# PythonerJOJO/GenPose2

Hardware: AMD Instinct MI355X
Metric: pose candidates/sec (B objs x K cands x T denoise steps) (higher is better)
Workload: dtype f32 (pose_encoder.2 / head-1 GEMMs: f16x3 -- three f16 planes per fp32 operand, six MFMA products, products to 2^-33, fp32 accumulation; encoder SA levels 1-3: split-f16, per-level error vs float64 within exact fp32 MFMA's: tests/test_gpu_precision.py); 1 GPU; config4: B=256 objects/GPU, N=1024 pts, K=50 candidates, T=500 PC steps, ScoreNet+EnergyNet+ranking/aggregation (encoder + sampler per step); global_batch=256, seq_len=500, parallelism=dp1 (object shards), encoder_pipelined=False, energy_encoder=beside the score encoder

## Files before the change

genpose2_amd/_lib.py:

```python
from __future__ import annotations

import ctypes
import os
from typing import Dict, Iterable

_HERE = os.path.dirname(os.path.abspath(__file__))
LIB_PATH = os.environ.get("GENPOSE_HIP_LIB", os.path.join(_HERE, "libgenpose_hip.so"))

c_int, c_float, c_size_t, c_void_p = ctypes.c_int, ctypes.c_float, ctypes.c_size_t, ctypes.c_void_p
c_double = ctypes.c_double
c_int64_p = ctypes.POINTER(ctypes.c_int64)
c_uint64 = ctypes.c_uint64


class GenPoseHipError(RuntimeError):
    pass


class HeadWeights(ctypes.Structure):
    _fields_ = [(n, c_void_p) for n in ("pe0_w", "pe0_b", "pe2_w", "pe2_b", "h1p_w", "h2_w", "h2_b",
                                       "h1pts_t", "h1_b", "gfp_w", "te_w_t", "te_b", "h1t_t", "pe2_h", "h1p_h",
                                       "hsc")]


class HeadGradWeights(ctypes.Structure):
    _fields_ = [(n, c_void_p) for n in ("pe0_wt", "pe2_wt", "h1p_wt")]


class ScaleWeights(ctypes.Structure):
    _fields_ = [(n, c_void_p) for n in ("ae0_w", "ae0_b", "ae2_w", "ae2_b", "ft0_w", "ft0_b", "ft2_w",
                                       "ft2_b")]


_SIGS: Dict[str, tuple] = {
    "gp_last_error": (ctypes.c_char_p, []),
    "gp_abi_version": (c_int, []),
    "gp_furthest_point_sampling": (c_int, [c_int, c_int, c_int, c_void_p, c_void_p, c_void_p, c_void_p]),
    "gp_gather_points": (c_int, [c_int, c_int, c_int, c_int, c_void_p, c_void_p, c_void_p, c_void_p]),
    "gp_ball_query": (c_int, [c_int, c_int, c_int, c_float, c_int, c_void_p, c_void_p, c_void_p, c_void_p]),
    "gp_group_points": (c_int, [c_int, c_int, c_int, c_int, c_int, c_void_p, c_void_p, c_void_p, c_void_p]),
    "gp_encoder_workspace_size": (c_size_t, [c_int, c_int]),
    "gp_encoder_workspace_layout": (c_int, [c_int, c_int, c_int64_p]),
    "gp_encoder_forward": (c_int, [c_void_p, c_int64_p, c_void_p, c_int, c_int, c_void_p, c_size_t, c_void_p,
                                   c_void_p]),
    "gp_encoder_fps": (c_int, [c_void_p, c_int, c_int, c_void_p, c_size_t, c_void_p]),
    "gp_encoder_geometry": (c_int, [c_void_p, c_int, c_int, c_void_p, c_size_t, c_void_p]),
    "gp_encoder_forward_geom": (c_int, [c_void_p, c_int64_p, c_void_p, c_int, c_int, c_void_p, c_void_p, c_size_t,
                                        c_void_p, c_void_p]),
    "gp_encoder_geometry_levels": (c_int, [c_void_p, c_int, c_int, c_void_p, c_size_t, c_int, c_int, c_void_p]),
    "gp_encoder_forward_geom_levels": (c_int, [c_void_p, c_int64_p, c_void_p, c_int, c_int, c_void_p, c_void_p,
                                               c_size_t, c_void_p, c_int, c_int, c_void_p]),
    "gp_sa_level": (c_int, [c_void_p, c_int64_p, c_int, c_int, c_void_p, c_int, c_int, c_void_p, c_void_p, c_size_t,
                            c_void_p, c_void_p]),
    "gp_sa_level_geom": (c_int, [c_void_p, c_int64_p, c_int, c_int, c_void_p, c_int, c_int, c_void_p, c_void_p,
                                 c_void_p, c_size_t, c_void_p, c_void_p]),
    "gp_linear": (c_int, [c_void_p, c_int, c_int, c_int, c_void_p, c_void_p, c_int, c_int, c_void_p, c_int, c_void_p]),
    "gp_linear_split_words": (c_size_t, [c_int, c_int]),
    "gp_linear_split": (c_int, [c_void_p, c_int, c_int, c_int, c_void_p, c_void_p, c_int, c_int, c_void_p, c_int,
                                c_void_p, c_int, c_void_p, c_void_p]),
    "gp_add_layernorm": (c_int, [c_void_p, c_void_p, c_int, c_int, c_void_p, c_void_p, c_float, c_void_p, c_void_p,
                                 c_void_p]),
    "gp_relpe_bias_bytes": (c_size_t, [c_int, c_int]),
    "gp_relpe_bias": (c_int, [c_void_p, c_void_p, c_int, c_int, c_void_p, c_void_p]),
    "gp_mha_attention": (c_int, [c_void_p, c_void_p, c_int, c_int, c_int, c_void_p, c_void_p, c_void_p]),
    "gp_mha_relpe_attention": (c_int, [c_void_p, c_void_p, c_void_p, c_int, c_int, c_int, c_void_p, c_void_p,
                                       c_void_p]),
    "gp_interp_points": (c_int, [c_void_p, c_int, c_int, c_int, c_int, c_void_p, c_void_p, c_void_p]),
    "gp_fusion_attend_workspace_size": (c_size_t, [c_int, c_int, c_int]),
    "gp_fusion_attend": (c_int, [c_void_p, c_void_p, c_int, c_int, c_int, c_void_p, c_void_p, c_void_p, c_void_p,
                                 c_void_p, c_void_p, c_void_p, c_void_p, c_size_t, c_void_p]),
    "gp_fusion_mix": (c_int, [c_void_p, c_void_p, c_int, c_int, c_void_p, c_void_p]),
    "gp_weights_pack": (c_int, [c_int, c_int, c_void_p, c_void_p, c_void_p, ctypes.POINTER(c_void_p)]),
    "gp_weights_free": (None, [c_void_p]),
    "gp_weights_heads": (ctypes.POINTER(HeadWeights), [c_void_p]),
    "gp_weights_scale": (ctypes.POINTER(ScaleWeights), [c_void_p]),
    "gp_weights_encoder": (c_void_p, [c_void_p, ctypes.POINTER(c_int64_p)]),
    "gp_weights_pack_host": (c_int, [c_int, c_int, c_void_p, c_void_p, c_void_p, c_void_p, c_size_t,
                                     ctypes.POINTER(c_size_t), c_int64_p, c_int64_p]),
    "gp_head_object_proj": (c_int, [ctypes.POINTER(HeadWeights), c_void_p, c_int, c_void_p, c_void_p]),
    "gp_head_time_proj": (c_int, [ctypes.POINTER(HeadWeights), c_void_p, c_int, c_void_p, c_void_p]),
    "gp_score_eval": (c_int, [ctypes.POINTER(HeadWeights), c_void_p, c_void_p, c_float, c_void_p, c_int, c_int,
                              c_void_p, c_void_p]),
    "gp_energy_eval": (c_int, [ctypes.POINTER(HeadWeights), c_void_p, c_void_p, c_float, c_void_p, c_int, c_int,
                               c_void_p, c_void_p]),
    "gp_head_grad_floats": (c_size_t, []),
    "gp_head_grad_pack": (c_int, [c_void_p, c_void_p, c_void_p, c_void_p]),
    "gp_energy_score_eval": (c_int, [ctypes.POINTER(HeadWeights), ctypes.POINTER(HeadGradWeights), c_void_p, c_void_p,
                                     c_float, c_void_p, c_int, c_int, c_void_p, c_void_p, c_void_p]),
    "gp_pc_sample_energy": (c_int, [ctypes.POINTER(HeadWeights), ctypes.POINTER(HeadGradWeights), c_void_p, c_void_p,
                                    c_void_p, c_int, c_void_p, c_int, c_int, c_void_p, c_void_p, c_void_p, c_uint64,
                                    c_float, c_void_p, c_void_p, c_void_p, c_void_p, c_size_t, c_void_p]),
    "gp_pc_workspace_size": (c_size_t, [c_int]),
    "gp_pc_tile_rows": (c_int, [c_int, c_int]),
    "gp_pc_sample": (c_int, [ctypes.POINTER(HeadWeights), c_void_p, c_void_p, c_void_p, c_int, c_void_p, c_int,
                             c_int, c_void_p, c_void_p, c_void_p, c_uint64, c_float, c_void_p, c_void_p, c_void_p,
                             c_void_p, c_size_t, c_void_p]),
    "gp_pc_global_partials": (c_int, [c_int, c_int, c_int, c_int]),
    "gp_pc_sample_global": (c_int, [ctypes.POINTER(HeadWeights), c_void_p, c_void_p, c_void_p, c_int, c_void_p, c_int,
                                    c_int, c_void_p, c_uint64, c_float, c_void_p, c_void_p, c_void_p, c_int, c_int,
                                    c_int, c_int, c_int, c_void_p, c_void_p, c_void_p, c_void_p, c_size_t, c_void_p]),
    "gp_pose_epilogue_f64": (c_int, [c_void_p, c_int, c_int, c_void_p, c_void_p, c_void_p]),
    "gp_ode_workspace_size": (c_size_t, [c_int]),
    "gp_ode_rhs": (c_int, [ctypes.POINTER(HeadWeights), c_void_p, c_float, c_float, c_double, c_void_p, c_void_p,
                           c_void_p, c_int, c_double, c_int, c_int, c_void_p, c_void_p, c_size_t, c_void_p]),
    "gp_ode_attempt": (c_int, [ctypes.POINTER(HeadWeights), c_void_p, c_void_p, c_void_p, c_void_p, c_void_p,
                               c_void_p, c_void_p, c_void_p, c_void_p, c_double, c_double, c_double, c_int, c_int,
                               c_void_p, c_void_p, c_void_p, c_size_t, c_void_p]),
    "gp_score_div_eval": (c_int, [ctypes.POINTER(HeadWeights), c_void_p, c_void_p, c_float, c_void_p, c_void_p, c_int,
                                  c_int, c_void_p, c_void_p, c_void_p]),
    "gp_like_workspace_size": (c_size_t, [c_int]),
    "gp_like_rhs": (c_int, [ctypes.POINTER(HeadWeights), c_void_p, c_float, c_float, c_double, c_void_p, c_void_p,
                            c_void_p, c_void_p, c_int, c_double, c_int, c_int, c_void_p, c_void_p, c_size_t,
                            c_void_p]),
    "gp_like_attempt": (c_int, [ctypes.POINTER(HeadWeights), c_void_p, c_void_p, c_void_p, c_void_p, c_void_p,
                                c_void_p, c_void_p, c_void_p, c_void_p, c_void_p, c_double, c_double, c_double,
                                c_int, c_int, c_void_p, c_void_p, c_void_p, c_size_t, c_void_p]),
    "gp_ode_init_norms": (c_int, [c_void_p, c_void_p, c_void_p, ctypes.c_longlong, c_double, c_double, c_void_p,
                                  c_void_p]),
    "gp_ode_dense": (c_int, [c_void_p, c_void_p, c_void_p, c_void_p, c_int, c_int, c_int, c_int, c_double, c_double,
                             ctypes.c_longlong, c_void_p, c_void_p]),
    "gp_ode_denoise": (c_int, [ctypes.POINTER(HeadWeights), c_void_p, c_float, c_float, c_float, c_float, c_void_p,
                               c_int, c_int, c_void_p, c_void_p, c_void_p, c_void_p, c_size_t, c_void_p]),
    "gp_ode_ctl_size": (c_size_t, []),
    "gp_ode_auto_workspace_size": (c_size_t, [c_int]),
    "gp_ode_auto_attempt": (c_int, [ctypes.POINTER(HeadWeights), c_void_p, c_int, c_int, c_double, c_double, c_double,
                                    c_double, c_double, c_double, c_double, c_void_p, c_void_p, c_void_p, c_void_p,
                                    c_void_p, c_void_p, c_int, c_int, c_void_p, c_size_t, c_void_p]),
    "gp_ode_auto_attempt_hs": (c_int, [ctypes.POINTER(HeadWeights), c_void_p, c_int, c_int, c_double, c_double, c_double,
                                    c_double, c_double, c_double, c_double, c_void_p, c_void_p, c_void_p, c_void_p,
                                    c_void_p, c_void_p, c_int, c_int, c_void_p, c_size_t, c_void_p, c_void_p]),
    "gp_ode_global_partials": (c_int, [c_int, c_int, c_int, c_int]),
    "gp_ode_global_workspace_size": (c_size_t, [c_int]),
    "gp_ode_auto_partials_offset": (c_size_t, []),
    "gp_ode_auto_attempt_global": (c_int, [ctypes.POINTER(HeadWeights), c_void_p, c_int, c_int, c_double, c_double,
                                           c_double, c_double, c_double, c_double, c_double, c_void_p, c_void_p,
                                           c_void_p, c_void_p, c_void_p, c_void_p, c_int, c_int, c_int, c_int, c_int,
                                           c_int, c_int, c_void_p, c_void_p, c_void_p, c_size_t, c_void_p,
                                           c_void_p]),
    "gp_pc_step_table": (c_int, [c_int, c_float, c_void_p]),
    "gp_ode_sample_workspace_size": (c_size_t, [c_int]),
    "gp_ode_sample": (c_int, [ctypes.POINTER(HeadWeights), c_void_p, c_void_p, c_int, c_int, c_double, c_double,
                              c_int, c_double, c_double, c_void_p, c_void_p, c_void_p, ctypes.POINTER(c_int),
                              ctypes.POINTER(c_int), c_void_p, c_size_t, c_void_p]),
    "gp_img_encoder_workspace_size": (c_size_t, [c_int, c_int, c_int]),
    "gp_img_encoder": (c_int, [c_void_p, c_void_p, c_void_p, c_int, c_int, c_int, c_void_p, c_void_p, c_void_p, c_float,
                               c_void_p, c_void_p, c_void_p, c_float, c_float, c_void_p, c_void_p, c_void_p, c_void_p,
                               c_size_t, c_void_p]),
    "gp_img_encoder2": (c_int, [c_void_p, c_void_p, c_void_p, c_int, c_int, c_int, c_void_p, c_void_p, c_void_p, c_float,
                                c_void_p, c_void_p, c_void_p, c_float, c_float, c_void_p, c_void_p, c_void_p, c_void_p,
                                c_void_p, c_void_p, c_size_t, c_void_p]),
    "gp_img_encoder3": (c_int, [c_void_p, c_void_p, c_void_p, c_int, c_int, c_int, c_void_p, c_void_p, c_void_p, c_float,
                                c_void_p, c_void_p, c_void_p, c_float, c_float, c_void_p, c_void_p, c_void_p, c_void_p,
                                c_void_p, c_void_p, c_size_t, c_void_p]),
    "gp_img_encoder3_workspace_size": (c_size_t, [c_int, c_int, c_int, c_int]),
    "gp_img_geo_table": (c_int, [c_void_p, c_int, c_int, c_int, c_void_p]),
    "gp_gather_patch_points": (c_int, [c_void_p, c_int, c_int, c_int, c_void_p, c_void_p, c_int, c_int, c_int,
                                       c_void_p, c_void_p]),
    "gp_scale_forward": (c_int, [ctypes.POINTER(ScaleWeights), c_void_p, c_void_p, c_int, c_void_p, c_void_p]),
    "gp_randn": (c_int, [c_uint64, ctypes.c_uint32, c_int, c_int, c_void_p, c_void_p]),
    "gp_points_mean": (c_int, [c_void_p, c_int, c_int, c_int, c_void_p, c_void_p]),
    "gp_bbox_length": (c_int, [c_void_p, c_int, c_int, c_int, c_void_p, c_void_p, c_void_p]),
    "gp_rank_aggregate": (c_int, [c_void_p, c_void_p, c_int, c_int, c_int, c_int, c_float, c_int, c_void_p, c_void_p,
                                  c_void_p, c_void_p]),
}

EXPORTED = tuple(_SIGS)
_lib = None


PC_EXCHANGE_FN = ctypes.CFUNCTYPE(c_int, c_void_p, c_int, c_void_p, c_int, c_void_p)
ODE_EXCHANGE_FN = PC_EXCHANGE_FN


def load(path: str = LIB_PATH):
    global _lib
    if _lib is not None:
        return _lib
    if not os.path.exists(path):
        raise GenPoseHipError(f"{path} not found: build it with `python -c 'import __graft_entry__ as g; "
                              f"g.build()'` (there is no CPU fallback)")
    lib = ctypes.CDLL(path)
    for name, (res, args) in _SIGS.items():
        fn = getattr(lib, name)
        fn.restype = res
        fn.argtypes = args
    _lib = lib
    return lib


def check(rc: int, what: str = "") -> None:
    if rc != 0:
        msg = load().gp_last_error().decode(errors="replace")
        raise GenPoseHipError(f"{what or 'genpose_hip'} failed ({rc}): {msg}")


def exported_symbols(path: str = LIB_PATH) -> Iterable[str]:
    lib = ctypes.CDLL(path)
    return [n for n in _SIGS if hasattr(lib, n)]
```

genpose2_amd/csrc/gp_head.h:

```cpp
#pragma once
#include "gp_common.h"

constexpr int HT = 256;
constexpr int HID = 256;
constexpr int KG_HID = HID / 16;
#ifndef PC_WV1
#define PC_WV1 8
#endif
#ifndef EVAL_WV
#define EVAL_WV 8
#endif
#ifndef PC_D2
#define PC_D2 3
#endif
#ifndef HEAD_PREFETCH
#define HEAD_PREFETCH 2
#endif


#ifndef PC_MARK
#define PC_MARK(k) ((void)trace_slot)
#endif


__device__ __forceinline__ int tid_x() {
    int t = threadIdx.x;
    asm volatile("" : "+v"(t));
    return t;
}

template <int NT, int WV, int PL = 0>
struct HeadSmem {
    static constexpr bool kAliasAct = NT >= 4;
    static constexpr int kAct = PL ? (HID / 32) * NT * PL * 64 : KG_HID * NT * 64;
    float xin[NT * 16 * 16];
    f32x4 act1[kAct];
    f32x4 act2[kAliasAct ? 4 : kAct];
    static constexpr int kRedV = (9 * NT + 3) / 4 * 4;
    float red[kRedV][16][WV];
    float xu[NT * 16 * 9];
    float scratch[WV * 64];
    f32x4 pe0w[PL ? 1 : 16 * 64];
    float pe0b[PL ? 1 : HID], pe2b[HID];
    float h2w[9 * HID];
    float h2b[12];
    f32x4 cscl[NT * 16][2];
};

template <int NT, int WV, int FIRST = 0, bool PE0 = true, int PL>
__device__ __forceinline__ void stage_small_weights(const gp_head_weights& w, HeadSmem<NT, WV, PL>& sm) {
    static_assert(PE0 || PL, "the fp32 trunk reads pose_encoder.0 from LDS");
    constexpr int NTH = WV * 64 - FIRST;
    const int t0 = (int)threadIdx.x - FIRST;
    if (t0 < 0) return;
    if constexpr (PE0)
        for (int i = t0; i < 16 * 64; i += NTH) sm.pe0w[i] = ld4(w.pe0_w + (size_t)i * 4);
    for (int i = t0; i < HID; i += NTH) {
        if constexpr (PE0) sm.pe0b[i] = w.pe0_b[i];
        sm.pe2b[i] = w.pe2_b[i];
    }
    for (int i = t0; i < 9 * HID / 4; i += NTH) st4(&sm.h2w[i * 4], ld4(w.h2_w + (size_t)i * 4));
    if (t0 < 9) sm.h2b[t0] = w.h2_b[t0];
}

template <int NT, int WV, int PL>
__device__ __forceinline__ float head_out(const HeadSmem<NT, WV, PL>& sm, int c, int o) {
    const int h = o / 3;
    const int v = (h * NT + (c >> 4)) * 3 + (o - 3 * h);
    float acc = 0.f;
#pragma unroll
    for (int w = 0; w < WV; ++w) acc += sm.red[v][c & 15][w];
    return sm.h2b[o] + acc;
}

__device__ __forceinline__ void wave_sync() {
    __builtin_amdgcn_fence(__ATOMIC_RELEASE, "wavefront");
    __builtin_amdgcn_wave_barrier();
    __builtin_amdgcn_fence(__ATOMIC_ACQUIRE, "wavefront");
}

template <int G, int GEND, int TT, int NT, int KG, int D>
__device__ __forceinline__ void stream_step(__amdgpu_buffer_rsrc_t W, const int (&T)[TT], const f32x4* __restrict__ B,
                                            int lane, int voff, f32x4 (&ring)[D + 1][TT], f32x4 (&acc)[TT][NT]) {
    if constexpr (G < GEND) {
        if constexpr (G < KG) {
#pragma unroll
            for (int t = 0; t < TT; ++t) ring[G % (D + 1)][t] = ldbuf4(W, voff, (T[t] * KG + G) * 1024);
        }
        __builtin_amdgcn_sched_barrier(0);
        if constexpr (G >= D) {
            constexpr int GG = G - D;
            f32x4 bf[NT];
#pragma unroll
            for (int ct = 0; ct < NT; ++ct) bf[ct] = B[(GG * NT + ct) * 64 + lane];
#pragma unroll
            for (int j = 0; j < 4; ++j)
#pragma unroll
                for (int t = 0; t < TT; ++t)
#pragma unroll
                    for (int ct = 0; ct < NT; ++ct)
                        acc[t][ct] = mfma4(ring[GG % (D + 1)][t][j], bf[ct][j], acc[t][ct]);
        }
        stream_step<G + 1, GEND, TT, NT, KG, D>(W, T, B, lane, voff, ring, acc);
    }
}

template <int TT, int NT, int KG, int D>
__device__ __forceinline__ void stream_layer(__amdgpu_buffer_rsrc_t W, const int (&T)[TT],
                                             const f32x4* __restrict__ B, int lane, f32x4 (&acc)[TT][NT]) {
    f32x4 ring[D + 1][TT];
    stream_step<0, KG + D, TT, NT, KG, D>(W, T, B, lane, lane * 16, ring, acc);
}

__device__ __forceinline__ f32x4 mask4(f32x4 d, f32x4 pre) {
    return f32x4{pre.x > 0.f ? d.x : 0.f, pre.y > 0.f ? d.y : 0.f, pre.z > 0.f ? d.z : 0.f, pre.w > 0.f ? d.w : 0.f};
}
template <int NT, int WV, int PL>
__device__ __forceinline__ float head_out_tan(const HeadSmem<NT, WV, PL>& sm, int c, int o) {
    const int h = o / 3;
    const int v = (h * NT + (c >> 4)) * 3 + (o - 3 * h);
    float acc = 0.f;
#pragma unroll
    for (int w = 0; w < WV; ++w) acc += sm.red[v][c & 15][w];
    return acc;
}

struct GradSmem {
    f32x4 gh[3 * KG_HID * 64];
    f32x4 g2[KG_HID * 64];
};

template <int NT, int WV, bool JVP = false, bool GRAD = false>
__device__ __forceinline__ void head_trunk(const gp_head_weights& w, const float* __restrict__ pobj,
                           const float* __restrict__ tproj, const int* obj_of_col, HeadSmem<NT, WV>& sm,
                           int trace_slot = 0, GradSmem* gs = nullptr, float sigma = 1.f) {
    static_assert(!GRAD || (NT == 1 && !JVP), "the reverse pass runs one 16-candidate tile");
    constexpr int TPW = 16 / WV;
    constexpr int NP = JVP ? NT / 2 : NT;
    static_assert(!JVP || NT % 2 == 0, "a JVP trunk pairs every primal tile with a tangent tile");
    static_assert(!HeadSmem<NT, WV>::kAliasAct, "the exact-fp32 trunk keeps separate activation buffers");
    const int lane = threadIdx.x & 63;
    const int wid = __builtin_amdgcn_readfirstlane(threadIdx.x >> 6);
    const int q = lane >> 4, n = lane & 15;
    const int voff = lane * 16;
    const __amdgpu_buffer_rsrc_t W2 = make_rsrc(w.pe2_w, HID * HID * 4);
    const __amdgpu_buffer_rsrc_t WH = make_rsrc(w.h1p_w, 3 * HID * HID * 4);
    constexpr int D2 = PC_D2, DH = HEAD_PREFETCH;
    int T2[TPW], TH[3 * TPW];
#pragma unroll
    for (int t = 0; t < TPW; ++t) T2[t] = wid * TPW + t;
#pragma unroll
    for (int h = 0; h < 3; ++h)
#pragma unroll
        for (int t = 0; t < TPW; ++t) TH[h * TPW + t] = h * 16 + wid * TPW + t;
    f32x4 acc2[TPW][NT];
#pragma unroll
    for (int t = 0; t < TPW; ++t)
#pragma unroll
        for (int ct = 0; ct < NT; ++ct) acc2[t][ct] = f32x4{0.f, 0.f, 0.f, 0.f};
    f32x4 ring2[D2 + 1][TPW];
    stream_step<0, D2, TPW, NT, KG_HID, D2>(W2, T2, sm.act1, lane, voff, ring2, acc2);
    __syncthreads();
    PC_MARK(1);
    {
        f32x4 bf[NT];
#pragma unroll
        for (int ct = 0; ct < NT; ++ct) bf[ct] = ld4(&sm.xin[(ct * 16 + n) * 16 + 4 * q]);
#pragma unroll
        for (int t = 0; t < TPW; ++t) {
            const int T = wid * TPW + t;
            const f32x4 a = sm.pe0w[T * 64 + lane];
            const f32x4 bias = ld4(&sm.pe0b[16 * T + 4 * q]);
            if constexpr (JVP) {
#pragma unroll
                for (int ct = 0; ct < NP; ++ct) {
                    const f32x4 pre = mfma_kgroup(a, bf[ct], f32x4{0.f, 0.f, 0.f, 0.f}) + bias;
                    sm.act1[(T * NT + ct) * 64 + lane] = relu4(pre);
                    sm.act1[(T * NT + NP + ct) * 64 + lane] =
                        mask4(mfma_kgroup(a, bf[NP + ct], f32x4{0.f, 0.f, 0.f, 0.f}), pre);
                }
            } else {
#pragma unroll
                for (int ct = 0; ct < NT; ++ct)
                    sm.act1[(T * NT + ct) * 64 + lane] = relu4(mfma_kgroup(a, bf[ct], f32x4{0.f, 0.f, 0.f, 0.f}) + bias);
            }
        }
    }
    __syncthreads();
    PC_MARK(2);
    constexpr int PE2_TAIL = 4;
    stream_step<D2, KG_HID + D2 - PE2_TAIL, TPW, NT, KG_HID, D2>(W2, T2, sm.act1, lane, voff, ring2, acc2);
    f32x4 tpv[3 * TPW], pov[3 * TPW][NP];
#pragma unroll
    for (int i = 0; i < 3 * TPW; ++i) {
        const int T = TH[i];
        tpv[i] = ld4(tproj + 16 * T + 4 * q);
#pragma unroll
        for (int ct = 0; ct < NP; ++ct) pov[i][ct] = ld4(pobj + (size_t)obj_of_col[ct * 16 + n] * (3 * HID) + 16 * T + 4 * q);
    }
    stream_step<KG_HID + D2 - PE2_TAIL, KG_HID + D2, TPW, NT, KG_HID, D2>(W2, T2, sm.act1, lane, voff, ring2, acc2);
    PC_MARK(3);
    f32x4 acc[3 * TPW][NT];
#pragma unroll
    for (int i = 0; i < 3 * TPW; ++i)
#pragma unroll
        for (int ct = 0; ct < NT; ++ct) {
            if constexpr (JVP) {
                if (ct < NP) acc[i][ct] = pov[i][ct < NP ? ct : 0] + tpv[i];
                else acc[i][ct] = f32x4{0.f, 0.f, 0.f, 0.f};
            } else {
                acc[i][ct] = pov[i][ct] + tpv[i];
            }
        }
    f32x4 ringh[DH + 1][3 * TPW];
    stream_step<0, DH, 3 * TPW, NT, KG_HID, DH>(WH, TH, sm.act2, lane, voff, ringh, acc);
#pragma unroll
    for (int t = 0; t < TPW; ++t) {
        const f32x4 bias = ld4(&sm.pe2b[16 * T2[t] + 4 * q]);
#pragma unroll
        for (int ct = 0; ct < NT; ++ct) {
            if constexpr (JVP)
                sm.act2[(T2[t] * NT + ct) * 64 + lane] =
                    ct < NP ? relu4(acc2[t][ct] + bias) : mask4(acc2[t][ct], acc2[t][ct < NP ? 0 : ct - NP] + bias);
            else
                sm.act2[(T2[t] * NT + ct) * 64 + lane] = relu4(acc2[t][ct] + bias);
        }
    }
    __syncthreads();
    PC_MARK(4);
    stream_step<DH, KG_HID + DH, 3 * TPW, NT, KG_HID, DH>(WH, TH, sm.act2, lane, voff, ringh, acc);
    PC_MARK(5);
#pragma unroll
    for (int h = 0; h < 3; ++h) {
        [[maybe_unused]] float c0 = 0.f, c1 = 0.f, c2 = 0.f;
        if constexpr (GRAD) {
            c0 = fdiv(ld1(&sm.xin[n * 16 + 3 * h + 0]), sigma);
            c1 = fdiv(ld1(&sm.xin[n * 16 + 3 * h + 1]), sigma);
            c2 = fdiv(ld1(&sm.xin[n * 16 + 3 * h + 2]), sigma);
        }
#pragma unroll
        for (int ct = 0; ct < NT; ++ct) {
            float p0 = 0.f, p1 = 0.f, p2 = 0.f;
#pragma unroll
            for (int t = 0; t < TPW; ++t) {
                f32x4 u;
                if constexpr (JVP)
                    u = ct < NP ? relu4(acc[h * TPW + t][ct])
                                : mask4(acc[h * TPW + t][ct], acc[h * TPW + t][ct < NP ? 0 : ct - NP]);
                else
                    u = relu4(acc[h * TPW + t][ct]);
                const int ch = 16 * (wid * TPW + t) + 4 * q;
                const f32x4 w0 = ld4(&sm.h2w[(h * 3 + 0) * HID + ch]);
                const f32x4 w1 = ld4(&sm.h2w[(h * 3 + 1) * HID + ch]);
                const f32x4 w2 = ld4(&sm.h2w[(h * 3 + 2) * HID + ch]);
                p0 += u.x * w0.x + u.y * w0.y + u.z * w0.z + u.w * w0.w;
                p1 += u.x * w1.x + u.y * w1.y + u.z * w1.z + u.w * w1.w;
                p2 += u.x * w2.x + u.y * w2.y + u.z * w2.z + u.w * w2.w;
                if constexpr (GRAD)
                    gs->gh[TH[h * TPW + t] * 64 + lane] = mask4(w0 * c0 + w1 * c1 + w2 * c2, acc[h * TPW + t][ct]);
            }
            p0 = rows_sum(p0);
            p1 = rows_sum(p1);
            p2 = rows_sum(p2);
            if (q == 0) {
                sm.red[(h * NT + ct) * 3 + 0][n][wid] = p0;
                sm.red[(h * NT + ct) * 3 + 1][n][wid] = p1;
                sm.red[(h * NT + ct) * 3 + 2][n][wid] = p2;
            }
        }
    }
    if constexpr (!GRAD) __syncthreads();
    PC_MARK(6);
}

#ifndef GRAD_D
#define GRAD_D 4
#endif

template <int WV>
__device__ __forceinline__ void head_backward(const gp_head_grad_weights& gw, const HeadSmem<1, WV>& sm, GradSmem& gs,
                                              int trace_slot = 0) {
    constexpr int TPW = 16 / WV;
    constexpr int KPW = KG_HID / WV;
    constexpr int D = GRAD_D;
    static_assert(KPW * WV == KG_HID && WV * 64 <= KG_HID * 64, "the partial tiles fit g2");
    const int tid = tid_x();
    const int lane = tid & 63;
    const int wid = __builtin_amdgcn_readfirstlane(tid >> 6);
    const int voff = lane * 16;
    const __amdgpu_buffer_rsrc_t WH = make_rsrc(gw.h1p_wt, 3 * HID * HID * 4);
    const __amdgpu_buffer_rsrc_t W2 = make_rsrc(gw.pe2_wt, HID * HID * 4);
    const __amdgpu_buffer_rsrc_t W0 = make_rsrc(gw.pe0_wt, 16 * HID * 4);
    int T2[TPW];
#pragma unroll
    for (int t = 0; t < TPW; ++t) T2[t] = wid * TPW + t;
    f32x4 ring[D + 1][TPW];
    f32x4 acc[TPW][1];
#pragma unroll
    for (int t = 0; t < TPW; ++t) acc[t][0] = f32x4{0.f, 0.f, 0.f, 0.f};
    stream_step<0, D, TPW, 1, 3 * KG_HID, D>(WH, T2, gs.gh, lane, voff, ring, acc);
    __syncthreads();
    PC_MARK(13);
    stream_step<D, 3 * KG_HID + D, TPW, 1, 3 * KG_HID, D>(WH, T2, gs.gh, lane, voff, ring, acc);
#pragma unroll
    for (int t = 0; t < TPW; ++t) {
        gs.g2[T2[t] * 64 + lane] = mask4(acc[t][0], sm.act2[T2[t] * 64 + lane]);
        acc[t][0] = f32x4{0.f, 0.f, 0.f, 0.f};
    }
    f32x4* g1 = gs.gh;
    stream_step<0, D, TPW, 1, KG_HID, D>(W2, T2, gs.g2, lane, voff, ring, acc);
    __syncthreads();
    PC_MARK(14);
    stream_step<D, KG_HID + D, TPW, 1, KG_HID, D>(W2, T2, gs.g2, lane, voff, ring, acc);
#pragma unroll
    for (int t = 0; t < TPW; ++t) g1[T2[t] * 64 + lane] = mask4(acc[t][0], sm.act1[T2[t] * 64 + lane]);
    const int T0[1] = {wid};
    f32x4 ring0[KPW + 1][1];
    f32x4 acc0[1][1] = {{f32x4{0.f, 0.f, 0.f, 0.f}}};
    stream_step<0, KPW, 1, 1, KPW, KPW>(W0, T0, g1, lane, voff, ring0, acc0);
    __syncthreads();
    PC_MARK(15);
    stream_step<KPW, 2 * KPW, 1, 1, KPW, KPW>(W0, T0, g1 + wid * KPW * 64, lane, voff, ring0, acc0);
    gs.g2[wid * 64 + lane] = acc0[0][0];
    __syncthreads();
}

template <int WV>
__device__ __forceinline__ float pose_grad(const GradSmem& gs, int c, int o) {
    float acc = 0.f;
#pragma unroll
    for (int w = 0; w < WV; ++w) acc += gs.g2[w * 64 + 16 * (o >> 2) + c][o & 3];
    return acc;
}

typedef _Float16 f16x8 __attribute__((ext_vector_type(8)));
constexpr int KC_HID = HID / 32;

__device__ __forceinline__ f32x4 mfma_h(f16x8 a, f16x8 b, f32x4 c) {
    return __builtin_amdgcn_mfma_f32_16x16x32_f16(a, b, c, 0, 0, 0);
}
__device__ __forceinline__ float exp2i(int e) {
    e = e < -126 ? -126 : (e > 127 ? 127 : e);
    return __uint_as_float((uint32_t)(e + 127) << 23);
}
__device__ __forceinline__ int ilog2f(float v) { return (int)((__float_as_uint(v) >> 23) & 0xff) - 127; }
__device__ __forceinline__ float rows_max(float v) {
    const auto a = __builtin_amdgcn_permlane16_swap(__float_as_uint(v), __float_as_uint(v), false, false);
    v = fmaxf(__uint_as_float(a[0]), __uint_as_float(a[1]));
    const auto b = __builtin_amdgcn_permlane32_swap(__float_as_uint(v), __float_as_uint(v), false, false);
    return fmaxf(__uint_as_float(b[0]), __uint_as_float(b[1]));
}
__device__ __forceinline__ void split_pair(f32x4 u, f32x4 v, float s, f16x8& hi, f16x8& lo) {
#pragma clang fp contract(off)
    const float x[8] = {u.x * s, u.y * s, u.z * s, u.w * s, v.x * s, v.y * s, v.z * s, v.w * s};
#pragma unroll
    for (int j = 0; j < 8; ++j) {
        const _Float16 h = (_Float16)x[j];
        hi[j] = h;
        lo[j] = (_Float16)(x[j] - (float)h);
    }
}

template <int KC, int G, int GEND, int TT, int NT, int D>
__device__ __forceinline__ void stream_hk_step(__amdgpu_buffer_rsrc_t W, const int (&T)[TT], const f16x8* __restrict__ B,
                                               int lane, int voff, f16x8 (&ring)[D + 1][TT][2], f32x4 (&acc)[TT][NT]) {
    if constexpr (G < GEND) {
        if constexpr (G < KC) {
#pragma unroll
            for (int t = 0; t < TT; ++t)
#pragma unroll
                for (int p = 0; p < 2; ++p)
                    ring[G % (D + 1)][t][p] =
                        __builtin_bit_cast(f16x8, ldbuf4(W, voff, ((T[t] * KC + G) * 2 + p) * 1024));
        }
        __builtin_amdgcn_sched_barrier(0);
        if constexpr (G >= D && NT > 4) {
            constexpr int GG = G - D, S = GG % (D + 1);
#pragma unroll
            for (int ct = 0; ct < NT; ++ct) {
                const f16x8 bh = B[((GG * NT + ct) * 2 + 0) * 64 + lane];
                const f16x8 bl = B[((GG * NT + ct) * 2 + 1) * 64 + lane];
#pragma unroll
                for (int t = 0; t < TT; ++t) acc[t][ct] = mfma_h(ring[S][t][1], bh, acc[t][ct]);
#pragma unroll
                for (int t = 0; t < TT; ++t) acc[t][ct] = mfma_h(ring[S][t][0], bl, acc[t][ct]);
#pragma unroll
                for (int t = 0; t < TT; ++t) acc[t][ct] = mfma_h(ring[S][t][0], bh, acc[t][ct]);
            }
        } else if constexpr (G >= D) {
            constexpr int GG = G - D, S = GG % (D + 1);
            f16x8 bh[NT], bl[NT];
#pragma unroll
            for (int ct = 0; ct < NT; ++ct) {
                bh[ct] = B[((GG * NT + ct) * 2 + 0) * 64 + lane];
                bl[ct] = B[((GG * NT + ct) * 2 + 1) * 64 + lane];
            }
#pragma unroll
            for (int t = 0; t < TT; ++t)
#pragma unroll
                for (int ct = 0; ct < NT; ++ct) acc[t][ct] = mfma_h(ring[S][t][1], bh[ct], acc[t][ct]);
#pragma unroll
            for (int t = 0; t < TT; ++t)
#pragma unroll
                for (int ct = 0; ct < NT; ++ct) acc[t][ct] = mfma_h(ring[S][t][0], bl[ct], acc[t][ct]);
#pragma unroll
            for (int t = 0; t < TT; ++t)
#pragma unroll
                for (int ct = 0; ct < NT; ++ct) acc[t][ct] = mfma_h(ring[S][t][0], bh[ct], acc[t][ct]);
        }
        stream_hk_step<KC, G + 1, GEND, TT, NT, D>(W, T, B, lane, voff, ring, acc);
    }
}


constexpr int HSPLIT_WV = 8;
struct SplitScalars {
    float A0, B0, A2, B2;
    int ew2, ewh;
    f32x4 pe0a[4], pe0b[4];
};
template <int WV = HSPLIT_WV>
__device__ __forceinline__ SplitScalars load_split_scalars(const gp_head_weights& w) {
    static_assert(WV == 4 || WV == 8, "the split trunk runs 4- or 8-wave workgroups");
    const f32x4 a = ld4(w.hsc), b = ld4(w.hsc + 4);
    SplitScalars r{a.x, a.y, a.z, a.w, (int)b.x, (int)b.y, {}, {}};
    const int tid = tid_x();
    const int lane = tid & 63, q = lane >> 4;
    const int wid = __builtin_amdgcn_readfirstlane(tid >> 6);
#pragma unroll
    for (int t = 0; t < 16 / WV; ++t) {
        const int T = wid * (16 / WV) + t;
        r.pe0a[t] = ld4(w.pe0_w + ((size_t)T * 64 + lane) * 4);
        r.pe0b[t] = ld4(w.pe0_b + 16 * T + 4 * q);
    }
    return r;
}

__device__ __forceinline__ float rows_sum_scatter4(float a, float b, float c, float d) {
    const auto ab = __builtin_amdgcn_permlane16_swap(__float_as_uint(a), __float_as_uint(b), false, false);
    const auto cd = __builtin_amdgcn_permlane16_swap(__float_as_uint(c), __float_as_uint(d), false, false);
    const float s = __uint_as_float(ab[0]) + __uint_as_float(ab[1]);
    const float t = __uint_as_float(cd[0]) + __uint_as_float(cd[1]);
    const auto st = __builtin_amdgcn_permlane32_swap(__float_as_uint(s), __float_as_uint(t), false, false);
    return __uint_as_float(st[0]) + __uint_as_float(st[1]);
}


struct ColScales {
    float s1, s2, u2, uh, sh;
};
__device__ __forceinline__ ColScales split_col_scales(float m0, const SplitScalars& hs) {
    const float b1 = fmaxf(__builtin_fmaf(hs.A0, m0, hs.B0) * 1.0009765625f, 1e-18f);
    const float b2 = fmaxf(__builtin_fmaf(hs.A2, b1, hs.B2) * 1.0009765625f, 1e-18f);
    const int e1 = ilog2f(b1), e2 = ilog2f(b2);
    return ColScales{exp2i(14 - e1), exp2i(14 - e2), exp2i(e1 - 14 - hs.ew2), exp2i(e2 - 14 - hs.ewh),
                     exp2i(14 - e2 + hs.ewh)};
}
__device__ __forceinline__ float xin_row_absmax(f32x4 b) {
    return rows_max(fmaxf(fmaxf(fabsf(b.x), fabsf(b.y)), fmaxf(fabsf(b.z), fabsf(b.w))));
}

#ifndef X3_D2
#define X3_D2 2
#endif
#ifndef X3_DH
#define X3_DH 1
#endif
#ifndef X3_PRIO
#define X3_PRIO 0
#endif
#ifndef X3_BPIPE
#define X3_BPIPE 1
#endif
#ifndef X3_CHAIN
#define X3_CHAIN 1
#endif
#ifndef X3_EPI_EARLY
#define X3_EPI_EARLY 1
#endif
#ifndef X3_DIAG
#define X3_DIAG 0
#endif
#ifndef X3_HEAD_BARRIER
#define X3_HEAD_BARRIER 0
#endif
constexpr int X3P = 3;

__device__ __forceinline__ void split3(float x, _Float16& h, _Float16& m, _Float16& l) {
#pragma clang fp contract(off)
    h = (_Float16)x;
    const float r = x - (float)h;
    m = (_Float16)r;
    l = (_Float16)(r - (float)m);
}
__device__ __forceinline__ void split3_pair(f32x4 u, f32x4 v, float s, f16x8 (&p)[X3P]) {
#pragma clang fp contract(off)
    const float x[8] = {u.x * s, u.y * s, u.z * s, u.w * s, v.x * s, v.y * s, v.z * s, v.w * s};
#pragma unroll
    for (int j = 0; j < 8; ++j) {
        _Float16 h, m, l;
        split3(x[j], h, m, l);
        p[0][j] = h;
        p[1][j] = m;
        p[2][j] = l;
    }
}

template <int G, int GEND, int TT, int NT, int D>
__device__ __forceinline__ void stream_x3_rec(__amdgpu_buffer_rsrc_t W, const int (&T)[TT], const f16x8* __restrict__ B,
                                              int lane, int voff, f16x8 (&ring)[D + 1][TT][X3P],
                                              f32x4 (&acc)[TT][NT], f32x4 (&cor)[TT][NT], f16x8 (&bc)[X3P]) {
    if constexpr (G < GEND) {
        if constexpr (G < KC_HID && ((X3_DIAG & 2) == 0 || G < D + 1)) {
#pragma unroll
            for (int t = 0; t < TT; ++t)
#pragma unroll
                for (int p = 0; p < X3P; ++p)
                    ring[G % (D + 1)][t][p] =
                        __builtin_bit_cast(f16x8, ldbuf4(W, voff, ((T[t] * KC_HID + G) * X3P + p) * 1024));
        }
        __builtin_amdgcn_sched_barrier(0);
        if constexpr (G >= D) {
            constexpr int GG = G - D, S = GG % (D + 1);
#if X3_PRIO
            if ((__builtin_amdgcn_readfirstlane(threadIdx.x >> 8) ^ GG) & 1)
                __builtin_amdgcn_s_setprio(1);
            else
                __builtin_amdgcn_s_setprio(0);
#endif
#if X3_BPIPE
            if constexpr (GG == 0) {
#pragma unroll
                for (int p = 0; p < X3P; ++p) bc[p] = B[p * 64 + lane];
            }
#pragma unroll
            for (int ct = 0; ct < NT; ++ct) {
                f16x8 bn[X3P];
                const int nx = ct + 1 < NT ? (GG * NT + ct + 1) : ((GG + 1) * NT);
                if ((X3_DIAG & 1) == 0 && (ct + 1 < NT || GG + 1 < KC_HID)) {
#pragma unroll
                    for (int p = 0; p < X3P; ++p) bn[p] = B[(nx * X3P + p) * 64 + lane];
                }
#if X3_DIAG & 1
#pragma unroll
                for (int p = 0; p < X3P; ++p) {
                    using u4 = __attribute__((ext_vector_type(4))) unsigned;
                    bn[p] = __builtin_bit_cast(f16x8, __builtin_bit_cast(u4, bc[p]) ^ (unsigned)(nx + 1));
                }
#endif
                __builtin_amdgcn_sched_barrier(0);
                const f16x8 b0 = bc[0], b1 = bc[1], b2 = bc[2];
#if X3_CHAIN
#pragma unroll
                for (int t = 0; t < TT; ++t) {
                    f32x4 c = cor[t][ct];
                    c = mfma_h(ring[S][t][2], b0, c);
                    c = mfma_h(ring[S][t][0], b2, c);
                    c = mfma_h(ring[S][t][1], b1, c);
                    c = mfma_h(ring[S][t][1], b0, c);
                    c = mfma_h(ring[S][t][0], b1, c);
                    cor[t][ct] = c;
                    __builtin_amdgcn_sched_barrier(0);
                }
#pragma unroll
                for (int t = 0; t < TT; ++t) acc[t][ct] = mfma_h(ring[S][t][0], b0, acc[t][ct]);
#else
#pragma unroll
                for (int t = 0; t < TT; ++t) {
                    f32x4 c = cor[t][ct];
                    c = mfma_h(ring[S][t][2], b0, c);
                    c = mfma_h(ring[S][t][0], b2, c);
                    c = mfma_h(ring[S][t][1], b1, c);
                    c = mfma_h(ring[S][t][1], b0, c);
                    c = mfma_h(ring[S][t][0], b1, c);
                    cor[t][ct] = c;
                    acc[t][ct] = mfma_h(ring[S][t][0], b0, acc[t][ct]);
                }
#endif
                __builtin_amdgcn_sched_barrier(0);
                if (ct + 1 < NT || GG + 1 < KC_HID) {
#pragma unroll
                    for (int p = 0; p < X3P; ++p) bc[p] = bn[p];
                }
            }
#else
#pragma unroll
            for (int ct = 0; ct < NT; ++ct) {
                const f16x8 b0 = B[((GG * NT + ct) * X3P + 0) * 64 + lane];
                const f16x8 b1 = B[((GG * NT + ct) * X3P + 1) * 64 + lane];
                const f16x8 b2 = B[((GG * NT + ct) * X3P + 2) * 64 + lane];
#pragma unroll
                for (int t = 0; t < TT; ++t) {
                    f32x4 c = cor[t][ct];
                    c = mfma_h(ring[S][t][2], b0, c);
                    c = mfma_h(ring[S][t][0], b2, c);
                    c = mfma_h(ring[S][t][1], b1, c);
                    c = mfma_h(ring[S][t][1], b0, c);
                    c = mfma_h(ring[S][t][0], b1, c);
                    cor[t][ct] = c;
                    acc[t][ct] = mfma_h(ring[S][t][0], b0, acc[t][ct]);
                }
            }
#endif
        }
        stream_x3_rec<G + 1, GEND, TT, NT, D>(W, T, B, lane, voff, ring, acc, cor, bc);
    }
}
template <int G, int GEND, int TT, int NT, int D>
__device__ __forceinline__ void stream_x3_step(__amdgpu_buffer_rsrc_t W, const int (&T)[TT], const f16x8* __restrict__ B,
                                               int lane, int voff, f16x8 (&ring)[D + 1][TT][X3P],
                                               f32x4 (&acc)[TT][NT], f32x4 (&cor)[TT][NT]) {
    f16x8 bc[X3P];
    stream_x3_rec<G, GEND, TT, NT, D>(W, T, B, lane, voff, ring, acc, cor, bc);
}

template <int H, int NT, int TPW, int NP = NT>
__device__ __forceinline__ void head_x3_init_load(__amdgpu_buffer_rsrc_t RP, __amdgpu_buffer_rsrc_t RT, const int (&vo)[NT],
                                                  int wid, int lane, f32x4 (&tpv)[TPW], f32x4 (&pov)[TPW][NP]) {
    const int q = lane >> 4;
#pragma unroll
    for (int t = 0; t < TPW; ++t) {
        const int T = H * 16 + wid * TPW + t;
        tpv[t] = ldbuf4(RT, 16 * q, 64 * T);
#pragma unroll
        for (int ct = 0; ct < NP; ++ct) pov[t][ct] = ldbuf4(RP, vo[ct], 64 * T);
    }
}

template <int H, int NT, int WV, int TPW, int DH, bool JVP = false>
__device__ __forceinline__ void head_x3_head(__amdgpu_buffer_rsrc_t WH, const f16x8* __restrict__ act2h,
                                             __amdgpu_buffer_rsrc_t RP, __amdgpu_buffer_rsrc_t RT, const int (&vo)[NT],
                                             HeadSmem<NT, WV, X3P>& sm, const float (&uh)[NT], const float (&sh)[NT],
                                             int wid, int lane, f16x8 (&ringh)[DH + 1][TPW][X3P],
                                             f32x4 (&tpv)[TPW], f32x4 (&pov)[TPW][JVP ? NT / 2 : NT],
                                             float (&pv)[HeadSmem<NT, WV, X3P>::kRedV]) {
    constexpr int NP = JVP ? NT / 2 : NT;
    const int q = lane >> 4, n = lane & 15;
    const int voff = lane * 16;
    int TH[TPW];
#pragma unroll
    for (int t = 0; t < TPW; ++t) TH[t] = H * 16 + wid * TPW + t;
    f32x4 acc[TPW][NT], cor[TPW][NT];
#pragma unroll
    for (int t = 0; t < TPW; ++t)
#pragma unroll
        for (int ct = 0; ct < NT; ++ct) {
            if constexpr (JVP) {
                if (ct < NP) acc[t][ct] = (pov[t][ct < NP ? ct : 0] + tpv[t]) * sh[ct];
                else acc[t][ct] = f32x4{0.f, 0.f, 0.f, 0.f};
            } else {
                acc[t][ct] = (pov[t][ct] + tpv[t]) * sh[ct];
            }
            cor[t][ct] = f32x4{0.f, 0.f, 0.f, 0.f};
        }
    stream_x3_step<DH, KC_HID + DH, TPW, NT, DH>(WH, TH, act2h, lane, voff, ringh, acc, cor);
    if constexpr (H < 2) {
        int TN[TPW];
#pragma unroll
        for (int t = 0; t < TPW; ++t) TN[t] = TH[t] + 16;
        stream_x3_step<0, DH, TPW, NT, DH>(WH, TN, act2h, lane, voff, ringh, acc, cor);
        head_x3_init_load<H + 1, NT, TPW, NP>(RP, RT, vo, wid, lane, tpv, pov);
    }
    __builtin_amdgcn_sched_barrier(0);
    float p[NT][3];
#pragma unroll
    for (int ct = 0; ct < NT; ++ct) p[ct][0] = p[ct][1] = p[ct][2] = 0.f;
#if X3_DIAG & 4
#pragma unroll
    for (int t = 0; t < TPW; ++t)
#pragma unroll
        for (int ct = 0; ct < NT; ++ct)
#pragma unroll
            for (int o = 0; o < 3; ++o) p[ct][o] += acc[t][ct][o] + cor[t][ct][o + 1];
#else
#pragma unroll
    for (int t = 0; t < TPW; ++t) {
        const int ch = 16 * (wid * TPW + t) + 4 * q;
        const f32x4 w0 = ld4(&sm.h2w[(H * 3 + 0) * HID + ch]);
        const f32x4 w1 = ld4(&sm.h2w[(H * 3 + 1) * HID + ch]);
        const f32x4 w2 = ld4(&sm.h2w[(H * 3 + 2) * HID + ch]);
#pragma unroll
        for (int ct = 0; ct < NT; ++ct) {
            f32x4 u;
            if constexpr (JVP) {
                constexpr int NPP = JVP ? NP : 0;
                const int cp = ct < NPP ? 0 : ct - NPP;
                u = ct < NPP ? relu4((acc[t][ct] + cor[t][ct]) * uh[ct])
                             : mask4((acc[t][ct] + cor[t][ct]) * uh[ct], (acc[t][cp] + cor[t][cp]) * uh[cp]);
            } else {
                u = relu4((acc[t][ct] + cor[t][ct]) * uh[ct]);
            }
#pragma unroll
            for (int j = 0; j < 4; ++j) {
                p[ct][0] = __builtin_fmaf(u[j], w0[j], p[ct][0]);
                p[ct][1] = __builtin_fmaf(u[j], w1[j], p[ct][1]);
                p[ct][2] = __builtin_fmaf(u[j], w2[j], p[ct][2]);
            }
        }
    }
#endif
#pragma unroll
    for (int ct = 0; ct < NT; ++ct)
#pragma unroll
        for (int o = 0; o < 3; ++o) pv[(H * NT + ct) * 3 + o] = p[ct][o];
    if constexpr ((3 * NT) % 4 == 0) {
#pragma unroll
        for (int g = H * 3 * NT / 4; g < (H + 1) * 3 * NT / 4; ++g)
            sm.red[4 * g + q][n][wid] = rows_sum_scatter4(pv[4 * g], pv[4 * g + 1], pv[4 * g + 2], pv[4 * g + 3]);
    }
    __builtin_amdgcn_sched_barrier(0);
}

template <int NT, int WV, bool PRE = false, bool JVP = false>
__device__ __forceinline__ void head_trunk_x3(const gp_head_weights& w, const float* __restrict__ pobj,
                                              const float* __restrict__ tproj, const int* obj_of_col,
                                              HeadSmem<NT, WV, X3P>& sm, int trace_slot, const SplitScalars hs) {
    constexpr int TPW = 16 / WV;
    static_assert(TPW % 2 == 0, "the f16x3 trunk pairs a wave's output tiles into 32-deep chunks");
    static_assert(TPW <= 4, "SplitScalars carries at most four pose_encoder.0 tiles per wave");
    constexpr int CPW = TPW / 2;
    constexpr int NP = JVP ? NT / 2 : NT;
    static_assert(!JVP || NT % 2 == 0, "a JVP trunk pairs every primal tile with a tangent tile");
    using SM = HeadSmem<NT, WV, X3P>;
    const int tid = tid_x();
    const int lane = tid & 63;
    const int wid = __builtin_amdgcn_readfirstlane(tid >> 6);
    const int q = lane >> 4, n = lane & 15;
    const int voff = lane * 16;
    const __amdgpu_buffer_rsrc_t W2 = make_rsrc(w.pe2_h, HID * HID * 2 * X3P);
    const __amdgpu_buffer_rsrc_t WH = make_rsrc(w.h1p_h, 3 * HID * HID * 2 * X3P);
    f16x8* act1h = reinterpret_cast<f16x8*>(sm.act1);
    f16x8* act2h = reinterpret_cast<f16x8*>(SM::kAliasAct ? sm.act1 : sm.act2);
    constexpr int D2 = X3_D2, DH = X3_DH;
    int T2[TPW];
#pragma unroll
    for (int t = 0; t < TPW; ++t) T2[t] = wid * TPW + t;
    f32x4 acc2[TPW][NT], cor2[TPW][NT];
#pragma unroll
    for (int t = 0; t < TPW; ++t)
#pragma unroll
        for (int ct = 0; ct < NT; ++ct) acc2[t][ct] = cor2[t][ct] = f32x4{0.f, 0.f, 0.f, 0.f};
    f16x8 ring2[D2 + 1][TPW][X3P];
    stream_x3_step<0, D2, TPW, NT, D2>(W2, T2, act1h, lane, voff, ring2, acc2, cor2);
    __syncthreads();
    PC_MARK(1);
    f32x4 bf[NT];
    float s1[NT], s2[NT], u2[NT], uh[NT], sh[NT];
#pragma unroll
    for (int ct = 0; ct < NT; ++ct) {
        bf[ct] = ld4(&sm.xin[(ct * 16 + n) * 16 + 4 * q]);
        ColScales cs;
        if constexpr (PRE) {
            const f32x4 a = sm.cscl[ct * 16 + n][0];
            cs = ColScales{a.x, a.y, a.z, a.w, sm.cscl[ct * 16 + n][1].x};
        } else {
            cs = split_col_scales(xin_row_absmax(bf[ct]), hs);
        }
        s1[ct] = cs.s1;
        s2[ct] = cs.s2;
        u2[ct] = cs.u2;
        uh[ct] = cs.uh;
        sh[ct] = cs.sh;
    }
#pragma unroll
    for (int c = 0; c < CPW; ++c) {
        const int Ta = wid * TPW + 2 * c;
        const f32x4 a0 = hs.pe0a[2 * c], a1 = hs.pe0a[2 * c + 1];
        const f32x4 bias0 = hs.pe0b[2 * c], bias1 = hs.pe0b[2 * c + 1];
#pragma unroll
        for (int ct = 0; ct < NP; ++ct) {
            const f32x4 z = f32x4{0.f, 0.f, 0.f, 0.f};
            f16x8 pl[X3P];
            if constexpr (JVP) {
                constexpr int dt = JVP ? NP : 0;
                const f32x4 pre0 = mfma_kgroup(a0, bf[ct], z) + bias0, pre1 = mfma_kgroup(a1, bf[ct], z) + bias1;
                split3_pair(relu4(pre0), relu4(pre1), s1[ct], pl);
#pragma unroll
                for (int p = 0; p < X3P; ++p) act1h[(((Ta >> 1) * NT + ct) * X3P + p) * 64 + lane] = pl[p];
                split3_pair(mask4(mfma_kgroup(a0, bf[ct + dt], z), pre0), mask4(mfma_kgroup(a1, bf[ct + dt], z), pre1),
                            s1[ct + dt], pl);
#pragma unroll
                for (int p = 0; p < X3P; ++p) act1h[(((Ta >> 1) * NT + ct + dt) * X3P + p) * 64 + lane] = pl[p];
            } else {
                split3_pair(relu4(mfma_kgroup(a0, bf[ct], z) + bias0), relu4(mfma_kgroup(a1, bf[ct], z) + bias1), s1[ct], pl);
#pragma unroll
                for (int p = 0; p < X3P; ++p) act1h[(((Ta >> 1) * NT + ct) * X3P + p) * 64 + lane] = pl[p];
            }
        }
    }
    __syncthreads();
    PC_MARK(2);
    stream_x3_step<D2, KC_HID + D2, TPW, NT, D2>(W2, T2, act1h, lane, voff, ring2, acc2, cor2);
    PC_MARK(3);
    f16x8 ringh[DH + 1][TPW][X3P];
    {
        int TH0[TPW];
#pragma unroll
        for (int t = 0; t < TPW; ++t) TH0[t] = wid * TPW + t;
        stream_x3_step<0, DH, TPW, NT, DH>(WH, TH0, act2h, lane, voff, ringh, acc2, cor2);
    }
    const __amdgpu_buffer_rsrc_t RP = make_rsrc(pobj, 0x7ffffff0u), RT = make_rsrc(tproj, 3 * HID * 4);
    int vo[NT];
#pragma unroll
    for (int ct = 0; ct < NT; ++ct) vo[ct] = obj_of_col[ct * 16 + n] * (3 * HID * 4) + 16 * q;
    f32x4 tpv[TPW], pov[TPW][NP];
    head_x3_init_load<0, NT, TPW, NP>(RP, RT, vo, wid, lane, tpv, pov);
#if X3_EPI_EARLY
    f16x8 pls[CPW][NT][X3P];
#pragma unroll
    for (int c = 0; c < CPW; ++c) {
        const int Ta = T2[2 * c];
        const f32x4 bias0 = ld4(&sm.pe2b[16 * Ta + 4 * q]), bias1 = ld4(&sm.pe2b[16 * (Ta + 1) + 4 * q]);
#pragma unroll
        for (int ct = 0; ct < NP; ++ct) {
            if constexpr (JVP) {
                constexpr int dt = JVP ? NP : 0;
                const f32x4 pre0 = (acc2[2 * c][ct] + cor2[2 * c][ct]) * u2[ct] + bias0;
                const f32x4 pre1 = (acc2[2 * c + 1][ct] + cor2[2 * c + 1][ct]) * u2[ct] + bias1;
                split3_pair(relu4(pre0), relu4(pre1), s2[ct], pls[c][ct]);
                split3_pair(mask4((acc2[2 * c][ct + dt] + cor2[2 * c][ct + dt]) * u2[ct + dt], pre0),
                            mask4((acc2[2 * c + 1][ct + dt] + cor2[2 * c + 1][ct + dt]) * u2[ct + dt], pre1),
                            s2[ct + dt], pls[c][ct + dt]);
            } else {
                split3_pair(relu4((acc2[2 * c][ct] + cor2[2 * c][ct]) * u2[ct] + bias0),
                            relu4((acc2[2 * c + 1][ct] + cor2[2 * c + 1][ct]) * u2[ct] + bias1), s2[ct], pls[c][ct]);
            }
        }
    }
    if constexpr (SM::kAliasAct) __syncthreads();
#pragma unroll
    for (int c = 0; c < CPW; ++c)
#pragma unroll
        for (int ct = 0; ct < NT; ++ct)
#pragma unroll
            for (int p = 0; p < X3P; ++p) act2h[(((T2[2 * c] >> 1) * NT + ct) * X3P + p) * 64 + lane] = pls[c][ct][p];
#else
    if constexpr (SM::kAliasAct) __syncthreads();
#pragma unroll
    for (int c = 0; c < CPW; ++c) {
        const int Ta = T2[2 * c];
        const f32x4 bias0 = ld4(&sm.pe2b[16 * Ta + 4 * q]), bias1 = ld4(&sm.pe2b[16 * (Ta + 1) + 4 * q]);
#pragma unroll
        for (int ct = 0; ct < NP; ++ct) {
            f16x8 pl[X3P];
            if constexpr (!JVP) {
                split3_pair(relu4((acc2[2 * c][ct] + cor2[2 * c][ct]) * u2[ct] + bias0),
                            relu4((acc2[2 * c + 1][ct] + cor2[2 * c + 1][ct]) * u2[ct] + bias1), s2[ct], pl);
#pragma unroll
                for (int p = 0; p < X3P; ++p) act2h[(((Ta >> 1) * NT + ct) * X3P + p) * 64 + lane] = pl[p];
            } else {
                constexpr int dt = JVP ? NP : 0;
                const f32x4 pre0 = (acc2[2 * c][ct] + cor2[2 * c][ct]) * u2[ct] + bias0;
                const f32x4 pre1 = (acc2[2 * c + 1][ct] + cor2[2 * c + 1][ct]) * u2[ct] + bias1;
                split3_pair(relu4(pre0), relu4(pre1), s2[ct], pl);
#pragma unroll
                for (int p = 0; p < X3P; ++p) act2h[(((Ta >> 1) * NT + ct) * X3P + p) * 64 + lane] = pl[p];
                split3_pair(mask4((acc2[2 * c][ct + dt] + cor2[2 * c][ct + dt]) * u2[ct + dt], pre0),
                            mask4((acc2[2 * c + 1][ct + dt] + cor2[2 * c + 1][ct + dt]) * u2[ct + dt], pre1),
                            s2[ct + dt], pl);
#pragma unroll
                for (int p = 0; p < X3P; ++p) act2h[(((Ta >> 1) * NT + ct + dt) * X3P + p) * 64 + lane] = pl[p];
            }
        }
    }
#endif
    __syncthreads();
    PC_MARK(4);
    float pv[SM::kRedV];
#pragma unroll
    for (int v = 9 * NT; v < SM::kRedV; ++v) pv[v] = 0.f;
#if X3_DIAG & 8
    if (wid < WV / 2) {
        head_x3_head<0, NT, WV, TPW, DH, JVP>(WH, act2h, RP, RT, vo, sm, uh, sh, wid, lane, ringh, tpv, pov, pv);
        PC_MARK(13);
        head_x3_head<1, NT, WV, TPW, DH, JVP>(WH, act2h, RP, RT, vo, sm, uh, sh, wid, lane, ringh, tpv, pov, pv);
        PC_MARK(14);
        head_x3_head<2, NT, WV, TPW, DH, JVP>(WH, act2h, RP, RT, vo, sm, uh, sh, wid, lane, ringh, tpv, pov, pv);
        const int vw = wid + WV / 2;
        int TV[TPW];
#pragma unroll
        for (int t = 0; t < TPW; ++t) TV[t] = vw * TPW + t;
        stream_x3_step<0, DH, TPW, NT, DH>(WH, TV, act2h, lane, voff, ringh, acc2, cor2);
        head_x3_init_load<0, NT, TPW, NP>(RP, RT, vo, vw, lane, tpv, pov);
        head_x3_head<0, NT, WV, TPW, DH, JVP>(WH, act2h, RP, RT, vo, sm, uh, sh, vw, lane, ringh, tpv, pov, pv);
        head_x3_head<1, NT, WV, TPW, DH, JVP>(WH, act2h, RP, RT, vo, sm, uh, sh, vw, lane, ringh, tpv, pov, pv);
        head_x3_head<2, NT, WV, TPW, DH, JVP>(WH, act2h, RP, RT, vo, sm, uh, sh, vw, lane, ringh, tpv, pov, pv);
    }
#else
    head_x3_head<0, NT, WV, TPW, DH, JVP>(WH, act2h, RP, RT, vo, sm, uh, sh, wid, lane, ringh, tpv, pov, pv);
    if constexpr (X3_HEAD_BARRIER) __syncthreads();
    PC_MARK(13);
    head_x3_head<1, NT, WV, TPW, DH, JVP>(WH, act2h, RP, RT, vo, sm, uh, sh, wid, lane, ringh, tpv, pov, pv);
    if constexpr (X3_HEAD_BARRIER) __syncthreads();
    PC_MARK(14);
    head_x3_head<2, NT, WV, TPW, DH, JVP>(WH, act2h, RP, RT, vo, sm, uh, sh, wid, lane, ringh, tpv, pov, pv);
#endif
    if constexpr (X3_PRIO) __builtin_amdgcn_s_setprio(0);
    PC_MARK(5);
    if constexpr ((3 * NT) % 4 != 0) {
#pragma unroll
        for (int g = 0; g < SM::kRedV / 4; ++g)
            sm.red[4 * g + q][n][wid] = rows_sum_scatter4(pv[4 * g], pv[4 * g + 1], pv[4 * g + 2], pv[4 * g + 3]);
    }
    __syncthreads();
    PC_MARK(6);
}

#ifndef PC_SPLIT_NT2_MIN
#define PC_SPLIT_NT2_MIN 4097
#endif
#ifndef PC_SPLIT_NT4_MIN
#define PC_SPLIT_NT4_MIN 8193
#endif
static inline int head_pick_nt(int rows, bool split) {
    if (!split) return 1;
    return rows >= PC_SPLIT_NT4_MIN ? 4 : (rows >= PC_SPLIT_NT2_MIN ? 2 : 1);
}

template <typename T>
__device__ __forceinline__ T tsqrt(T v);
template <>
__device__ __forceinline__ float tsqrt<float>(float v) { return sqrtf(v); }
template <>
__device__ __forceinline__ double tsqrt<double>(double v) { return sqrt(v); }

template <typename T>
__device__ __forceinline__ void gram_schmidt6(T* v) {
#pragma clang fp contract(off)
    T n1 = tsqrt<T>((v[0] * v[0] + v[1] * v[1]) + v[2] * v[2]);
    n1 = n1 > (T)1e-12 ? n1 : (T)1e-12;
    const T b0 = v[0] / n1, b1 = v[1] / n1, b2 = v[2] / n1;
    const T d = (b0 * v[3] + b1 * v[4]) + b2 * v[5];
    T c0 = v[3] - d * b0, c1 = v[4] - d * b1, c2 = v[5] - d * b2;
    T n2 = tsqrt<T>((c0 * c0 + c1 * c1) + c2 * c2);
    n2 = n2 > (T)1e-12 ? n2 : (T)1e-12;
    v[0] = b0;
    v[1] = b1;
    v[2] = b2;
    v[3] = c0 / n2;
    v[4] = c1 / n2;
    v[5] = c2 / n2;
}

#ifdef PC_FAST_UPDATE
__device__ __forceinline__ float udiv(float a, float b) { return a * __builtin_amdgcn_rcpf(b); }
__device__ __forceinline__ float usqrt(float x) { return __builtin_amdgcn_sqrtf(x); }
#else
__device__ __forceinline__ float udiv(float a, float b) { return fdiv(a, b); }
__device__ __forceinline__ float usqrt(float x) { return sqrtf(x); }
#endif

__device__ __forceinline__ void gram_schmidt6_quad(float* v, int p, int lane) {
#pragma clang fp contract(off)
    float n1 = usqrt((v[0] * v[0] + v[1] * v[1]) + v[2] * v[2]);
    n1 = n1 > 1e-12f ? n1 : 1e-12f;
    const float b0 = udiv(v[0], n1), b1 = udiv(v[1], n1), b2 = udiv(v[2], n1);
    (void)lane;
    const float B0 = quad_bcast0(b0), B1 = quad_bcast0(b1), B2 = quad_bcast0(b2);
    const float d = (B0 * v[0] + B1 * v[1]) + B2 * v[2];
    float c0 = v[0] - d * B0, c1 = v[1] - d * B1, c2 = v[2] - d * B2;
    float n2 = usqrt((c0 * c0 + c1 * c1) + c2 * c2);
    n2 = n2 > 1e-12f ? n2 : 1e-12f;
    if (p == 0) {
        v[0] = b0; v[1] = b1; v[2] = b2;
    } else if (p == 1) {
        v[0] = udiv(c0, n2); v[1] = udiv(c1, n2); v[2] = udiv(c2, n2);
    }
}

template <typename T>
__device__ __forceinline__ void quat_from_gs(const T* v, T* qo) {
#pragma clang fp contract(off)
    T g[6] = {v[0], v[1], v[2], v[3], v[4], v[5]};
    gram_schmidt6<T>(g);
    const T b3x = g[1] * g[5] - g[2] * g[4];
    const T b3y = g[2] * g[3] - g[0] * g[5];
    const T b3z = g[0] * g[4] - g[1] * g[3];
    const T m00 = g[0], m01 = g[3], m02 = b3x;
    const T m10 = g[1], m11 = g[4], m12 = b3y;
    const T m20 = g[2], m21 = g[5], m22 = b3z;
    const T one = (T)1;
    T qa[4] = {((one + m00) + m11) + m22, ((one + m00) - m11) - m22, ((one - m00) + m11) - m22,
               ((one - m00) - m11) + m22};
#pragma unroll
    for (int i = 0; i < 4; ++i) qa[i] = qa[i] > (T)0 ? tsqrt<T>(qa[i]) : (T)0;
    int best = 0;
#pragma unroll
    for (int i = 1; i < 4; ++i)
        if (qa[i] > qa[best]) best = i;
    T c[4];
    if (best == 0) {
        c[0] = qa[0] * qa[0]; c[1] = m21 - m12; c[2] = m02 - m20; c[3] = m10 - m01;
    } else if (best == 1) {
        c[0] = m21 - m12; c[1] = qa[1] * qa[1]; c[2] = m10 + m01; c[3] = m02 + m20;
    } else if (best == 2) {
        c[0] = m02 - m20; c[1] = m10 + m01; c[2] = qa[2] * qa[2]; c[3] = m12 + m21;
    } else {
        c[0] = m10 - m01; c[1] = m20 + m02; c[2] = m21 + m12; c[3] = qa[3] * qa[3];
    }
    const T den = (T)2 * (qa[best] > (T)0.1 ? qa[best] : (T)0.1);
#pragma unroll
    for (int i = 0; i < 4; ++i) qo[i] = c[i] / den;
}

template <int N, int CH>
__device__ __forceinline__ float dot_chains(const float* __restrict__ W, size_t stride, const float* x) {
    static_assert(N % CH == 0 && (CH & (CH - 1)) == 0, "N must be a multiple of the power-of-two CH");
    float p[CH];
#pragma unroll
    for (int j = 0; j < CH; ++j) p[j] = 0.f;
#pragma unroll 1
    for (int c0 = 0; c0 < N; c0 += CH) {
#pragma unroll
        for (int j = 0; j < CH; ++j) p[j] = fmaf(W[(size_t)(c0 + j) * stride], x[c0 + j], p[j]);
    }
#pragma unroll
    for (int s = CH / 2; s >= 1; s >>= 1)
#pragma unroll
        for (int j = 0; j < s; ++j) p[j] += p[j + s];
    return p[0];
}

#ifndef HOIST64
#define HOIST64 0
#endif
template <int N>
__device__ __forceinline__ double dot_f64(const float* __restrict__ W, size_t stride, const float* x) {
    double s = 0.0;
#pragma unroll 8
    for (int c = 0; c < N; ++c) s = fma((double)W[(size_t)c * stride], (double)x[c], s);
    return s;
}

__device__ __forceinline__ void time_row(const gp_head_weights& w, float t, float* emb, float* tf,
                                         float* __restrict__ out, int o0 = 0, int o1 = 768) {
    const int i = threadIdx.x;
    if (i < 64) {
        const float a = fmul(fmul(fmul(t, w.gfp_w[i]), 2.0f), 3.14159265358979323846f);
        emb[i] = sinf(a);
        emb[64 + i] = cosf(a);
    }
    __syncthreads();
#if HOIST64
    if (i < 128) tf[i] = fmaxf((float)(dot_f64<128>(w.te_w_t + i, 128, emb) + (double)w.te_b[i]), 0.f);
    __syncthreads();
    for (int o = o0 + i; o < o1; o += HT) out[o] = (float)dot_f64<128>(w.h1t_t + o, 768, tf);
#else
    if (i < 128) tf[i] = fmaxf(dot_chains<128, 16>(w.te_w_t + i, 128, emb) + w.te_b[i], 0.f);
    __syncthreads();
    for (int o = o0 + i; o < o1; o += HT) out[o] = dot_chains<128, 16>(w.h1t_t + o, 768, tf);
#endif
}
```

genpose2_amd/csrc/gp_pack.hip:

```cpp
#include <cmath>
#include <cstring>
#include <map>
#include <string>
#include <vector>

#include "gp_common.h"

namespace {

struct Tensor {
    const float* p;
    int64_t n;
};

struct StateDict {
    std::map<std::string, Tensor> m;
    std::string missing;
    const float* get(const std::string& k, int64_t numel) {
        auto it = m.find(k);
        if (it == m.end() || it->second.n != numel) {
            if (missing.empty())
                missing = k + (it == m.end() ? " (missing)" : " (size " + std::to_string(it->second.n) + ", want " +
                                                                  std::to_string(numel) + ")");
            return nullptr;
        }
        return it->second.p;
    }
};

const int kW[5][2][4] = {{{3, 16, 16, 32}, {3, 32, 32, 64}},
                         {{99, 64, 64, 128}, {99, 64, 96, 128}},
                         {{259, 128, 196, 256}, {259, 128, 196, 256}},
                         {{515, 256, 256, 512}, {515, 256, 384, 512}},
                         {{1027, 512, 512, 0}, {1027, 512, 512, 0}}};
constexpr double kBnEps = 1e-5;

int pad_to(int v, int a) { return (v + a - 1) / a * a; }

std::vector<float> pack_a(const std::vector<float>& w, int n_out, int k_in, int n_pad, int k_pad) {
    std::vector<float> out((size_t)n_pad * k_pad, 0.f);
    const int NT = n_pad / 16, KG = k_pad / 16;
    for (int T = 0; T < NT; ++T)
        for (int g = 0; g < KG; ++g)
            for (int q = 0; q < 4; ++q)
                for (int i = 0; i < 16; ++i)
                    for (int j = 0; j < 4; ++j) {
                        const int r = 16 * T + i, c = 16 * g + 4 * q + j;
                        out[((((size_t)T * KG + g) * 4 + q) * 16 + i) * 4 + j] =
                            (r < n_out && c < k_in) ? w[(size_t)r * k_in + c] : 0.f;
                    }
    return out;
}

int split_exponent(const std::vector<float>& w) {
    float m = 0.f;
    for (float v : w) m = std::fmax(m, std::fabs(v));
    return m > 0.f ? 14 - (int)std::floor(std::log2((double)m)) : 0;
}

std::vector<uint32_t> pack_h16(const std::vector<float>& w, int n_out, int k_in, int e, int planes = 2) {
    const int NT = n_out / 16, KC = k_in / 32;
    std::vector<uint16_t> h((size_t)n_out * k_in * planes);
    const float s = std::ldexp(1.0f, e);
    for (int T = 0; T < NT; ++T)
        for (int c = 0; c < KC; ++c)
            for (int q = 0; q < 4; ++q)
                for (int i = 0; i < 16; ++i)
                    for (int half = 0; half < 2; ++half)
                        for (int j4 = 0; j4 < 4; ++j4) {
                            float r = w[(size_t)(16 * T + i) * k_in + 32 * c + 16 * half + 4 * q + j4] * s;
                            for (int plane = 0; plane < planes; ++plane) {
                                const _Float16 v = (_Float16)r;
                                r = r - (float)v;
                                uint16_t bits;
                                std::memcpy(&bits, &v, 2);
                                h[((((((size_t)T * KC + c) * planes + plane) * 4 + q) * 16 + i) * 2 + half) * 4 + j4] = bits;
                            }
                        }
    std::vector<uint32_t> out(h.size() / 2);
    std::memcpy(out.data(), h.data(), h.size() * 2);
    return out;
}

double np_pairwise(const double* a, int64_t n) {
    if (n < 8) {
        double r = 0.0;
        for (int64_t i = 0; i < n; ++i) r += a[i];
        return r;
    }
    if (n <= 128) {
        double r[8];
        for (int k = 0; k < 8; ++k) r[k] = a[k];
        int64_t i;
        for (i = 8; i < n - (n % 8); i += 8)
            for (int k = 0; k < 8; ++k) r[k] += a[i + k];
        double res = ((r[0] + r[1]) + (r[2] + r[3])) + ((r[4] + r[5]) + (r[6] + r[7]));
        for (; i < n; ++i) res += a[i];
        return res;
    }
    int64_t n2 = n / 2;
    n2 -= n2 % 8;
    return np_pairwise(a, n2) + np_pairwise(a + n2, n - n2);
}

double max_row_l1(const float* w, int rows, int cols) {
    std::vector<double> r(cols);
    double m = 0.0;
    for (int o = 0; o < rows; ++o) {
        for (int c = 0; c < cols; ++c) r[c] = std::fabs((double)w[(size_t)o * cols + c]);
        m = std::fmax(m, np_pairwise(r.data(), cols));
    }
    return m;
}

struct Packer {
    std::vector<float> buf;
    size_t add(const float* p, size_t n) {
        const size_t o = buf.size();
        buf.insert(buf.end(), p, p + n);
        buf.resize(buf.size() + (4 - buf.size() % 4) % 4, 0.f);
        return o;
    }
    size_t add(const std::vector<float>& v) { return add(v.data(), v.size()); }
    size_t add_bits(const std::vector<uint32_t>& v) {
        std::vector<float> f(v.size());
        std::memcpy(f.data(), v.data(), v.size() * 4);
        return add(f);
    }
};

bool fold_conv_bn(StateDict& sd, const std::string& p, int n_out, int k_in, std::vector<float>& W, std::vector<float>& b) {
    const float* w = sd.get(p + ".conv.weight", (int64_t)n_out * k_in);
    const float* g = sd.get(p + ".bn.bn.weight", n_out);
    const float* be = sd.get(p + ".bn.bn.bias", n_out);
    const float* mu = sd.get(p + ".bn.bn.running_mean", n_out);
    const float* var = sd.get(p + ".bn.bn.running_var", n_out);
    if (!w || !g || !be || !mu || !var) return false;
    W.resize((size_t)n_out * k_in);
    b.resize(n_out);
    for (int o = 0; o < n_out; ++o) {
        const double sc = (double)g[o] / std::sqrt((double)var[o] + kBnEps);
        for (int c = 0; c < k_in; ++c) W[(size_t)o * k_in + c] = (float)((double)w[(size_t)o * k_in + c] * sc);
        b[o] = (float)((double)be[o] - (double)mu[o] * sc);
    }
    return true;
}

bool pack_encoder(StateDict& sd, Packer& P, int64_t* table) {
    const size_t base = P.buf.size();
    for (int i = 0; i < 120; ++i) table[i] = -1;
    for (int lv = 0; lv < 5; ++lv) {
        const int c_prev = kW[lv][0][0] - 3;
        const int nl = lv < 4 ? 3 : 2;
        for (int br = 0; br < 2; ++br)
            for (int i = 0; i < nl; ++i) {
                const int n_out = kW[lv][br][i + 1], k_in = kW[lv][br][i];
                std::vector<float> W, b;
                const std::string p = "pts_encoder.SA_modules." + std::to_string(lv) + ".mlps." + std::to_string(br) +
                                      ".layer" + std::to_string(i);
                if (!fold_conv_bn(sd, p, n_out, k_in, W, b)) return false;
                int64_t* row = table + ((lv * 2 + br) * 3 + i) * 4;
                std::vector<float> packed;
                if (i == 0) {
                    std::vector<float> wp((size_t)n_out * (c_prev + 16), 0.f);
                    for (int o = 0; o < n_out; ++o) {
                        for (int c = 0; c < c_prev; ++c) wp[(size_t)o * (c_prev + 16) + c] = W[(size_t)o * k_in + 3 + c];
                        for (int c = 0; c < 3; ++c) wp[(size_t)o * (c_prev + 16) + c_prev + c] = W[(size_t)o * k_in + c];
                    }
                    packed = pack_a(wp, n_out, c_prev + 16, pad_to(n_out, 16), c_prev + 16);
                } else {
                    packed = pack_a(W, n_out, k_in, pad_to(n_out, 16), pad_to(k_in, 16));
                }
                row[0] = (int64_t)(P.add(packed) - base);
                std::vector<float> bp(pad_to(n_out, 32), 0.f);
                std::copy(b.begin(), b.end(), bp.begin());
                row[1] = (int64_t)(P.add(bp) - base);
                if (lv >= 1 || i >= 1) {
                    const int np = pad_to(n_out, 32), kp = pad_to(k_in, 32);
                    std::vector<float> wq((size_t)np * kp, 0.f);
                    for (int o = 0; o < n_out; ++o) {
                        if (i == 0) {
                            for (int c = 0; c < c_prev; ++c) wq[(size_t)o * kp + c] = W[(size_t)o * k_in + 3 + c];
                            for (int c = 0; c < 3; ++c) wq[(size_t)o * kp + c_prev + c] = W[(size_t)o * k_in + c];
                        } else {
                            for (int c = 0; c < k_in; ++c) wq[(size_t)o * kp + c] = W[(size_t)o * k_in + c];
                        }
                    }
                    const int e = split_exponent(W);
                    row[2] = (int64_t)(P.add_bits(pack_h16(wq, np, kp, e)) - base);
                    row[3] = e;
                }
            }
    }
    return true;
}

bool pack_heads(StateDict& sd, Packer& P, int64_t* f) {
    const std::string n = "pose_score_net.";
    const float* pe0_w = sd.get(n + "pose_encoder.0.weight", 256 * 9);
    const float* pe0_b = sd.get(n + "pose_encoder.0.bias", 256);
    const float* pe2_w = sd.get(n + "pose_encoder.2.weight", 256 * 256);
    const float* pe2_b = sd.get(n + "pose_encoder.2.bias", 256);
    const float* gfp = sd.get(n + "t_encoder.0.W", 64);
    const float* te_w = sd.get(n + "t_encoder.1.weight", 128 * 128);
    const float* te_b = sd.get(n + "t_encoder.1.bias", 128);
    const char* heads[3] = {"fusion_tail_rot_x", "fusion_tail_rot_y", "fusion_tail_trans"};
    const float *h1w[3], *h1b[3], *h2w[3], *h2b[3];
    for (int h = 0; h < 3; ++h) {
        h1w[h] = sd.get(n + heads[h] + ".0.weight", 256 * 1408);
        h1b[h] = sd.get(n + heads[h] + ".0.bias", 256);
        h2w[h] = sd.get(n + heads[h] + ".2.weight", 3 * 256);
        h2b[h] = sd.get(n + heads[h] + ".2.bias", 3);
        if (!h1w[h] || !h1b[h] || !h2w[h] || !h2b[h]) return false;
    }
    if (!pe0_w || !pe0_b || !pe2_w || !pe2_b || !gfp || !te_w || !te_b) return false;
    std::vector<float> w_pe0(pe0_w, pe0_w + 256 * 9), w_pe2(pe2_w, pe2_w + 256 * 256);
    std::vector<float> h1_pose((size_t)768 * 256), h1pts_t((size_t)1024 * 768), h1t_t((size_t)128 * 768), h1_b(768);
    std::vector<float> h2_w(9 * 256), h2_b(9), te_w_t(128 * 128);
    for (int h = 0; h < 3; ++h)
        for (int o = 0; o < 256; ++o) {
            const float* row = h1w[h] + (size_t)o * 1408;
            const int oo = h * 256 + o;
            for (int c = 0; c < 1024; ++c) h1pts_t[(size_t)c * 768 + oo] = row[c];
            for (int c = 0; c < 128; ++c) h1t_t[(size_t)c * 768 + oo] = row[1024 + c];
            for (int c = 0; c < 256; ++c) h1_pose[(size_t)oo * 256 + c] = row[1152 + c];
            h1_b[oo] = h1b[h][o];
        }
    for (int h = 0; h < 3; ++h) {
        for (int i = 0; i < 3 * 256; ++i) h2_w[h * 768 + i] = h2w[h][i];
        for (int i = 0; i < 3; ++i) h2_b[h * 3 + i] = h2b[h][i];
    }
    for (int r = 0; r < 128; ++r)
        for (int c = 0; c < 128; ++c) te_w_t[(size_t)c * 128 + r] = te_w[(size_t)r * 128 + c];
    f[0] = P.add(pack_a(w_pe0, 256, 9, 256, 16));
    f[1] = P.add(pe0_b, 256);
    f[2] = P.add(pack_a(w_pe2, 256, 256, 256, 256));
    f[3] = P.add(pe2_b, 256);
    f[4] = P.add(pack_a(h1_pose, 768, 256, 768, 256));
    f[5] = P.add(h2_w);
    f[6] = P.add(h2_b);
    f[7] = P.add(h1pts_t);
    f[8] = P.add(h1_b);
    f[9] = P.add(gfp, 64);
    f[10] = P.add(te_w_t);
    f[11] = P.add(te_b, 128);
    f[12] = P.add(h1t_t);
    const int e2 = split_exponent(w_pe2), eh = split_exponent(h1_pose);
    f[13] = P.add_bits(pack_h16(w_pe2, 256, 256, e2, 3));
    f[14] = P.add_bits(pack_h16(h1_pose, 768, 256, eh, 3));
    float b0 = 0.f, b2 = 0.f;
    for (int i = 0; i < 256; ++i) {
        b0 = std::fmax(b0, std::fabs(pe0_b[i]));
        b2 = std::fmax(b2, std::fabs(pe2_b[i]));
    }
    const float v[4] = {(float)max_row_l1(pe0_w, 256, 9), b0, (float)max_row_l1(pe2_w, 256, 256), b2};
    float hsc[8];
    for (int i = 0; i < 4; ++i) hsc[i] = std::nextafter(v[i], INFINITY);
    hsc[4] = (float)e2;
    hsc[5] = (float)eh;
    hsc[6] = hsc[7] = 0.f;
    f[15] = P.add(hsc, 8);
    return true;
}

bool pack_scale(StateDict& sd, Packer& P, int64_t* f) {
    const char* keys[8] = {"axes_encoder.0.weight", "axes_encoder.0.bias", "axes_encoder.2.weight",
                           "axes_encoder.2.bias", "fusion_tail_length.0.weight", "fusion_tail_length.0.bias",
                           "fusion_tail_length.2.weight", "fusion_tail_length.2.bias"};
    const int64_t sz[8] = {256 * 180, 256, 256 * 256, 256, 256 * 1280, 256, 3 * 256, 3};
    for (int i = 0; i < 8; ++i) {
        const float* p = sd.get(keys[i], sz[i]);
        if (!p) return false;
        f[i] = P.add(p, sz[i]);
    }
    return true;
}

int pack_all(int kind, int n, const char* const* names, const float* const* data, const int64_t* numel, Packer& P,
             int64_t* fields, int64_t* enc_table) {
    GP_REQUIRE(kind >= GP_MODEL_SCORE && kind <= GP_MODEL_SCALE, "weights_pack: kind %d", kind);
    GP_REQUIRE(n >= 0 && (n == 0 || (names && data && numel)), "weights_pack: null arrays");
    StateDict sd;
    for (int i = 0; i < n; ++i) {
        GP_REQUIRE(names[i] && (data[i] || numel[i] == 0), "weights_pack: null entry %d", i);
        std::string k = names[i];
        if (k.rfind("module.", 0) == 0) k = k.substr(7);
        sd.m[k] = Tensor{data[i], numel[i]};
    }
    for (int i = 0; i < GP_PACK_NFIELDS; ++i) fields[i] = -1;
    bool ok;
    if (kind == GP_MODEL_SCALE) {
        ok = pack_scale(sd, P, fields + GP_PACK_SCALE);
    } else {
        fields[GP_PACK_ENC] = 0;
        ok = pack_encoder(sd, P, enc_table) && pack_heads(sd, P, fields + GP_PACK_HEADS);
    }
    if (!ok) {
        gp_set_error("weights_pack: state dict entry %s", sd.missing.c_str());
        return GP_ERR_INVALID;
    }
    return GP_OK;
}

}

struct gp_weights {
    int kind;
    void* dev;
    size_t bytes;
    gp_head_weights heads;
    gp_scale_weights scale;
    int64_t table[120];
};

extern "C" int gp_weights_pack_host(int kind, int n, const char* const* names, const float* const* data,
                                    const int64_t* numel, float* out, size_t out_floats, size_t* need_floats,
                                    int64_t* fields, int64_t* enc_table) {
    GP_REQUIRE(need_floats && fields && enc_table, "weights_pack_host: null outputs");
    Packer P;
    const int rc = pack_all(kind, n, names, data, numel, P, fields, enc_table);
    if (rc) return rc;
    *need_floats = P.buf.size();
    if (out) {
        GP_REQUIRE(out_floats >= P.buf.size(), "weights_pack_host: out holds %zu floats, need %zu", out_floats,
                   P.buf.size());
        std::memcpy(out, P.buf.data(), P.buf.size() * sizeof(float));
    }
    return GP_OK;
}

extern "C" int gp_weights_pack(int kind, int n, const char* const* names, const float* const* data,
                               const int64_t* numel, gp_weights** out) {
    GP_REQUIRE(out, "weights_pack: null out");
    *out = nullptr;
    Packer P;
    int64_t fields[GP_PACK_NFIELDS];
    gp_weights* w = new gp_weights();
    int rc = pack_all(kind, n, names, data, numel, P, fields, w->table);
    if (rc) {
        delete w;
        return rc;
    }
    w->kind = kind;
    w->bytes = P.buf.size() * sizeof(float);
    if (hipMalloc(&w->dev, w->bytes) != hipSuccess ||
        hipMemcpy(w->dev, P.buf.data(), w->bytes, hipMemcpyHostToDevice) != hipSuccess) {
        if (w->dev) (void)hipFree(w->dev);
        delete w;
        return gp_check_launch("weights_pack: device upload");
    }
    const float* base = static_cast<const float*>(w->dev);
    auto at = [&](int64_t o) -> const float* { return o >= 0 ? base + o : nullptr; };
    if (kind == GP_MODEL_SCALE) {
        const float** s = reinterpret_cast<const float**>(&w->scale);
        for (int i = 0; i < 8; ++i) s[i] = at(fields[GP_PACK_SCALE + i]);
    } else {
        const float** h = reinterpret_cast<const float**>(&w->heads);
        for (int i = 0; i < 16; ++i) h[i] = at(fields[GP_PACK_HEADS + i]);
    }
    *out = w;
    return GP_OK;
}

extern "C" int gp_head_grad_pack(const float* pe0_w, const float* pe2_w, const float* h1_pose, float* out) {
    GP_REQUIRE(pe0_w && pe2_w && h1_pose && out, "head_grad_pack: null pointer");
    auto transposed = [](const float* w, int n_out, int k_in) {
        std::vector<float> t((size_t)n_out * k_in);
        for (int o = 0; o < n_out; ++o)
            for (int c = 0; c < k_in; ++c) t[(size_t)c * n_out + o] = w[(size_t)o * k_in + c];
        return t;
    };
    const std::vector<float> p0 = pack_a(transposed(pe0_w, 256, 9), 9, 256, 16, 256);
    const std::vector<float> p2 = pack_a(transposed(pe2_w, 256, 256), 256, 256, 256, 256);
    const std::vector<float> ph = pack_a(transposed(h1_pose, 768, 256), 256, 768, 256, 768);
    std::memcpy(out, p0.data(), p0.size() * sizeof(float));
    std::memcpy(out + p0.size(), p2.data(), p2.size() * sizeof(float));
    std::memcpy(out + p0.size() + p2.size(), ph.data(), ph.size() * sizeof(float));
    return GP_OK;
}

extern "C" void gp_weights_free(gp_weights* w) {
    if (!w) return;
    if (w->dev) (void)hipFree(w->dev);
    delete w;
}

extern "C" const gp_head_weights* gp_weights_heads(const gp_weights* w) {
    return w && w->kind != GP_MODEL_SCALE ? &w->heads : nullptr;
}

extern "C" const gp_scale_weights* gp_weights_scale(const gp_weights* w) {
    return w && w->kind == GP_MODEL_SCALE ? &w->scale : nullptr;
}

extern "C" const float* gp_weights_encoder(const gp_weights* w, const int64_t** layer_off) {
    if (!w || w->kind == GP_MODEL_SCALE) return nullptr;
    if (layer_off) *layer_off = w->table;
    return static_cast<const float*>(w->dev);
}
```

genpose2_amd/csrc/gp_score.hip:

```cpp

#include "gp_common.h"


#ifdef PC_TRACE
constexpr int PC_TR_SLOTS = 20;
__device__ unsigned long long g_pc_trace[3 * 256 * 8 * PC_TR_SLOTS];
#define PC_TR_AT(k) g_pc_trace[((trace_slot * 256 + blockIdx.x) * 8 + (threadIdx.x >> 6)) * PC_TR_SLOTS + (k)]
#define PC_MARK(k)                                                                                       \
    do {                                                                                                 \
        if ((threadIdx.x & 63) == 0 && blockIdx.x < 256) {                                               \
            PC_TR_AT(k) = __builtin_amdgcn_s_memtime();                                                  \
            if ((k) == 0 || (k) == 8) PC_TR_AT(16 + ((k) == 8)) = __builtin_amdgcn_s_memrealtime();      \
            if ((k) == 0)                                                                                \
                PC_TR_AT(18) = (unsigned long long)(unsigned)__builtin_amdgcn_s_getreg((31 << 11) | 4) | \
                               ((unsigned long long)(unsigned)__builtin_amdgcn_s_getreg((3 << 11) | 20) << 32); \
        }                                                                                                \
    } while (0)
extern "C" int gp_debug_pc_trace(unsigned long long* host) {
    return hipMemcpyFromSymbol(host, HIP_SYMBOL(g_pc_trace), sizeof(g_pc_trace)) == hipSuccess ? 0 : -1;
}
#else
#define PC_MARK(k) ((void)trace_slot)
#endif
#include "gp_head.h"

__global__ __launch_bounds__(HT) void object_proj_kernel(gp_head_weights w, const float* __restrict__ feat,
                                                         float* __restrict__ pobj) {
    __shared__ float sf[1024];
    const int b = blockIdx.y;
    for (int i = threadIdx.x; i < 1024; i += HT) sf[i] = feat[(size_t)b * 1024 + i];
    __syncthreads();
    const int o = blockIdx.x * HT + threadIdx.x;
#if HOIST64
    pobj[(size_t)b * 768 + o] = (float)(dot_f64<1024>(w.h1pts_t + o, 768, sf) + (double)w.h1_b[o]);
#else
    pobj[(size_t)b * 768 + o] = dot_chains<1024, 32>(w.h1pts_t + o, 768, sf) + w.h1_b[o];
#endif
}

extern "C" int gp_head_object_proj(const gp_head_weights* w, const float* pts_feat, int b, float* pobj,
                                   hipStream_t stream) {
    GP_REQUIRE(w && pts_feat && pobj && b >= 0, "head_object_proj: bad arguments");
    if (!b) return GP_OK;
    hipLaunchKernelGGL(object_proj_kernel, dim3(3, b), dim3(HT), 0, stream, *w, pts_feat, pobj);
    return gp_check_launch("object_proj_kernel");
}

__global__ __launch_bounds__(HT) void time_proj_kernel(gp_head_weights w, const float* __restrict__ tv,
                                                       float* __restrict__ tproj) {
    __shared__ float emb[128];
    __shared__ float tf[128];
    const int k = blockIdx.x;
    time_row(w, tv[k], emb, tf, tproj + (size_t)k * 768);
}

extern "C" int gp_head_time_proj(const gp_head_weights* w, const float* t, int nt, float* tproj,
                                 hipStream_t stream) {
    GP_REQUIRE(w && t && tproj && nt >= 0, "head_time_proj: bad arguments");
    if (!nt) return GP_OK;
    hipLaunchKernelGGL(time_proj_kernel, dim3(nt), dim3(HT), 0, stream, *w, t, tproj);
    return gp_check_launch("time_proj_kernel");
}

template <int MODE, int PL>
__global__ __launch_bounds__(EVAL_WV * 64) void head_eval_kernel(gp_head_weights w, const float* __restrict__ pobj,
                                                       const float* __restrict__ tproj, float sigma,
                                                       const float* __restrict__ x, int rows, int kper,
                                                       float* __restrict__ out) {
    __shared__ HeadSmem<1, EVAL_WV, PL> sm;
    constexpr bool SPLIT = PL != 0;
    __shared__ int obj[16];
    const int r0 = blockIdx.x * 16;
    SplitScalars hs = {};
    if constexpr (SPLIT) hs = load_split_scalars(w);
    stage_small_weights<1, EVAL_WV, 0, !SPLIT>(w, sm);
    for (int i = threadIdx.x; i < 256; i += EVAL_WV * 64) {
        const int c = i >> 4, j = i & 15;
        const int r = r0 + c;
        sm.xin[i] = (r < rows && j < 9) ? x[(size_t)r * 9 + j] : 0.f;
    }
    if (threadIdx.x < 16) {
        const int r = r0 + threadIdx.x;
        obj[threadIdx.x] = (r < rows ? r : rows - 1) / kper;
    }
    if constexpr (SPLIT)
        head_trunk_x3<1, EVAL_WV>(w, pobj, tproj, obj, sm, 0, hs);
    else
        head_trunk<1, EVAL_WV>(w, pobj, tproj, obj, sm);
    if (MODE == 0) {
        if (threadIdx.x < 144) {
            const int c = threadIdx.x / 9, o = threadIdx.x - c * 9;
            if (r0 + c < rows) out[(size_t)(r0 + c) * 9 + o] = fdiv(head_out(sm, c, o), fadd(sigma, 1e-7f));
        }
    } else {
        if (threadIdx.x < 32) {
            const int c = threadIdx.x >> 1, part = threadIdx.x & 1;
            if (r0 + c < rows) {
                float p[9];
#pragma unroll
                for (int o = 0; o < 9; ++o) p[o] = fmul(sm.xin[c * 16 + o], fdiv(head_out(sm, c, o), sigma));
                const float e = part ? fadd(fadd(p[6], p[7]), p[8])
                                     : fadd(fadd(fadd(fadd(fadd(p[0], p[4]), p[5]), p[1]), p[2]), p[3]);
                out[(size_t)(r0 + c) * 2 + part] = e;
            }
        }
    }
}

extern "C" int gp_score_eval(const gp_head_weights* w, const float* pobj, const float* tproj_row, float sigma,
                             const float* x, int rows, int k, float* score, hipStream_t stream) {
    GP_REQUIRE(w && pobj && tproj_row && x && score && rows >= 0 && k >= 1, "score_eval: bad arguments");
    if (!rows) return GP_OK;
    if (w->pe2_h)
        hipLaunchKernelGGL((head_eval_kernel<0, X3P>), dim3((rows + 15) / 16), dim3(EVAL_WV * 64), 0, stream, *w, pobj, tproj_row,
                       sigma, x, rows, k, score);
    else
        hipLaunchKernelGGL((head_eval_kernel<0, 0>), dim3((rows + 15) / 16), dim3(EVAL_WV * 64), 0, stream, *w, pobj, tproj_row,
                       sigma, x, rows, k, score);
    return gp_check_launch("head_eval_kernel<score>");
}

template <int PL>
__global__ __launch_bounds__(EVAL_WV * 64) void head_div_eval_kernel(gp_head_weights w, const float* __restrict__ pobj,
                                                       const float* __restrict__ tproj, float sigma,
                                                       const float* __restrict__ x, const float* __restrict__ eps,
                                                       int rows, int kper, float* __restrict__ score,
                                                       float* __restrict__ div) {
    __shared__ HeadSmem<2, EVAL_WV, PL> sm;
    constexpr bool SPLIT = PL != 0;
    __shared__ int obj[32];
    const int r0 = blockIdx.x * 16;
    SplitScalars hs = {};
    if constexpr (SPLIT) hs = load_split_scalars(w);
    stage_small_weights<2, EVAL_WV, 0, !SPLIT>(w, sm);
    for (int i = threadIdx.x; i < 512; i += EVAL_WV * 64) {
        const int c = i >> 4, j = i & 15;
        const int r = r0 + (c & 15);
        const float* src = c < 16 ? x : eps;
        sm.xin[i] = (r < rows && j < 9) ? src[(size_t)r * 9 + j] : 0.f;
    }
    if (threadIdx.x < 32) {
        const int r = r0 + (threadIdx.x & 15);
        obj[threadIdx.x] = (r < rows ? r : rows - 1) / kper;
    }
    if constexpr (SPLIT)
        head_trunk_x3<2, EVAL_WV, false, true>(w, pobj, tproj, obj, sm, 0, hs);
    else
        head_trunk<2, EVAL_WV, true>(w, pobj, tproj, obj, sm);
    if (threadIdx.x < 160) {
        const int c = threadIdx.x / 10, o = threadIdx.x - c * 10;
        if (r0 + c < rows) {
            const float den = fadd(sigma, 1e-7f);
            if (o < 9) {
                score[(size_t)(r0 + c) * 9 + o] = fdiv(head_out(sm, c, o), den);
            } else {
                float d = 0.f;
#pragma unroll
                for (int j = 0; j < 9; ++j) d = fadd(d, fmul(ld1(&sm.xin[(16 + c) * 16 + j]), fdiv(head_out_tan(sm, 16 + c, j), den)));
                div[r0 + c] = d;
            }
        }
    }
}

extern "C" int gp_score_div_eval(const gp_head_weights* w, const float* pobj, const float* tproj_row, float sigma,
                                 const float* x, const float* eps, int rows, int k, float* score, float* div,
                                 hipStream_t stream) {
    GP_REQUIRE(w && pobj && tproj_row && x && eps && score && div && rows >= 0 && k >= 1, "score_div_eval: bad arguments");
    if (!rows) return GP_OK;
    if (w->pe2_h)
        hipLaunchKernelGGL((head_div_eval_kernel<X3P>), dim3((rows + 15) / 16), dim3(EVAL_WV * 64), 0, stream, *w, pobj,
                           tproj_row, sigma, x, eps, rows, k, score, div);
    else
        hipLaunchKernelGGL((head_div_eval_kernel<0>), dim3((rows + 15) / 16), dim3(EVAL_WV * 64), 0, stream, *w, pobj,
                           tproj_row, sigma, x, eps, rows, k, score, div);
    return gp_check_launch("head_div_eval_kernel");
}

extern "C" int gp_energy_eval(const gp_head_weights* w, const float* pobj, const float* tproj_row, float sigma,
                              const float* pose, int rows, int k, float* energy, hipStream_t stream) {
    GP_REQUIRE(w && pobj && tproj_row && pose && energy && rows >= 0 && k >= 1, "energy_eval: bad arguments");
    if (!rows) return GP_OK;
    if (w->pe2_h)
        hipLaunchKernelGGL((head_eval_kernel<1, X3P>), dim3((rows + 15) / 16), dim3(EVAL_WV * 64), 0, stream, *w, pobj, tproj_row,
                       sigma, pose, rows, k, energy);
    else
        hipLaunchKernelGGL((head_eval_kernel<1, 0>), dim3((rows + 15) / 16), dim3(EVAL_WV * 64), 0, stream, *w, pobj, tproj_row,
                       sigma, pose, rows, k, energy);
    return gp_check_launch("head_eval_kernel<energy>");
}

__global__ __launch_bounds__(EVAL_WV * 64) void head_grad_eval_kernel(gp_head_weights w, gp_head_grad_weights gw,
                                                       const float* __restrict__ pobj,
                                                       const float* __restrict__ tproj, float sigma,
                                                       const float* __restrict__ x, int rows, int kper,
                                                       float* __restrict__ score, float* __restrict__ energy) {
    __shared__ HeadSmem<1, EVAL_WV, 0> sm;
    __shared__ GradSmem gs;
    __shared__ int obj[16];
    const int r0 = blockIdx.x * 16;
    stage_small_weights<1, EVAL_WV, 0, true>(w, sm);
    for (int i = threadIdx.x; i < 256; i += EVAL_WV * 64) {
        const int c = i >> 4, j = i & 15;
        const int r = r0 + c;
        sm.xin[i] = (r < rows && j < 9) ? x[(size_t)r * 9 + j] : 0.f;
    }
    if (threadIdx.x < 16) {
        const int r = r0 + threadIdx.x;
        obj[threadIdx.x] = (r < rows ? r : rows - 1) / kper;
    }
    head_trunk<1, EVAL_WV, false, true>(w, pobj, tproj, obj, sm, 0, &gs, sigma);
    head_backward<EVAL_WV>(gw, sm, gs);
    if (threadIdx.x < 144) {
        const int c = threadIdx.x / 9, o = threadIdx.x - c * 9;
        float f = fdiv(head_out(sm, c, o), sigma);
        asm volatile("" : "+v"(f));
        if (r0 + c < rows) score[(size_t)(r0 + c) * 9 + o] = fadd(f, pose_grad<EVAL_WV>(gs, c, o));
        sm.scratch[c * 9 + o] = fmul(ld1(&sm.xin[c * 16 + o]), f);
    }
    if (energy != nullptr) {
        __syncthreads();
        if (threadIdx.x < 16 && r0 + (int)threadIdx.x < rows) {
            float e = 0.f;
#pragma unroll
            for (int j = 0; j < 9; ++j) e = fadd(e, ld1(&sm.scratch[threadIdx.x * 9 + j]));
            energy[r0 + threadIdx.x] = e;
        }
    }
}

extern "C" size_t gp_head_grad_floats(void) { return (size_t)16 * HID + (size_t)HID * HID + (size_t)HID * 3 * HID; }

static bool grad_weights_ok(const gp_head_grad_weights* gw) { return gw && gw->pe0_wt && gw->pe2_wt && gw->h1p_wt; }

extern "C" int gp_energy_score_eval(const gp_head_weights* w, const gp_head_grad_weights* gw, const float* pobj,
                                    const float* tproj_row, float sigma, const float* x, int rows, int k,
                                    float* score, float* energy, hipStream_t stream) {
    GP_REQUIRE(w && grad_weights_ok(gw) && pobj && tproj_row && x && score && rows >= 0 && k >= 1 && sigma > 0.f,
               "energy_score_eval: bad arguments");
    if (!rows) return GP_OK;
    hipLaunchKernelGGL(head_grad_eval_kernel, dim3((rows + 15) / 16), dim3(EVAL_WV * 64), 0, stream, *w, *gw, pobj,
                       tproj_row, sigma, x, rows, k, score, energy);
    return gp_check_launch("head_grad_eval_kernel");
}

struct PCStep {
    float t, sigma, g, dt, sqrt_dt;
};

struct PCArgs {
    gp_head_weights w;
    const float* pobj;
    const float* tproj;
    float* x;
    float* s;
    float* part;
    int part_n, part_off;
    int norm_rows;
    int row_off;
    float* zbuf;
    const float* z1;
    const float* z2;
    uint64_t seed;
    const float* center;
    float* res;
    float* q;
    float* xs;
    int rows, kper, steps, nwg;
    float ls_coef;
};
struct PCArgsGrad : PCArgs {
    gp_head_grad_weights gw;
};

template <int NT, int WV, int PL>
__device__ __forceinline__ void pc_update_rows(const PCArgs& a, int i, const PCStep& prev, HeadSmem<NT, WV, PL>& sm,
                                               int* obj, int g, int lane, int r0, float gacc, float (&x3)[3],
                                               const float (&sv)[3], const float (&z1v)[3], const float (&z2v)[3],
                                               const SplitScalars& hs, bool store_x, int trace_slot) {
#pragma clang fp contract(off)
    constexpr bool SPLIT = PL != 0;
    const int p = lane & 3;
    const int e0 = 3 * (p < 3 ? p : 0);
    if (lane < 16) {
        const int r = r0 + 16 * g + lane;
        obj[16 * g + lane] = (r < a.rows ? r : a.rows - 1) / a.kper;
    }
    PC_MARK(10);
    gacc = wave_sum(gacc);
    PC_MARK(11);
    const int c = 16 * g + (lane >> 2);
    const int r = r0 + c;
    const bool upd = i > 0 && r < a.rows && p < 3;
    if (upd) {
        const float gn = udiv(gacc, (float)a.norm_rows);
        const float ratio = udiv(a.ls_coef, gn);
        const float ls = 2.0f * (ratio * ratio);
        const float sq2ls = usqrt(2.0f * ls);
        float mean[3];
#pragma unroll
        for (int k = 0; k < 3; ++k) x3[k] = (x3[k] + ls * sv[k]) + sq2ls * z1v[k];
        if (p < 2) {
            const float nn = usqrt((x3[0] * x3[0] + x3[1] * x3[1]) + x3[2] * x3[2]);
            x3[0] = udiv(x3[0], nn); x3[1] = udiv(x3[1], nn); x3[2] = udiv(x3[2], nn);
        }
        const float g2 = prev.g * prev.g;
        const float gs = prev.g * prev.sqrt_dt;
#pragma unroll
        for (int k = 0; k < 3; ++k) {
            const float drift = 0.0f - g2 * sv[k];
            mean[k] = x3[k] + drift * prev.dt;
            x3[k] = mean[k] + gs * z2v[k];
        }
        gram_schmidt6_quad(x3, p, lane);
        float cen[3] = {0.f, 0.f, 0.f};
        if (a.xs || i == a.steps) {
            const float* cp = a.center + (size_t)(r / a.kper) * 3;
            cen[0] = ld1(cp);
            cen[1] = ld1(cp + 1);
            cen[2] = ld1(cp + 2);
        }
        if (a.xs) {
            float* o = a.xs + ((size_t)r * a.steps + (i - 1)) * 9 + e0;
#pragma unroll
            for (int k = 0; k < 3; ++k) o[k] = p == 2 ? x3[k] + cen[k] : x3[k];
        }
        if (i == a.steps) {
            if (p == 2) {
                mean[0] += cen[0];
                mean[1] += cen[1];
                mean[2] += cen[2];
            }
            gram_schmidt6_quad(mean, p, lane);
#pragma unroll
            for (int k = 0; k < 3; ++k) {
                a.res[(size_t)r * 9 + e0 + k] = mean[k];
                sm.xu[c * 9 + e0 + k] = mean[k];
            }
        }
        if (store_x || i == a.steps) {
#pragma unroll
            for (int k = 0; k < 3; ++k) a.x[(size_t)r * 9 + e0 + k] = x3[k];
        }
    }
    if (i == a.steps) {
        wave_sync();
        if (p == 0 && r < a.rows) {
            float m9[9], qq[4];
#pragma unroll
            for (int j = 0; j < 9; ++j) m9[j] = sm.xu[c * 9 + j];
            quat_from_gs<float>(m9, qq);
#pragma unroll
            for (int j = 0; j < 4; ++j) a.q[(size_t)r * 7 + j] = qq[j];
            a.q[(size_t)r * 7 + 4] = m9[6];
            a.q[(size_t)r * 7 + 5] = m9[7];
            a.q[(size_t)r * 7 + 6] = m9[8];
        }
    }
    if (p < 3) {
#pragma unroll
        for (int k = 0; k < 3; ++k) sm.xin[c * 16 + e0 + k] = (r < a.rows) ? x3[k] : 0.f;
    } else {
#pragma unroll
        for (int j = 9; j < 16; ++j) sm.xin[c * 16 + j] = 0.f;
    }
    if constexpr (SPLIT) {
        float m = (p < 3 && r < a.rows) ? fmaxf(fmaxf(fabsf(x3[0]), fabsf(x3[1])), fabsf(x3[2])) : 0.f;
        m = fmaxf(m, __int_as_float(__builtin_amdgcn_mov_dpp(__float_as_int(m), 0xB1, 0xF, 0xF, true)));
        m = fmaxf(m, __int_as_float(__builtin_amdgcn_mov_dpp(__float_as_int(m), 0x4E, 0xF, 0xF, true)));
        if (p == 0) {
            const ColScales cs = split_col_scales(m, hs);
            sm.cscl[c][0] = f32x4{cs.s1, cs.s2, cs.u2, cs.uh};
            sm.cscl[c][1] = f32x4{cs.sh, 0.f, 0.f, 0.f};
        }
    }
}

template <int NT, int WV, typename Dst>
__device__ __forceinline__ void pc_make_draws(const PCArgs& a, int i, int r0, Dst dst) {
    constexpr int ROWS = NT * 16;
    for (int e = tid_x() - 64 * NT; e < ROWS * 6; e += (WV - NT) * 64) {
        const int c = e / 6, st = (e - c * 6) / 3, blk = e - c * 6 - st * 3;
        const int r = r0 + c;
        if (r < a.rows) {
            const f32x4 v = philox_normal4(a.seed, (uint32_t)(st + 2 * i), (uint32_t)(a.row_off + r), (uint32_t)blk);
            dst(st, c, blk * 4 + 0, v.x);
            if (blk < 2) {
                dst(st, c, blk * 4 + 1, v.y);
                dst(st, c, blk * 4 + 2, v.z);
                dst(st, c, blk * 4 + 3, v.w);
            }
        }
    }
}

template <int NT, int WV, int PL, typename Put>
__device__ __forceinline__ float pc_score_norm(const PCArgs& a, const PCStep& cur, HeadSmem<NT, WV, PL>& sm, int r0,
                                               int wid, int lane, Put put) {
    constexpr int ROWS = NT * 16;
    const float den = fadd(cur.sigma, 1e-7f);
    float wsum = 0.f;
    for (int cg = wid; cg < ROWS / 4; cg += WV) {
        const int c = 4 * cg + (lane >> 4), o = lane & 15;
        const int r = r0 + c;
        float v = 0.f;
        if (o < 9 && r < a.rows) {
            v = fdiv(head_out(sm, c, o), den);
            put(c, o, v);
        }
        wsum += rows_sum(sqrtf(row16_sum(fmul(v, v))));
    }
    if (lane == 0) sm.scratch[wid] = wsum;
    __syncthreads();
    float t = 0.f;
    if (wid == 0 && lane == 0) {
#pragma unroll
        for (int v = 0; v < WV; ++v) t += sm.scratch[v];
    }
    return t;
}

template <int WV, typename Put>
__device__ __forceinline__ float pc_energy_score_norm(const PCArgs& a, const PCStep& cur, HeadSmem<1, WV, 0>& sm,
                                                      const GradSmem& gs, int r0, int wid, int lane, Put put) {
    float wsum = 0.f;
    for (int cg = wid; cg < 4; cg += WV) {
        const int c = 4 * cg + (lane >> 4), o = lane & 15;
        const int r = r0 + c;
        float v = 0.f;
        if (o < 9 && r < a.rows) {
            float f = fdiv(head_out(sm, c, o), cur.sigma);
            asm volatile("" : "+v"(f));
            v = fadd(f, pose_grad<WV>(gs, c, o));
            put(c, o, v);
        }
        wsum += rows_sum(sqrtf(row16_sum(fmul(v, v))));
    }
    if (lane == 0) sm.scratch[wid] = wsum;
    __syncthreads();
    float t = 0.f;
    if (wid == 0 && lane == 0) {
#pragma unroll
        for (int v = 0; v < WV; ++v) t += sm.scratch[v];
    }
    return t;
}

template <int NT, int WV, int PL, bool GRAD = false>
__global__ __launch_bounds__(WV * 64) void pc_step_kernel(std::conditional_t<GRAD, PCArgsGrad, PCArgs> a, int i,
                                                          PCStep cur, PCStep prev) {
    constexpr int ROWS = NT * 16;
    static_assert(NT < WV, "at least one wave besides the update waves");
    static_assert(!GRAD || (NT == 1 && PL == 0), "the energy gradient runs the exact-fp32 16-candidate tile");
    __shared__ HeadSmem<NT, WV, PL> sm;
    constexpr bool SPLIT = PL != 0;
    __shared__ int obj[ROWS];
    const int tid = threadIdx.x;
    const int lane = tid & 63;
    const int wid = __builtin_amdgcn_readfirstlane(tid >> 6);
    const int r0 = blockIdx.x * ROWS;
    const int trace_slot = i == a.steps ? 2 : (i & 1);
    SplitScalars hs = {};
    if constexpr (SPLIT) hs = load_split_scalars<WV>(a.w);
    PC_MARK(0);
    if (wid < NT) {
        const int g = wid;
        const bool inj = a.z1 != nullptr;
        const float* zslot = a.zbuf + (size_t)((i - 1) & 1) * 2 * a.rows * 9;
        const float* z1p = inj ? a.z1 + ((size_t)(i > 0 ? i - 1 : 0) * a.rows) * 9 : zslot;
        const float* z2p = inj ? a.z2 + ((size_t)(i > 0 ? i - 1 : 0) * a.rows) * 9 : zslot + (size_t)a.rows * 9;
        const float* part = a.part + (size_t)((i - 1) & 1) * a.part_n;
        float pv[8];
#pragma unroll
        for (int u = 0; u < 8; ++u) pv[u] = part[min(lane + 64 * u, a.part_n - 1)];
        const int p = lane & 3;
        const int e0 = 3 * (p < 3 ? p : 0);
        float x3[3], sv[3], z1v[3], z2v[3];
        {
            const size_t e = (size_t)min(r0 + 16 * g + (lane >> 2), a.rows - 1) * 9 + e0;
#pragma unroll
            for (int k = 0; k < 3; ++k) {
                x3[k] = ld1(a.x + e + k);
                sv[k] = ld1(a.s + e + k);
                z1v[k] = ld1(z1p + e + k);
                z2v[k] = ld1(z2p + e + k);
            }
        }
        float gacc = 0.f;
#pragma unroll
        for (int u = 0; u < 8; ++u) gacc += lane + 64 * u < a.part_n ? pv[u] : 0.f;
        for (int t0 = 512; t0 < a.part_n; t0 += 512) {
#pragma unroll
            for (int u = 0; u < 8; ++u) pv[u] = part[min(t0 + lane + 64 * u, a.part_n - 1)];
#pragma unroll
            for (int u = 0; u < 8; ++u) gacc += t0 + lane + 64 * u < a.part_n ? pv[u] : 0.f;
        }
        PC_MARK(9);
        pc_update_rows<NT, WV, PL>(a, i, prev, sm, obj, g, lane, r0, gacc, x3, sv, z1v, z2v, hs, true, trace_slot);
        PC_MARK(12);
    }
    if (i == a.steps) return;
    if (wid >= NT && a.z1 == nullptr)
        pc_make_draws<NT, WV>(a, i, r0, [&](int st, int c, int e, float v) {
            a.zbuf[((size_t)((i & 1) * 2 + st) * a.rows + r0 + c) * 9 + e] = v;
        });
    stage_small_weights<NT, WV, 64 * NT, !SPLIT>(a.w, sm);
    if constexpr (GRAD) {
        __shared__ GradSmem gs;
        head_trunk<NT, WV, false, true>(a.w, a.pobj, a.tproj + (size_t)i * 768, obj, sm, trace_slot, &gs, cur.sigma);
        head_backward<WV>(a.gw, sm, gs, trace_slot);
        PC_MARK(7);
        const float t = pc_energy_score_norm<WV>(a, cur, sm, gs, r0, wid, lane,
                                                 [&](int c, int o, float v) { a.s[(size_t)(r0 + c) * 9 + o] = v; });
        if (tid == 0) a.part[(size_t)(i & 1) * a.part_n + a.part_off + blockIdx.x] = t;
        PC_MARK(8);
    } else {
        if constexpr (SPLIT)
            head_trunk_x3<NT, WV, true>(a.w, a.pobj, a.tproj + (size_t)i * 768, obj, sm, trace_slot, hs);
        else
            head_trunk<NT, WV>(a.w, a.pobj, a.tproj + (size_t)i * 768, obj, sm, trace_slot);
        PC_MARK(7);
        const float t = pc_score_norm<NT, WV, PL>(a, cur, sm, r0, wid, lane,
                                                  [&](int c, int o, float v) { a.s[(size_t)(r0 + c) * 9 + o] = v; });
        if (tid == 0) a.part[(size_t)(i & 1) * a.part_n + a.part_off + blockIdx.x] = t;
        PC_MARK(8);
    }
}

__global__ void randn_kernel(uint64_t seed, uint32_t stream, int rows, int cols, float* __restrict__ out) {
    const int nb = (cols + 3) >> 2;
    const long long e = (long long)blockIdx.x * blockDim.x + threadIdx.x;
    if (e >= (long long)rows * nb) return;
    const int r = (int)(e / nb), blk = (int)(e - (long long)r * nb);
    const f32x4 v = philox_normal4(seed, stream, (uint32_t)r, (uint32_t)blk);
    const float vv[4] = {v.x, v.y, v.z, v.w};
#pragma unroll
    for (int k = 0; k < 4; ++k)
        if (4 * blk + k < cols) out[(size_t)r * cols + 4 * blk + k] = vv[k];
}

extern "C" int gp_randn(uint64_t seed, uint32_t stream, int rows, int cols, float* out, hipStream_t hs) {
    GP_REQUIRE(rows >= 0 && cols >= 1 && (out || rows == 0), "randn: bad arguments");
    if (!rows) return GP_OK;
    const long long n = (long long)rows * ((cols + 3) >> 2);
    hipLaunchKernelGGL(randn_kernel, dim3((unsigned)((n + 255) / 256)), dim3(256), 0, hs, seed, stream, rows, cols, out);
    return gp_check_launch("randn_kernel");
}

extern "C" size_t gp_pc_workspace_size(int rows) {
    const size_t ntiles = ((size_t)rows + 15) / 16;
    return sizeof(float) * ((size_t)rows * 9 * 5 + 2 * ntiles) + 256;
}

extern "C" int gp_pc_tile_rows(int rows, int split) { return 16 * head_pick_nt(rows, split != 0); }

extern "C" int gp_pc_step_table(int steps, float eps, float* out) {
    GP_REQUIRE(out && steps >= 2, "pc_step_table: need steps >= 2 and an output of steps x 5 floats");
    const float start = 1.0f, end = eps;
    const float step = (end - start) / (float)(steps - 1);
    const int half = steps / 2;
    const float diff_scale = (float)sqrt(2.0 * (log(50.0) - log(0.01)));
    float t0 = 0.f, t1 = 0.f;
    for (int i = 0; i < steps; ++i) {
        const float t = i < half ? fmaf(step, (float)i, start) : fmaf(-step, (float)(steps - 1 - i), end);
        if (i == 0) t0 = t;
        if (i == 1) t1 = t;
        out[5 * i] = t;
    }
    const float dt = t0 - t1, sdt = sqrtf(t0 - t1);
    for (int i = 0; i < steps; ++i) {
        const float t = out[5 * i];
        const float sig = 0.01f * (float)pow(5000.0, (double)t);
        out[5 * i + 1] = sig;
        out[5 * i + 2] = sig * diff_scale;
        out[5 * i + 3] = dt;
        out[5 * i + 4] = sdt;
    }
    return GP_OK;
}

static int pc_sample_impl(const gp_head_weights* w, const float* pobj, const float* tproj, const float* step_tab,
                          int steps, float* x, int rows, int k, const float* pts_center, const float* z1,
                          const float* z2, uint64_t seed, float snr, float* res, float* q, float* xs, void* workspace,
                          size_t workspace_bytes, int nt, float* part, int part_n, int part_off, int norm_rows,
                          int row_off, gp_pc_exchange_fn exchange, void* ctx, hipStream_t stream,
                          const gp_head_grad_weights* gw = nullptr) {
    GP_REQUIRE(w && pobj && tproj && step_tab && x && pts_center && res && q && workspace,
               "pc_sample: null pointer");
    GP_REQUIRE(steps >= 2 && rows >= 1 && k >= 1, "pc_sample: need steps>=2, rows>=1, k>=1");
    GP_REQUIRE((z1 == nullptr) == (z2 == nullptr), "pc_sample: z1/z2 must both be given or both null");
    GP_REQUIRE(workspace_bytes >= gp_pc_workspace_size(rows), "pc_sample: workspace too small");
    const bool split = w->pe2_h != nullptr;
    GP_REQUIRE(!split || (w->h1p_h && w->hsc), "pc_sample: pe2_h, h1p_h and hsc must be given together");
    PCArgs a;
    a.w = *w;
    a.pobj = pobj;
    a.tproj = tproj;
    a.x = x;
    a.s = static_cast<float*>(workspace);
    a.zbuf = a.s + (size_t)rows * 9 + 2 * (((size_t)rows + 15) / 16);
    a.z1 = z1;
    a.z2 = z2;
    a.seed = seed;
    a.center = pts_center;
    a.res = res;
    a.q = q;
    a.xs = xs;
    a.rows = rows;
    a.kper = k;
    a.steps = steps;
    a.nwg = (rows + 16 * nt - 1) / (16 * nt);
    a.part = part != nullptr ? part : a.s + (size_t)rows * 9;
    a.part_n = part != nullptr ? part_n : a.nwg;
    a.part_off = part != nullptr ? part_off : 0;
    a.norm_rows = norm_rows;
    a.row_off = row_off;
    a.ls_coef = snr * 3.0f;
    GP_REQUIRE(gw == nullptr || nt == 1, "pc_sample_energy: one 16-candidate tile per workgroup");
    GP_REQUIRE(a.part_off >= 0 && a.part_off + a.nwg <= a.part_n, "pc_sample: partials [%d, %d) outside %d entries",
               a.part_off, a.part_off + a.nwg, a.part_n);
    const dim3 grid(a.nwg);
    for (int i = 0; i <= steps; ++i) {
        PCStep cur = {}, prev = {};
        if (i < steps) cur = PCStep{step_tab[5 * i], step_tab[5 * i + 1], step_tab[5 * i + 2], step_tab[5 * i + 3],
                                    step_tab[5 * i + 4]};
        if (i > 0) prev = PCStep{step_tab[5 * (i - 1)], step_tab[5 * (i - 1) + 1], step_tab[5 * (i - 1) + 2],
                                 step_tab[5 * (i - 1) + 3], step_tab[5 * (i - 1) + 4]};
        if (gw != nullptr) {
            PCArgsGrad ag;
            static_cast<PCArgs&>(ag) = a;
            ag.gw = *gw;
            hipLaunchKernelGGL((pc_step_kernel<1, PC_WV1, 0, true>), grid, dim3(PC_WV1 * 64), 0, stream, ag, i, cur, prev);
        }
        else if (nt == 4)
            hipLaunchKernelGGL((pc_step_kernel<4, PC_WV1, X3P>), grid, dim3(PC_WV1 * 64), 0, stream, a, i, cur, prev);
        else if (nt == 2)
            hipLaunchKernelGGL((pc_step_kernel<2, PC_WV1, X3P>), grid, dim3(PC_WV1 * 64), 0, stream, a, i, cur, prev);
        else if (split)
            hipLaunchKernelGGL((pc_step_kernel<1, PC_WV1, X3P>), grid, dim3(PC_WV1 * 64), 0, stream, a, i, cur, prev);
        else
            hipLaunchKernelGGL((pc_step_kernel<1, PC_WV1, 0>), grid, dim3(PC_WV1 * 64), 0, stream, a, i, cur, prev);
        if (exchange != nullptr && i < steps) {
            const int rc = gp_check_launch("pc_step_kernel");
            if (rc) return rc;
            GP_REQUIRE(exchange(ctx, i, a.part + (size_t)(i & 1) * a.part_n, a.part_n, stream) == 0,
                       "pc_sample_global: the partials exchange of step %d failed", i);
        }
    }
    return gp_check_launch("pc_step_kernel");
}

extern "C" int gp_pc_sample(const gp_head_weights* w, const float* pobj, const float* tproj, const float* step_tab,
                            int steps, float* x, int rows, int k, const float* pts_center, const float* z1,
                            const float* z2, uint64_t seed, float snr, float* res, float* q, float* xs,
                            void* workspace, size_t workspace_bytes, hipStream_t stream) {
    GP_REQUIRE(w != nullptr, "pc_sample: null pointer");
    return pc_sample_impl(w, pobj, tproj, step_tab, steps, x, rows, k, pts_center, z1, z2, seed, snr, res, q, xs,
                          workspace, workspace_bytes, head_pick_nt(rows, w->pe2_h != nullptr), nullptr, 0, 0, rows, 0,
                          nullptr, nullptr, stream);
}

extern "C" int gp_pc_sample_energy(const gp_head_weights* w, const gp_head_grad_weights* gw, const float* pobj,
                                   const float* tproj, const float* step_tab, int steps, float* x, int rows, int k,
                                   const float* pts_center, const float* z1, const float* z2, uint64_t seed,
                                   float snr, float* res, float* q, float* xs, void* workspace,
                                   size_t workspace_bytes, hipStream_t stream) {
    GP_REQUIRE(w != nullptr && grad_weights_ok(gw), "pc_sample_energy: null pointer");
    return pc_sample_impl(w, pobj, tproj, step_tab, steps, x, rows, k, pts_center, z1, z2, seed, snr, res, q, xs,
                          workspace, workspace_bytes, 1, nullptr, 0, 0, rows, 0, nullptr, nullptr, stream, gw);
}

extern "C" int gp_pc_global_partials(int rows_total, int shard_rows_max, int shards, int split) {
    if (rows_total < 1 || shard_rows_max < 1 || shards < 1) return 0;
    const int tile = 16 * head_pick_nt(rows_total, split != 0);
    return shards * ((shard_rows_max + tile - 1) / tile);
}

extern "C" int gp_pc_sample_global(const gp_head_weights* w, const float* pobj, const float* tproj,
                                   const float* step_tab, int steps, float* x, int rows, int k,
                                   const float* pts_center, uint64_t seed, float snr, float* res, float* q, float* xs,
                                   int rows_total, int row_off, int shard, int shards, int shard_rows_max,
                                   float* part, gp_pc_exchange_fn exchange, void* ctx, void* workspace,
                                   size_t workspace_bytes, hipStream_t stream) {
    GP_REQUIRE(w && part && exchange, "pc_sample_global: null pointer");
    GP_REQUIRE(shards >= 1 && shard >= 0 && shard < shards && rows >= 1 && rows <= shard_rows_max &&
                   row_off >= 0 && row_off + rows <= rows_total,
               "pc_sample_global: shard %d of %d, rows [%d, %d) of %d (at most %d per shard)", shard, shards, row_off,
               row_off + rows, rows_total, shard_rows_max);
    const int nt = head_pick_nt(rows_total, w->pe2_h != nullptr);
    const int per = (shard_rows_max + 16 * nt - 1) / (16 * nt);
    return pc_sample_impl(w, pobj, tproj, step_tab, steps, x, rows, k, pts_center, nullptr, nullptr, seed, snr, res, q,
                          xs, workspace, workspace_bytes, nt, part, shards * per, shard * per, rows_total, row_off,
                          exchange, ctx, stream);
}

__global__ void pose_epilogue_f64_kernel(double* pose, int rows, int kper, const float* center, double* q) {
    const int r = blockIdx.x * blockDim.x + threadIdx.x;
    if (r >= rows) return;
    double v[9];
    for (int j = 0; j < 9; ++j) v[j] = pose[(size_t)r * 9 + j];
    gram_schmidt6<double>(v);
    const float* c = center + (size_t)(r / kper) * 3;
    v[6] += (double)ld1(c);
    v[7] += (double)ld1(c + 1);
    v[8] += (double)ld1(c + 2);
    double qq[4];
    quat_from_gs<double>(v, qq);
    for (int j = 0; j < 9; ++j) pose[(size_t)r * 9 + j] = v[j];
    for (int j = 0; j < 4; ++j) q[(size_t)r * 7 + j] = qq[j];
    for (int j = 0; j < 3; ++j) q[(size_t)r * 7 + 4 + j] = v[6 + j];
}

extern "C" int gp_pose_epilogue_f64(double* pose, int rows, int k, const float* pts_center, double* q,
                                    hipStream_t stream) {
    GP_REQUIRE(pose && pts_center && q && rows >= 0 && k >= 1, "pose_epilogue_f64: bad arguments");
    if (!rows) return GP_OK;
    hipLaunchKernelGGL(pose_epilogue_f64_kernel, dim3((rows + 255) / 256), dim3(256), 0, stream, pose, rows, k,
                       pts_center, q);
    return gp_check_launch("pose_epilogue_f64_kernel");
}

__global__ __launch_bounds__(HT) void scale_kernel(gp_scale_weights w, const float* __restrict__ axes,
                                                   const float* __restrict__ feat, float* __restrict__ len) {
    __shared__ float emb[180];
    __shared__ float h1[256];
    __shared__ float tot[1280];
    __shared__ float u[256];
    const int b = blockIdx.x, i = threadIdx.x;
    if (i < 90) {
        const int a = i / 10, e = i - a * 10;
        const float v = fmul((float)(1 << e), axes[(size_t)b * 9 + a]);
        emb[i] = sinf(v);
        emb[90 + i] = cosf(v);
    }
    for (int c = i; c < 1024; c += HT) tot[c] = feat[(size_t)b * 1024 + c];
    __syncthreads();
    {
        float acc = 0.f;
        for (int c = 0; c < 180; ++c) acc += w.ae0_w[i * 180 + c] * emb[c];
        h1[i] = fmaxf(acc + w.ae0_b[i], 0.f);
    }
    __syncthreads();
    {
        float acc = 0.f;
        for (int c = 0; c < 256; ++c) acc += w.ae2_w[i * 256 + c] * h1[c];
        tot[1024 + i] = fmaxf(acc + w.ae2_b[i], 0.f);
    }
    __syncthreads();
    {
        float acc = 0.f;
        for (int c = 0; c < 1280; ++c) acc += w.ft0_w[(size_t)i * 1280 + c] * tot[c];
        u[i] = fmaxf(acc + w.ft0_b[i], 0.f);
    }
    __syncthreads();
    if (i < 3) {
        float acc = 0.f;
        for (int c = 0; c < 256; ++c) acc += w.ft2_w[i * 256 + c] * u[c];
        len[(size_t)b * 3 + i] = acc + w.ft2_b[i];
    }
}

extern "C" int gp_scale_forward(const gp_scale_weights* w, const float* axes, const float* pts_feat, int b,
                                float* length, hipStream_t stream) {
    GP_REQUIRE(w && axes && pts_feat && length && b >= 0, "scale_forward: bad arguments");
    if (!b) return GP_OK;
    hipLaunchKernelGGL(scale_kernel, dim3(b), dim3(HT), 0, stream, *w, axes, pts_feat, length);
    return gp_check_launch("scale_kernel");
}
```

genpose2_amd/device.py:

```python
from __future__ import annotations

import ctypes
import os
from typing import Dict, Optional

import numpy as np
import torch

from . import _lib, arch, pack, weights
from ._lib import check


def _ptr(t: Optional[torch.Tensor]) -> Optional[int]:
    return None if t is None else t.data_ptr()


def stream_handle(device: torch.device) -> int:
    return torch.cuda.current_stream(device).cuda_stream


def require_device_tensor(t: torch.Tensor, name: str, dtype=torch.float32) -> torch.Tensor:
    if not isinstance(t, torch.Tensor):
        raise TypeError(f"{name} must be a torch.Tensor")
    if t.device.type != "cuda":
        raise ValueError(f"{name} must live on a HIP device (got {t.device}); the path has no CPU fallback")
    return t.to(dtype).contiguous()


class _Uploaded:
    def __init__(self, arrays: Dict[str, np.ndarray], device: torch.device):
        self.t = {k: torch.from_numpy(np.ascontiguousarray(v)).to(device) for k, v in arrays.items()}

    def ptr(self, k: str) -> int:
        return self.t[k].data_ptr()


class EncoderGeometry:

    def __init__(self, ws: torch.Tensor, event, key, producer=None, gen: int = 0, event0=None):
        self.ws, self.event, self.key = ws, event, key
        self.producer, self.gen = producer, gen
        self.event0 = event0


class EncoderModel:

    def __init__(self, sd: weights.StateDict, device: torch.device):
        self.lib = _lib.load()
        self.device = device
        buf, offs = pack.pack_encoder(sd)
        self.wbuf = torch.from_numpy(buf).to(device)
        self._table = np.ascontiguousarray(offs, np.int64)
        self._ws: Optional[torch.Tensor] = None
        self._gen = 0
        self.geometry_overlap = os.environ.get("GENPOSE2_GEOM_OVERLAP", "1") == "1"
        self._geo_stream: Optional[torch.cuda.Stream] = None
        self._geo_event: Optional[torch.cuda.Event] = None
        self.set_arith(os.environ.get("GENPOSE2_ENC_ARITH", "split_f16"))

    @property
    def table(self) -> np.ndarray:
        return self._table

    def set_table(self, table: np.ndarray) -> None:
        table = np.ascontiguousarray(table, np.int64).reshape(self._table.shape)
        self._table = table
        self.set_arith(self.arith)

    def set_arith(self, arith: str) -> None:
        if arith not in ("split_f16", "f32"):
            raise ValueError(f"unknown encoder arithmetic {arith!r} (split_f16 | f32)")
        t = self._table.copy()
        if arith == "f32":
            t[..., 2] = -1
        self.arith = arith
        self.offsets = np.ascontiguousarray(t.reshape(-1), np.int64)

    def workspace(self, b: int, n: int) -> torch.Tensor:
        need = int(self.lib.gp_encoder_workspace_size(b, n))
        if self._ws is None or self._ws.numel() < need:
            self._ws = torch.empty(need, dtype=torch.uint8, device=self.device)
        return self._ws

    def _after_side_writes(self, cur) -> None:
        if self._geo_event is not None:
            cur.wait_event(self._geo_event)

    @staticmethod
    def _xyz(pts: torch.Tensor) -> torch.Tensor:
        pts = require_device_tensor(pts, "pts")
        if pts.dim() != 3 or pts.shape[2] < 3:
            raise ValueError("pts must be (B, N, 3+)")
        return pts if pts.shape[2] == 3 else pts[..., :3].contiguous()

    def geometry(self, pts: torch.Tensor) -> "EncoderGeometry":
        key = (require_device_tensor(pts, "pts").data_ptr(), tuple(pts.shape[:2]))
        pts = self._xyz(pts)
        B, N, _ = pts.shape
        ws = self.workspace(B, N)
        self._gen += 1
        cur = torch.cuda.current_stream(self.device)
        self._after_side_writes(cur)
        if not self.geometry_overlap:
            check(self.lib.gp_encoder_geometry(ctypes.c_void_p(pts.data_ptr()), B, N, ctypes.c_void_p(ws.data_ptr()),
                                               ws.numel(), ctypes.c_void_p(cur.cuda_stream)), "encoder_geometry")
            ev = torch.cuda.Event()
            ev.record(cur)
            return EncoderGeometry(ws, ev, key, self, self._gen)
        check(self.lib.gp_encoder_geometry_levels(ctypes.c_void_p(pts.data_ptr()), B, N, ctypes.c_void_p(ws.data_ptr()),
                                                  ws.numel(), 0, 1, ctypes.c_void_p(cur.cuda_stream)),
              "encoder_geometry level 0")
        ev0 = torch.cuda.Event()
        ev0.record(cur)
        if self._geo_stream is None:
            self._geo_stream = torch.cuda.Stream(device=self.device)
        side = self._geo_stream
        side.wait_event(ev0)
        check(self.lib.gp_encoder_geometry_levels(ctypes.c_void_p(pts.data_ptr()), B, N, ctypes.c_void_p(ws.data_ptr()),
                                                  ws.numel(), 1, 4, ctypes.c_void_p(side.cuda_stream)),
              "encoder_geometry levels 1-3")
        ws.record_stream(side)
        pts.record_stream(side)
        ev = torch.cuda.Event()
        ev.record(side)
        self._geo_event = ev
        return EncoderGeometry(ws, ev, key, self, self._gen, event0=ev0)

    def forward(self, pts: torch.Tensor, return_workspace: bool = False,
                geometry: Optional["EncoderGeometry"] = None):
        key = (require_device_tensor(pts, "pts").data_ptr(), tuple(pts.shape[:2]))
        pts = self._xyz(pts)
        B, N, _ = pts.shape
        feat = torch.empty((B, arch.PTS_FEAT_DIM), dtype=torch.float32, device=self.device)
        ws = self.workspace(B, N)
        self._after_side_writes(torch.cuda.current_stream(self.device))
        st = ctypes.c_void_p(stream_handle(self.device))
        if geometry is None:
            self._gen += 1
            check(self.lib.gp_encoder_forward(
                ctypes.c_void_p(self.wbuf.data_ptr()), self.offsets.ctypes.data_as(_lib.c_int64_p),
                ctypes.c_void_p(pts.data_ptr()), B, N, ctypes.c_void_p(ws.data_ptr()), ws.numel(),
                ctypes.c_void_p(feat.data_ptr()), st), "encoder_forward")
        else:
            if geometry.key != key:
                raise ValueError("encoder geometry was computed for other points")
            if geometry.producer is not None and geometry.producer._gen != geometry.gen:
                raise ValueError("encoder geometry is stale: its model encoded other points since")
            cur = torch.cuda.current_stream(self.device)
            spans = ((0, 1, geometry.event0), (1, 5, geometry.event)) if geometry.event0 is not None else \
                ((0, 5, geometry.event),)
            for first, last, ev in spans:
                cur.wait_event(ev)
                check(self.lib.gp_encoder_forward_geom_levels(
                    ctypes.c_void_p(self.wbuf.data_ptr()), self.offsets.ctypes.data_as(_lib.c_int64_p),
                    ctypes.c_void_p(pts.data_ptr()), B, N, ctypes.c_void_p(geometry.ws.data_ptr()),
                    ctypes.c_void_p(ws.data_ptr()), ws.numel(), ctypes.c_void_p(feat.data_ptr()), first, last, st),
                    "encoder_forward_geom")
            if geometry.ws is not ws:
                geometry.ws.record_stream(torch.cuda.current_stream(self.device))
        return (feat, ws) if return_workspace else feat

    def levels(self, b: int, n: int, ws: torch.Tensor):
        off = np.zeros(25, np.int64)
        check(self.lib.gp_encoder_workspace_layout(b, n, off.ctypes.data_as(_lib.c_int64_p)))
        out = []
        couts = [arch.level_out_channels(lv) for lv in range(5)]
        for lv in range(5):
            m = arch.NPOINTS[lv] if lv < 4 else 1
            d = {}
            if lv < 4:
                d["fps_idx"] = ws[off[lv * 5]:].view(torch.int32)[: b * m].view(b, m)
                d["new_xyz"] = ws[off[lv * 5 + 1]:].view(torch.float32)[: b * m * 3].view(b, m, 3)
                d["ball_idx"] = [ws[off[lv * 5 + 2 + i]:].view(torch.int32)[: b * m * ns].view(b, m, ns)
                                 for i, ns in enumerate(arch.NSAMPLES[lv])]
            if lv < 4:
                d["features"] = ws[off[lv * 5 + 4]:].view(torch.float32)[: b * m * couts[lv]].view(b, m, couts[lv])
            out.append(d)
        return out


class HeadModel:

    def __init__(self, sd: weights.StateDict, device: torch.device):
        self.lib = _lib.load()
        self.device = device
        self.up = _Uploaded(pack.pack_heads(sd), device)
        self.set_arith(os.environ.get("GENPOSE2_HEAD_ARITH", "f16x3"))
        self._pc_ws: Optional[torch.Tensor] = None
        self._gw = None

    def weights_changed(self) -> None:
        self._gw = None

    @property
    def grad_weights(self) -> "_lib.HeadGradWeights":
        if self._gw is None:
            src = [self.up.t[k] for k in ("pe0_w", "pe2_w", "h1p_w")]
            bufs = {}
            for name, t, n_out, k_in in zip(pack.HEAD_GRAD_FIELDS, src, (arch.POSE_HID, arch.POSE_HID, 3 * arch.HEAD_HID),
                                            (16, arch.POSE_HID, arch.POSE_HID)):
                w = t.view(n_out // 16, k_in // 16, 4, 16, 4).permute(0, 3, 1, 2, 4).reshape(n_out, k_in)
                bufs[name] = w.t().reshape(k_in // 16, 16, n_out // 16, 4, 4).permute(0, 2, 3, 1, 4).contiguous().view(-1)
            self._gw = (bufs, _lib.HeadGradWeights(**{k: v.data_ptr() for k, v in bufs.items()}))
        return self._gw[1]

    def set_arith(self, arith: str) -> None:
        if arith not in ("f16x3", "f32"):
            raise ValueError(f"unknown head arithmetic {arith!r} (f16x3 | f32)")
        ptrs = {k: self.up.ptr(k) for k in pack.HEAD_FIELDS}
        if arith == "f32":
            ptrs.update(pe2_h=None, h1p_h=None, hsc=None)
        self.arith = arith
        self.w = _lib.HeadWeights(**ptrs)

    def _s(self):
        return ctypes.c_void_p(stream_handle(self.device))

    def object_proj(self, feat: torch.Tensor) -> torch.Tensor:
        feat = require_device_tensor(feat, "pts_feat")
        B = feat.shape[0]
        pobj = torch.empty((B, 3 * arch.HEAD_HID), dtype=torch.float32, device=self.device)
        check(self.lib.gp_head_object_proj(ctypes.byref(self.w), ctypes.c_void_p(feat.data_ptr()), B,
                                           ctypes.c_void_p(pobj.data_ptr()), self._s()), "head_object_proj")
        return pobj

    def time_proj(self, t: torch.Tensor) -> torch.Tensor:
        t = require_device_tensor(t.reshape(-1), "t")
        out = torch.empty((t.numel(), 3 * arch.HEAD_HID), dtype=torch.float32, device=self.device)
        check(self.lib.gp_head_time_proj(ctypes.byref(self.w), ctypes.c_void_p(t.data_ptr()), t.numel(),
                                         ctypes.c_void_p(out.data_ptr()), self._s()), "head_time_proj")
        return out

    def score(self, pobj, tproj_row, sigma: float, x: torch.Tensor, k: int, out=None) -> torch.Tensor:
        x = require_device_tensor(x, "x")
        R = x.shape[0]
        out = torch.empty((R, arch.POSE_DIM), dtype=torch.float32, device=self.device) if out is None else out
        check(self.lib.gp_score_eval(ctypes.byref(self.w), ctypes.c_void_p(pobj.data_ptr()),
                                     ctypes.c_void_p(tproj_row.data_ptr()), ctypes.c_float(sigma),
                                     ctypes.c_void_p(x.data_ptr()), R, k, ctypes.c_void_p(out.data_ptr()),
                                     self._s()), "score_eval")
        return out

    def score_div(self, pobj, tproj_row, sigma: float, x: torch.Tensor, eps: torch.Tensor, k: int):
        x = require_device_tensor(x, "x")
        eps = require_device_tensor(eps, "eps")
        R = x.shape[0]
        if tuple(eps.shape) != (R, arch.POSE_DIM):
            raise ValueError(f"eps must be ({R}, {arch.POSE_DIM}), got {tuple(eps.shape)}")
        score = torch.empty((R, arch.POSE_DIM), dtype=torch.float32, device=self.device)
        div = torch.empty((R,), dtype=torch.float32, device=self.device)
        check(self.lib.gp_score_div_eval(ctypes.byref(self.w), ctypes.c_void_p(pobj.data_ptr()),
                                         ctypes.c_void_p(tproj_row.data_ptr()), ctypes.c_float(sigma),
                                         ctypes.c_void_p(x.data_ptr()), ctypes.c_void_p(eps.data_ptr()), R, k,
                                         ctypes.c_void_p(score.data_ptr()), ctypes.c_void_p(div.data_ptr()),
                                         self._s()), "score_div_eval")
        return score, div

    def energy(self, pobj, tproj_row, sigma: float, pose: torch.Tensor, k: int) -> torch.Tensor:
        pose = require_device_tensor(pose, "pose")
        R = pose.shape[0]
        out = torch.empty((R, 2), dtype=torch.float32, device=self.device)
        check(self.lib.gp_energy_eval(ctypes.byref(self.w), ctypes.c_void_p(pobj.data_ptr()),
                                      ctypes.c_void_p(tproj_row.data_ptr()), ctypes.c_float(sigma),
                                      ctypes.c_void_p(pose.data_ptr()), R, k, ctypes.c_void_p(out.data_ptr()),
                                      self._s()), "energy_eval")
        return out

    def energy_score(self, pobj, tproj_row, sigma: float, x: torch.Tensor, k: int, want_energy: bool = False):
        x = require_device_tensor(x, "x")
        R = x.shape[0]
        score = torch.empty((R, arch.POSE_DIM), dtype=torch.float32, device=self.device)
        energy = torch.empty((R,), dtype=torch.float32, device=self.device) if want_energy else None
        check(self.lib.gp_energy_score_eval(ctypes.byref(self.w), ctypes.byref(self.grad_weights),
                                            ctypes.c_void_p(pobj.data_ptr()), ctypes.c_void_p(tproj_row.data_ptr()),
                                            ctypes.c_float(sigma), ctypes.c_void_p(x.data_ptr()), R, k,
                                            ctypes.c_void_p(score.data_ptr()), ctypes.c_void_p(_ptr(energy)),
                                            self._s()), "energy_score_eval")
        return (score, energy) if want_energy else score

    def pc_sample(self, pobj, tproj, step_tab: np.ndarray, x: torch.Tensor, k: int, pts_center: torch.Tensor,
                  z1=None, z2=None, seed: int = 0, snr: float = arch.SNR, want_xs: bool = False, global_batch=None,
                  energy_grad: bool = False):
        if energy_grad and global_batch is not None:
            raise NotImplementedError("the energy-gradient sampler has no global-batch mode")
        R = x.shape[0]
        T = step_tab.shape[0]
        need = int(self.lib.gp_pc_workspace_size(R))
        if self._pc_ws is None or self._pc_ws.numel() < need:
            self._pc_ws = torch.empty(need, dtype=torch.uint8, device=self.device)
        res = torch.empty((R, 9), dtype=torch.float32, device=self.device)
        q = torch.empty((R, 7), dtype=torch.float32, device=self.device)
        xs = torch.empty((R, T, 9), dtype=torch.float32, device=self.device) if want_xs else None
        tab = np.ascontiguousarray(step_tab, np.float32)
        if global_batch is not None:
            from .shard import PartialsExchange
            gb = global_batch
            if z1 is not None or z2 is not None:
                raise ValueError("global-batch sampling draws its noise on the device (z1 / z2 not supported)")
            rows_total, rows_max = gb.total * k, gb.per_max * k
            if R != (gb.hi - gb.lo) * k:
                raise ValueError(f"global-batch shard: {R} rows for objects [{gb.lo}, {gb.hi}) x {k}")
            n = int(self.lib.gp_pc_global_partials(rows_total, rows_max, gb.world, int(self.w.pe2_h is not None)))
            part = torch.zeros(2 * n, dtype=torch.float32, device=self.device)
            ex = PartialsExchange(part, n, gb)
            rc = self.lib.gp_pc_sample_global(
                ctypes.byref(self.w), ctypes.c_void_p(pobj.data_ptr()), ctypes.c_void_p(tproj.data_ptr()),
                tab.ctypes.data_as(ctypes.c_void_p), T, ctypes.c_void_p(x.data_ptr()), R, k,
                ctypes.c_void_p(pts_center.data_ptr()), ctypes.c_uint64(seed), ctypes.c_float(snr),
                ctypes.c_void_p(res.data_ptr()), ctypes.c_void_p(q.data_ptr()), ctypes.c_void_p(_ptr(xs)),
                rows_total, gb.lo * k, gb.rank, gb.world, rows_max, ctypes.c_void_p(part.data_ptr()), ex.fn, None,
                ctypes.c_void_p(self._pc_ws.data_ptr()), self._pc_ws.numel(), self._s())
            if ex.error is not None:
                raise RuntimeError("pc_sample_global: partials exchange failed") from ex.error
            check(rc, "pc_sample_global")
            return res, q, xs
        if energy_grad:
            check(self.lib.gp_pc_sample_energy(
                ctypes.byref(self.w), ctypes.byref(self.grad_weights), ctypes.c_void_p(pobj.data_ptr()),
                ctypes.c_void_p(tproj.data_ptr()), tab.ctypes.data_as(ctypes.c_void_p), T,
                ctypes.c_void_p(x.data_ptr()), R, k, ctypes.c_void_p(pts_center.data_ptr()),
                ctypes.c_void_p(_ptr(z1)), ctypes.c_void_p(_ptr(z2)), ctypes.c_uint64(seed), ctypes.c_float(snr),
                ctypes.c_void_p(res.data_ptr()), ctypes.c_void_p(q.data_ptr()), ctypes.c_void_p(_ptr(xs)),
                ctypes.c_void_p(self._pc_ws.data_ptr()), self._pc_ws.numel(), self._s()), "pc_sample_energy")
            return res, q, xs
        check(self.lib.gp_pc_sample(
            ctypes.byref(self.w), ctypes.c_void_p(pobj.data_ptr()), ctypes.c_void_p(tproj.data_ptr()),
            tab.ctypes.data_as(ctypes.c_void_p), T, ctypes.c_void_p(x.data_ptr()), R, k,
            ctypes.c_void_p(pts_center.data_ptr()), ctypes.c_void_p(_ptr(z1)), ctypes.c_void_p(_ptr(z2)),
            ctypes.c_uint64(seed), ctypes.c_float(snr), ctypes.c_void_p(res.data_ptr()),
            ctypes.c_void_p(q.data_ptr()), ctypes.c_void_p(_ptr(xs)), ctypes.c_void_p(self._pc_ws.data_ptr()),
            self._pc_ws.numel(), self._s()), "pc_sample")
        return res, q, xs


    def ode_denoise(self, pobj, t32: float, sigma: float, g2: float, step: float, x: torch.Tensor, k: int,
                    pts_center: torch.Tensor, ws: torch.Tensor):
        R = x.numel() // arch.POSE_DIM
        pose = torch.empty((R, arch.POSE_DIM), dtype=torch.float64, device=self.device)
        q = torch.empty((R, 7), dtype=torch.float64, device=self.device)
        check(self.lib.gp_ode_denoise(
            ctypes.byref(self.w), ctypes.c_void_p(pobj.data_ptr()), t32, sigma, g2, step,
            ctypes.c_void_p(x.data_ptr()), R, k, ctypes.c_void_p(require_device_tensor(pts_center, "pts_center").data_ptr()),
            ctypes.c_void_p(pose.data_ptr()), ctypes.c_void_p(q.data_ptr()), ctypes.c_void_p(ws.data_ptr()),
            ws.numel(), self._s()), "ode_denoise")
        return pose, q


class ScaleModel:
    def __init__(self, sd: weights.StateDict, device: torch.device):
        self.lib = _lib.load()
        self.device = device
        self.up = _Uploaded(pack.pack_scale(sd), device)
        self.w = _lib.ScaleWeights(**{k: self.up.ptr(k) for k in pack.SCALE_FIELDS})

    def forward(self, axes: torch.Tensor, pts_feat: torch.Tensor) -> torch.Tensor:
        axes = require_device_tensor(axes, "axes")
        pts_feat = require_device_tensor(pts_feat, "pts_feat")
        B = axes.shape[0]
        out = torch.empty((B, 3), dtype=torch.float32, device=self.device)
        check(self.lib.gp_scale_forward(ctypes.byref(self.w), ctypes.c_void_p(axes.data_ptr()),
                                        ctypes.c_void_p(pts_feat.data_ptr()), B, ctypes.c_void_p(out.data_ptr()),
                                        ctypes.c_void_p(stream_handle(self.device))), "scale_forward")
        return out


def pose_epilogue_f64(pose: torch.Tensor, k: int, pts_center: torch.Tensor):
    lib = _lib.load()
    pose = pose.contiguous()
    q = torch.empty((pose.shape[0], 7), dtype=torch.float64, device=pose.device)
    check(lib.gp_pose_epilogue_f64(ctypes.c_void_p(pose.data_ptr()), pose.shape[0], k,
                                   ctypes.c_void_p(require_device_tensor(pts_center, "pts_center").data_ptr()),
                                   ctypes.c_void_p(q.data_ptr()), ctypes.c_void_p(stream_handle(pose.device))),
          "pose_epilogue_f64")
    return pose, q


def points_mean(pts: torch.Tensor) -> torch.Tensor:
    pts = require_device_tensor(pts, "pts")
    B, N, C = pts.shape
    out = torch.empty((B, 3), dtype=torch.float32, device=pts.device)
    check(_lib.load().gp_points_mean(ctypes.c_void_p(pts.data_ptr()), B, N, C, ctypes.c_void_p(out.data_ptr()),
                                     ctypes.c_void_p(stream_handle(pts.device))), "points_mean")
    return out


def bbox_length(pcl: torch.Tensor, pose: torch.Tensor) -> torch.Tensor:
    pcl = require_device_tensor(pcl, "pcl")
    pose = require_device_tensor(pose, "pose")
    B, N, C = pcl.shape
    if pose.shape != (B, 4, 4):
        raise ValueError(f"pose must be ({B},4,4), got {tuple(pose.shape)}")
    out = torch.empty((B, 3), dtype=torch.float32, device=pcl.device)
    check(_lib.load().gp_bbox_length(ctypes.c_void_p(pcl.data_ptr()), B, N, C, ctypes.c_void_p(pose.data_ptr()),
                                     ctypes.c_void_p(out.data_ptr()), ctypes.c_void_p(stream_handle(pcl.device))),
          "bbox_length")
    return out


def randn(seed: int, stream: int, rows: int, cols: int, device) -> torch.Tensor:
    lib = _lib.load()
    out = torch.empty((rows, cols), dtype=torch.float32, device=device)
    check(lib.gp_randn(ctypes.c_uint64(seed), ctypes.c_uint32(stream), rows, cols, ctypes.c_void_p(out.data_ptr()),
                       ctypes.c_void_p(stream_handle(out.device))), "randn")
    return out
```

genpose2_amd/pack.py:

```python
from __future__ import annotations

from typing import Dict, List, Optional, Tuple

import numpy as np

from . import arch, weights


def pad16(v: int) -> int:
    return (v + 15) // 16 * 16


def pack_a_fragments(w: np.ndarray, k_pad: Optional[int] = None, n_pad: Optional[int] = None) -> np.ndarray:
    n_out, k_in = w.shape
    NP = pad16(n_out) if n_pad is None else n_pad
    KP = pad16(k_in) if k_pad is None else k_pad
    wp = np.zeros((NP, KP), np.float32)
    wp[:n_out, :k_in] = w
    NT, KG = NP // 16, KP // 16
    t = wp.reshape(NT, 16, KG, 4, 4)
    return np.ascontiguousarray(t.transpose(0, 2, 3, 1, 4)).reshape(-1)


def unpack_a_fragments(p: np.ndarray, n_pad: int, k_pad: int) -> np.ndarray:
    t = p.reshape(n_pad // 16, k_pad // 16, 4, 16, 4).transpose(0, 3, 1, 2, 4)
    return t.reshape(n_pad, k_pad)


def pad_vec(b: np.ndarray, n: int) -> np.ndarray:
    out = np.zeros(n, np.float32)
    out[: b.shape[0]] = b
    return out


ENC_SPLIT_LEVELS = (1, 2, 3, 4)


def enc_split_layer(lv: int, i: int) -> bool:
    return lv in ENC_SPLIT_LEVELS or i >= 1


def pad32(v: int) -> int:
    return (v + 31) // 32 * 32


def pack_encoder(sd: weights.StateDict, levels=None) -> Tuple[np.ndarray, np.ndarray]:
    levels = arch.sa_branches() if levels is None else levels
    folded = weights.encoder_layers(sd, levels)
    chunks: List[np.ndarray] = []
    offsets = np.full((5, 2, 3, 4), -1, np.int64)
    pos = 0

    def add(a: np.ndarray) -> int:
        nonlocal pos
        o = pos
        a = np.ascontiguousarray(a).reshape(-1)
        if a.dtype != np.float32:
            a = a.view(np.float32)
        chunks.append(a)
        pos += a.size
        padn = (-pos) % 4
        if padn:
            chunks.append(np.zeros(padn, np.float32))
            pos += padn
        return o

    for lv, branches in enumerate(levels):
        c_prev = branches[0].widths[0] - 3
        for br in branches:
            for i, (W, b) in enumerate(folded[lv][br.branch]):
                if i == 0:
                    wp = np.zeros((W.shape[0], c_prev + 16), np.float32)
                    wp[:, :c_prev] = W[:, 3:]
                    wp[:, c_prev:c_prev + 3] = W[:, :3]
                    packed = pack_a_fragments(wp, k_pad=c_prev + 16)
                else:
                    packed = pack_a_fragments(W)
                offsets[lv, br.branch, i, 0] = add(packed)
                offsets[lv, br.branch, i, 1] = add(pad_vec(b, pad32(W.shape[0])))
                if enc_split_layer(lv, i):
                    if i == 0:
                        wq = np.zeros((pad32(W.shape[0]), pad32(c_prev + 3)), np.float32)
                        wq[:W.shape[0], :c_prev] = W[:, 3:]
                        wq[:W.shape[0], c_prev:c_prev + 3] = W[:, :3]
                    else:
                        wq = np.zeros((pad32(W.shape[0]), pad32(W.shape[1])), np.float32)
                        wq[:W.shape[0], :W.shape[1]] = W
                    e = split_exponent(W)
                    offsets[lv, br.branch, i, 2] = add(pack_h16_fragments(wq, e))
                    offsets[lv, br.branch, i, 3] = e
    return np.concatenate(chunks), offsets


HEAD_FIELDS = ("pe0_w", "pe0_b", "pe2_w", "pe2_b", "h1p_w", "h2_w", "h2_b", "h1pts_t", "h1_b",
               "gfp_w", "te_w_t", "te_b", "h1t_t", "pe2_h", "h1p_h", "hsc")


def split_exponent(w: np.ndarray) -> int:
    m = float(np.abs(w).max())
    return 14 - int(np.floor(np.log2(m))) if m > 0 else 0


def pack_h16_fragments(w: np.ndarray, e: int, planes: int = 2) -> np.ndarray:
    n_out, k_in = w.shape
    assert n_out % 16 == 0 and k_in % 32 == 0, (n_out, k_in)
    assert planes in (2, 3), planes
    r = (np.asarray(w, np.float32) * np.float32(2.0 ** e)).astype(np.float32)
    ps = []
    for _ in range(planes):
        h = r.astype(np.float16)
        ps.append(h)
        r = (r - h.astype(np.float32)).astype(np.float32)
    NT, KC = n_out // 16, k_in // 32

    def frag(p):
        return p.reshape(NT, 16, KC, 2, 4, 4).transpose(0, 2, 4, 1, 3, 5)
    out = np.stack([frag(p) for p in ps], axis=2)
    return np.ascontiguousarray(out).reshape(-1).view(np.int32)


HEAD_PLANES = 3


def split_constants(p: Dict[str, np.ndarray], e2: int, eh: int) -> np.ndarray:
    a0 = np.abs(p["pe0_w"].astype(np.float64)).sum(1).max()
    a2 = np.abs(p["pe2_w"].astype(np.float64)).sum(1).max()
    b0, b2 = np.abs(p["pe0_b"]).max(), np.abs(p["pe2_b"]).max()
    return np.nextafter(np.array([a0, b0, a2, b2], np.float32), np.float32(np.inf)).tolist() + [e2, eh, 0, 0]


def pack_heads(sd: weights.StateDict) -> Dict[str, np.ndarray]:
    p = weights.head_params(sd)
    H = arch.HEAD_HID
    out = {
        "pe0_w": pack_a_fragments(p["pe0_w"], k_pad=16),
        "pe0_b": p["pe0_b"],
        "pe2_w": pack_a_fragments(p["pe2_w"]),
        "pe2_b": p["pe2_b"],
        "h1p_w": pack_a_fragments(p["h1_pose"].reshape(3 * H, arch.POSE_HID)),
        "h2_w": p["h2_w"].reshape(-1),
        "h2_b": p["h2_b"].reshape(-1),
        "h1pts_t": np.ascontiguousarray(p["h1_pts"].reshape(3 * H, arch.PTS_FEAT_DIM).T),
        "h1_b": p["h1_b"].reshape(-1),
        "gfp_w": p["gfp_w"],
        "te_w_t": np.ascontiguousarray(p["te_w"].T),
        "te_b": p["te_b"],
        "h1t_t": np.ascontiguousarray(p["h1_t"].reshape(3 * H, arch.T_EMB).T),
    }
    out = {k: np.ascontiguousarray(v, np.float32) for k, v in out.items()}
    h1_pose = p["h1_pose"].reshape(3 * H, arch.POSE_HID)
    e2, eh = split_exponent(p["pe2_w"]), split_exponent(h1_pose)
    out["pe2_h"] = pack_h16_fragments(p["pe2_w"], e2, HEAD_PLANES)
    out["h1p_h"] = pack_h16_fragments(h1_pose, eh, HEAD_PLANES)
    out["hsc"] = np.asarray(split_constants(p, e2, eh), np.float32)
    return out


HEAD_GRAD_FIELDS = ("pe0_wt", "pe2_wt", "h1p_wt")


def pack_heads_grad(sd: weights.StateDict) -> Dict[str, np.ndarray]:
    p = weights.head_params(sd)
    h1_pose = p["h1_pose"].reshape(3 * arch.HEAD_HID, arch.POSE_HID)
    out = {
        "pe0_wt": pack_a_fragments(np.ascontiguousarray(p["pe0_w"].T), n_pad=16),
        "pe2_wt": pack_a_fragments(np.ascontiguousarray(p["pe2_w"].T)),
        "h1p_wt": pack_a_fragments(np.ascontiguousarray(h1_pose.T)),
    }
    return {k: np.ascontiguousarray(v, np.float32) for k, v in out.items()}


SCALE_FIELDS = ("ae0_w", "ae0_b", "ae2_w", "ae2_b", "ft0_w", "ft0_b", "ft2_w", "ft2_b")


def pack_scale(sd: weights.StateDict) -> Dict[str, np.ndarray]:
    m = {"ae0": "axes_encoder.0", "ae2": "axes_encoder.2", "ft0": "fusion_tail_length.0",
         "ft2": "fusion_tail_length.2"}
    out = {}
    for short, key in m.items():
        out[f"{short}_w"] = np.ascontiguousarray(sd[f"{key}.weight"], np.float32)
        out[f"{short}_b"] = np.ascontiguousarray(sd[f"{key}.bias"], np.float32)
    return out
```

include/genpose_hip.h:

```cpp
#ifndef GENPOSE_HIP_H
#define GENPOSE_HIP_H

#include <stddef.h>
#include <stdint.h>
#include <hip/hip_runtime_api.h>

#ifdef __cplusplus
extern "C" {
#endif

enum { GP_OK = 0, GP_ERR_INVALID = -1, GP_ERR_LAUNCH = -2, GP_ERR_UNSUPPORTED = -3 };

const char *gp_last_error(void);
int gp_abi_version(void);
#define GP_ABI_VERSION 7


int gp_furthest_point_sampling(int b, int n, int m, const float *xyz, float *temp, int *idx,
                               hipStream_t stream);

int gp_gather_points(int b, int c, int n, int npoints, const float *points, const int *idx,
                     float *out, hipStream_t stream);

int gp_ball_query(int b, int n, int m, float radius, int nsample, const float *new_xyz,
                  const float *xyz, int *idx, hipStream_t stream);

int gp_group_points(int b, int c, int n, int npoints, int nsample, const float *points,
                    const int *idx, float *out, hipStream_t stream);

size_t gp_encoder_workspace_size(int b, int n);
int gp_encoder_workspace_layout(int b, int n, int64_t *offsets);
int gp_encoder_forward(const float *wbuf, const int64_t *layer_off, const float *pts, int b, int n,
                       void *workspace, size_t workspace_bytes, float *feat, hipStream_t stream);
int gp_encoder_geometry(const float *pts, int b, int n, void *workspace, size_t workspace_bytes,
                        hipStream_t stream);
int gp_encoder_forward_geom(const float *wbuf, const int64_t *layer_off, const float *pts, int b, int n,
                            const void *geometry, void *workspace, size_t workspace_bytes, float *feat,
                            hipStream_t stream);
int gp_encoder_geometry_levels(const float *pts, int b, int n, void *workspace, size_t workspace_bytes,
                               int first, int last, hipStream_t stream);
int gp_encoder_forward_geom_levels(const float *wbuf, const int64_t *layer_off, const float *pts, int b, int n,
                                   const void *geometry, void *workspace, size_t workspace_bytes, float *feat,
                                   int first, int last, hipStream_t stream);
int gp_encoder_fps(const float *pts, int b, int n, void *workspace, size_t workspace_bytes,
                   hipStream_t stream);
int gp_sa_level(const float *wbuf, const int64_t *layer_off, int level, int c_prev, const float *pts,
                int b, int n, const float *feat_prev, void *workspace, size_t workspace_bytes,
                float *out, hipStream_t stream);
int gp_sa_level_geom(const float *wbuf, const int64_t *layer_off, int level, int c_prev, const float *pts,
                     int b, int n, const float *feat_prev, const void *geometry, void *workspace,
                     size_t workspace_bytes, float *out, hipStream_t stream);

int gp_linear(const float *x, int ldx, int m, int k, const float *w, const float *bias, int n,
              int act, float *y, int ldy, hipStream_t stream);
#define GP_LINEAR_RMAX_GIVEN 1
size_t gp_linear_split_words(int n, int k);
int gp_linear_split(const float *x, int ldx, int m, int k, const int32_t *wpk, const float *bias, int n,
                    int act, float *y, int ldy, float *rmax, int flags, float *ymax, hipStream_t stream);
int gp_add_layernorm(const float *x, const float *r, int m, int d, const float *gamma,
                     const float *beta, float eps, float *y, float *ymax, hipStream_t stream);
size_t gp_relpe_bias_bytes(int b, int n);
int gp_relpe_bias(const float *pe, const float *xyz, int b, int n, float *bias, hipStream_t stream);
int gp_mha_attention(const float *qkv, const float *bias, int b, int n, int d, float *out,
                     float *ymax, hipStream_t stream);
int gp_mha_relpe_attention(const float *qkv, const float *xyz, const float *pe, int b, int n, int d,
                           float *out, float *ymax, hipStream_t stream);
int gp_interp_points(const float *x, int b, int n_in, int c, int n_out, float *y, float *ymax,
                     hipStream_t stream);
size_t gp_fusion_attend_workspace_size(int b, int n, int c);
int gp_fusion_attend(const float *cur, const float *ot, int b, int n, int c, const float *ca1_w,
                     const float *ca1_b, const float *ca3_w, const float *ca3_b, const float *sp_w,
                     float *gcat, float *gmax, void *ws, size_t ws_bytes, hipStream_t stream);
int gp_fusion_mix(const float *g, const float *gcat, int rows, int c, float *out, hipStream_t stream);

typedef struct {
    const float *pe0_w;
    const float *pe0_b;
    const float *pe2_w;
    const float *pe2_b;
    const float *h1p_w;
    const float *h2_w;
    const float *h2_b;
    const float *h1pts_t;
    const float *h1_b;
    const float *gfp_w;
    const float *te_w_t;
    const float *te_b;
    const float *h1t_t;
    const void *pe2_h;
    const void *h1p_h;
    const float *hsc;
} gp_head_weights;

int gp_head_object_proj(const gp_head_weights *w, const float *pts_feat, int b, float *pobj,
                        hipStream_t stream);
int gp_head_time_proj(const gp_head_weights *w, const float *t, int nt, float *tproj,
                      hipStream_t stream);

int gp_score_eval(const gp_head_weights *w, const float *pobj, const float *tproj_row,
                  float sigma, const float *x, int rows, int k, float *score, hipStream_t stream);

int gp_score_div_eval(const gp_head_weights *w, const float *pobj, const float *tproj_row,
                      float sigma, const float *x, const float *eps, int rows, int k, float *score,
                      float *div, hipStream_t stream);

int gp_energy_eval(const gp_head_weights *w, const float *pobj, const float *tproj_row,
                   float sigma, const float *pose, int rows, int k, float *energy,
                   hipStream_t stream);

typedef struct {
    const float *pe0_wt;
    const float *pe2_wt;
    const float *h1p_wt;
} gp_head_grad_weights;
size_t gp_head_grad_floats(void);
int gp_head_grad_pack(const float *pe0_w, const float *pe2_w, const float *h1_pose, float *out);
int gp_energy_score_eval(const gp_head_weights *w, const gp_head_grad_weights *gw, const float *pobj,
                         const float *tproj_row, float sigma, const float *x, int rows, int k,
                         float *score, float *energy, hipStream_t stream);

size_t gp_pc_workspace_size(int rows);
int gp_pc_tile_rows(int rows, int split);
int gp_pc_sample(const gp_head_weights *w, const float *pobj, const float *tproj,
                 const float *step_tab, int steps, float *x, int rows, int k,
                 const float *pts_center, const float *z1, const float *z2, uint64_t seed,
                 float snr, float *res, float *q, float *xs, void *workspace,
                 size_t workspace_bytes, hipStream_t stream);
int gp_pc_sample_energy(const gp_head_weights *w, const gp_head_grad_weights *gw, const float *pobj,
                        const float *tproj, const float *step_tab, int steps, float *x, int rows, int k,
                        const float *pts_center, const float *z1, const float *z2, uint64_t seed,
                        float snr, float *res, float *q, float *xs, void *workspace,
                        size_t workspace_bytes, hipStream_t stream);

typedef int (*gp_pc_exchange_fn)(void *ctx, int step, float *slot, int n, hipStream_t stream);
int gp_pc_global_partials(int rows_total, int shard_rows_max, int shards, int split);
int gp_pc_sample_global(const gp_head_weights *w, const float *pobj, const float *tproj,
                        const float *step_tab, int steps, float *x, int rows, int k,
                        const float *pts_center, uint64_t seed, float snr, float *res, float *q,
                        float *xs, int rows_total, int row_off, int shard, int shards,
                        int shard_rows_max, float *part, gp_pc_exchange_fn exchange, void *ctx,
                        void *workspace, size_t workspace_bytes, hipStream_t stream);

int gp_pc_step_table(int steps, float eps, float *out);

int gp_randn(uint64_t seed, uint32_t stream, int rows, int cols, float *out, hipStream_t hs);

int gp_pose_epilogue_f64(double *pose, int rows, int k, const float *pts_center, double *q,
                         hipStream_t stream);

size_t gp_ode_workspace_size(int rows);
int gp_ode_rhs(const gp_head_weights *w, const float *pobj, float t32, float sigma, double coef,
               const double *y, const double *const *kin, const double *acoef, int nk, double h,
               int rows, int k, double *kout, void *workspace, size_t workspace_bytes,
               hipStream_t stream);
int gp_ode_attempt(const gp_head_weights *w, const float *pobj, const float *t32_6,
                   const float *sigma_6, const double *coef_6, const double *y,
                   double *const *kslots, const double *tableau_a, const double *b, const double *e,
                   double h, double rtol, double atol, int rows, int k, double *ynew, double *err_out,
                   void *workspace, size_t workspace_bytes, hipStream_t stream);
int gp_ode_init_norms(const double *y0, const double *f0, const double *f1, long long n,
                      double atol, double rtol, double *out, hipStream_t stream);
size_t gp_like_workspace_size(int rows);
int gp_like_rhs(const gp_head_weights *w, const float *pobj, float t32, float sigma, double coef,
                const double *y, const float *eps, const double *const *kin, const double *acoef,
                int nk, double h, int rows, int k, double *kout, void *workspace,
                size_t workspace_bytes, hipStream_t stream);
int gp_like_attempt(const gp_head_weights *w, const float *pobj, const float *t32_6,
                    const float *sigma_6, const double *coef_6, const double *y, const float *eps,
                    double *const *kslots, const double *tableau_a, const double *b, const double *e,
                    double h, double rtol, double atol, int rows, int k, double *ynew,
                    double *err_out, void *workspace, size_t workspace_bytes, hipStream_t stream);
int gp_ode_dense(const double *const *kslots, const double *P7x4, const double *y_old,
                 const double *t_eval, int i0, int i1, int i_base, int reverse, double t_old,
                 double h, long long n, double *out, hipStream_t stream);
size_t gp_ode_ctl_size(void);
size_t gp_ode_auto_workspace_size(int rows);
int gp_ode_auto_attempt(const gp_head_weights *w, const float *pobj, int n, int what,
                        double t_bound, double direction, double rtol, double atol,
                        double sig_min, double base, double diff_scale, double *y0, double *y1,
                        double *const *kslots, const double *tableau_a, const double *b,
                        const double *e, int rows, int k, void *workspace, size_t workspace_bytes,
                        hipStream_t stream);
int gp_ode_auto_attempt_hs(const gp_head_weights *w, const float *pobj, int n, int what,
                           double t_bound, double direction, double rtol, double atol,
                           double sig_min, double base, double diff_scale, double *y0, double *y1,
                           double *const *kslots, const double *tableau_a, const double *b,
                           const double *e, int rows, int k, void *workspace, size_t workspace_bytes,
                           int *host_status, hipStream_t stream);
typedef int (*gp_ode_exchange_fn)(void *ctx, int attempt, double *part, int n, hipStream_t stream);
int gp_ode_global_partials(int rows_total, int shard_rows_max, int shards, int split);
size_t gp_ode_global_workspace_size(int part_n);
size_t gp_ode_auto_partials_offset(void);
int gp_ode_auto_attempt_global(const gp_head_weights *w, const float *pobj, int n, int what,
                               double t_bound, double direction, double rtol, double atol,
                               double sig_min, double base, double diff_scale, double *y0, double *y1,
                               double *const *kslots, const double *tableau_a, const double *b,
                               const double *e, int rows, int k, int rows_total, int row_off, int shard,
                               int shards, int shard_rows_max, gp_ode_exchange_fn exchange, void *ctx,
                               void *workspace, size_t workspace_bytes, int *host_status,
                               hipStream_t stream);
size_t gp_ode_sample_workspace_size(int rows);
int gp_ode_sample(const gp_head_weights *w, const float *pobj, const float *x0, int rows, int k,
                  double T0, double eps, int steps, double rtol, double atol,
                  const float *pts_center, double *pose, double *q, int *nfev, int *status,
                  void *workspace, size_t workspace_bytes, hipStream_t stream);
int gp_ode_denoise(const gp_head_weights *w, const float *pobj, float t32, float sigma, float g2,
                   float step, const double *x, int rows, int k, const float *pts_center,
                   double *pose, double *q, void *workspace, size_t workspace_bytes,
                   hipStream_t stream);

size_t gp_img_encoder_workspace_size(int b, int np, int d);
int gp_img_encoder(const float *l0, const float *l1, const float *l2, int b, int np, int d,
                   const float *la_w1, const float *la_b1, const float *la_w2, float la_b2,
                   const float *geo_table, const float *conv_w, const float *conv_b, float geo_gate,
                   float edge_gate, float *out, float *layer_w, float *edge_out, void *workspace,
                   size_t workspace_bytes, hipStream_t stream);
int gp_img_encoder2(const float *l0, const float *l1, const float *l2, int b, int np, int d,
                    const float *la_w1, const float *la_b1, const float *la_w2, float la_b2,
                    const float *geo_table, const float *conv_w, const float *conv_b, float geo_gate,
                    float edge_gate, const int32_t *la_w1_h, const int32_t *conv_w_h, float *out,
                    float *layer_w, float *edge_out, void *workspace, size_t workspace_bytes,
                    hipStream_t stream);
size_t gp_img_encoder3_workspace_size(int b, int np, int d, int split_conv);
int gp_img_encoder3(const float *l0, const float *l1, const float *l2, int b, int np, int d,
                    const float *la_w1, const float *la_b1, const float *la_w2, float la_b2,
                    const float *geo_table, const float *conv_w, const float *conv_b, float geo_gate,
                    float edge_gate, const int32_t *la_w1_h, const int32_t *conv_w_hp, float *out,
                    float *layer_w, float *edge_out, void *workspace, size_t workspace_bytes,
                    hipStream_t stream);
int gp_img_geo_table(const float *rel_pos_emb, int num_emb, int edim, int grid, float *table);
int gp_gather_patch_points(const float *feat, int b, int np, int d, const int *xs, const int *ys, int n,
                           int patch_px, int grid, float *out, hipStream_t stream);

typedef struct {
    const float *ae0_w;
    const float *ae0_b;
    const float *ae2_w;
    const float *ae2_b;
    const float *ft0_w;
    const float *ft0_b;
    const float *ft2_w;
    const float *ft2_b;
} gp_scale_weights;
int gp_scale_forward(const gp_scale_weights *w, const float *axes, const float *pts_feat, int b,
                     float *length, hipStream_t stream);

int gp_rank_aggregate(const float *poses, const float *energy, int b, int k, int retain,
                      int clustering, float eps, int min_samples, float *aggregated,
                      float *sorted_pose, float *sorted_energy, hipStream_t stream);

int gp_points_mean(const float *pts, int b, int n, int c, float *out, hipStream_t stream);
int gp_bbox_length(const float *pcl, int b, int n, int c, const float *pose, float *length,
                   hipStream_t stream);

enum { GP_MODEL_SCORE = 0, GP_MODEL_ENERGY = 1, GP_MODEL_SCALE = 2 };
enum { GP_PACK_ENC = 0, GP_PACK_HEADS = 1, GP_PACK_SCALE = 17, GP_PACK_NFIELDS = 25 };
typedef struct gp_weights gp_weights;
int gp_weights_pack(int kind, int n, const char *const *names, const float *const *data,
                    const int64_t *numel, gp_weights **out);
void gp_weights_free(gp_weights *w);
const gp_head_weights *gp_weights_heads(const gp_weights *w);
const gp_scale_weights *gp_weights_scale(const gp_weights *w);
const float *gp_weights_encoder(const gp_weights *w, const int64_t **layer_off);
int gp_weights_pack_host(int kind, int n, const char *const *names, const float *const *data,
                         const int64_t *numel, float *out, size_t out_floats, size_t *need_floats,
                         int64_t *fields, int64_t *enc_table);

#ifdef __cplusplus
}
#endif
#endif
```

Baseline: 261.0 million pose-candidate-steps/s.

## Replace small f16x3 cross products with scaled FP8 MFMA in head GEMMs

Adds a hybrid precision form for the pose_encoder.2 and head-1 GEMMs. Three of the five f16 correction products are replaced by one scaled FP8 (e4m3) 16x16x128 MFMA over pre-quantized weight planes with fixed per-plane exponents. Activations are split into two f16 planes plus three packed FP8 planes in LDS. The goal is to cut MFMA issue count and B-plane traffic in the correction chain. By default ('auto') it is used for score eval and PC steps at the 4-tile width, and in exchange it adds LDS footprint, new weight buffers and a precision risk in the lowest-order terms.

New measurement: 267.6 million pose-candidate-steps/s, median of 6. 2.5% higher.

```diff
diff --git a/genpose2_amd/_lib.py b/genpose2_amd/_lib.py
--- a/genpose2_amd/_lib.py
+++ b/genpose2_amd/_lib.py
@@ -20,7 +20,7 @@
 class HeadWeights(ctypes.Structure):
     _fields_ = [(n, c_void_p) for n in ("pe0_w", "pe0_b", "pe2_w", "pe2_b", "h1p_w", "h2_w", "h2_b",
                                        "h1pts_t", "h1_b", "gfp_w", "te_w_t", "te_b", "h1t_t", "pe2_h", "h1p_h",
-                                       "hsc")]
+                                       "hsc", "pe2_q", "h1p_q")] + [("q8_flags", c_size_t)]
 
 
 class HeadGradWeights(ctypes.Structure):
diff --git a/genpose2_amd/csrc/gp_head.h b/genpose2_amd/csrc/gp_head.h
--- a/genpose2_amd/csrc/gp_head.h
+++ b/genpose2_amd/csrc/gp_head.h
@@ -32,7 +32,7 @@
 template <int NT, int WV, int PL = 0>
 struct HeadSmem {
     static constexpr bool kAliasAct = NT >= 4;
-    static constexpr int kAct = PL ? (HID / 32) * NT * PL * 64 : KG_HID * NT * 64;
+    static constexpr int kAct = PL == 4 ? (HID / 32) * NT * 224 : (PL ? (HID / 32) * NT * PL * 64 : KG_HID * NT * 64);
     float xin[NT * 16 * 16];
     f32x4 act1[kAct];
     f32x4 act2[kAliasAct ? 4 : kAct];
@@ -486,6 +486,45 @@
 #endif
 constexpr int X3P = 3;
 
+constexpr int X3Q = 4;
+typedef int i32x8 __attribute__((ext_vector_type(8)));
+typedef unsigned u32x2 __attribute__((ext_vector_type(2)));
+constexpr int Q8_EXP_HI = -7, Q8_EXP_MID = 4, Q8_EXP_LO = 16;
+template <int PL>
+constexpr int act_f16_planes() { return PL == X3Q ? 2 : X3P; }
+template <int PL, int NT>
+__device__ __forceinline__ constexpr int act_plane(int chunk, int ct, int p) {
+    return ((chunk * NT + ct) * act_f16_planes<PL>() + p) * 64;
+}
+template <int NT>
+__device__ __forceinline__ constexpr int act_q8(int group, int ct, int k, int h) {
+    return KC_HID * NT * 2 * 64 + (((group * NT + ct) * 3 + k) * 2 + h) * 64;
+}
+template <int K>
+__device__ __forceinline__ f32x4 mfma_q8(f16x8 a0, f16x8 a1, f16x8 b0, f16x8 b1, f32x4 c) {
+    using u4 = __attribute__((ext_vector_type(4))) int;
+    const u4 x0 = __builtin_bit_cast(u4, a0), x1 = __builtin_bit_cast(u4, a1);
+    const u4 y0 = __builtin_bit_cast(u4, b0), y1 = __builtin_bit_cast(u4, b1);
+    const i32x8 a = {x0[0], x0[1], x0[2], x0[3], x1[0], x1[1], x1[2], x1[3]};
+    const i32x8 b = {y0[0], y0[1], y0[2], y0[3], y1[0], y1[1], y1[2], y1[3]};
+    constexpr int ea = K == 0 ? Q8_EXP_HI : (K == 1 ? Q8_EXP_MID : Q8_EXP_LO);
+    constexpr int eb = K == 0 ? Q8_EXP_LO : (K == 1 ? Q8_EXP_MID : Q8_EXP_HI);
+    return __builtin_amdgcn_mfma_scale_f32_16x16x128_f8f6f4(a, b, c, 0, 0, 0, 127 - ea, 0, 127 - eb);
+}
+__device__ __forceinline__ u32x2 q8_of(f16x8 p, float s) {
+    int lo = 0, hi = 0;
+    lo = __builtin_amdgcn_cvt_pk_fp8_f32((float)p[0] * s, (float)p[1] * s, lo, false);
+    lo = __builtin_amdgcn_cvt_pk_fp8_f32((float)p[2] * s, (float)p[3] * s, lo, true);
+    hi = __builtin_amdgcn_cvt_pk_fp8_f32((float)p[4] * s, (float)p[5] * s, hi, false);
+    hi = __builtin_amdgcn_cvt_pk_fp8_f32((float)p[6] * s, (float)p[7] * s, hi, true);
+    return u32x2{(unsigned)lo, (unsigned)hi};
+}
+template <int PL>
+struct ActPlanes {
+    f16x8 h[act_f16_planes<PL>()];
+    u32x2 q[PL == X3Q ? 3 : 1];
+};
+
 __device__ __forceinline__ void split3(float x, _Float16& h, _Float16& m, _Float16& l) {
 #pragma clang fp contract(off)
     h = (_Float16)x;
@@ -505,23 +544,84 @@
         p[2][j] = l;
     }
 }
-
-template <int G, int GEND, int TT, int NT, int D>
-__device__ __forceinline__ void stream_x3_rec(__amdgpu_buffer_rsrc_t W, const int (&T)[TT], const f16x8* __restrict__ B,
-                                              int lane, int voff, f16x8 (&ring)[D + 1][TT][X3P],
-                                              f32x4 (&acc)[TT][NT], f32x4 (&cor)[TT][NT], f16x8 (&bc)[X3P]) {
+template <int PL>
+__device__ __forceinline__ void split_act(f32x4 u, f32x4 v, float s, ActPlanes<PL>& a) {
+    f16x8 p[X3P];
+    split3_pair(u, v, s, p);
+    a.h[0] = p[0];
+    a.h[1] = p[1];
+    if constexpr (PL == X3Q) {
+        a.q[0] = q8_of(p[2], exp2i(Q8_EXP_LO));
+        a.q[1] = q8_of(p[1], exp2i(Q8_EXP_MID));
+        a.q[2] = q8_of(p[0], exp2i(Q8_EXP_HI));
+    } else {
+        a.h[2] = p[2];
+    }
+}
+template <int PL, int NT>
+__device__ __forceinline__ void store_act(f16x8* act, int chunk, int ct, int lane, const ActPlanes<PL>& a) {
+#pragma unroll
+    for (int p = 0; p < act_f16_planes<PL>(); ++p) act[act_plane<PL, NT>(chunk, ct, p) + lane] = a.h[p];
+    if constexpr (PL == X3Q) {
+        const int cc = chunk & 3;
+#pragma unroll
+        for (int k = 0; k < 3; ++k)
+            reinterpret_cast<u32x2*>(act + act_q8<NT>(chunk >> 2, ct, k, cc >> 1) + lane)[cc & 1] = a.q[k];
+    }
+}
+
+template <int PL>
+constexpr int ring_planes() { return PL == X3Q ? 4 : X3P; }
+template <int PL, int NT>
+__device__ __forceinline__ void load_b_planes(const f16x8* __restrict__ B, int GG, int ct, int lane,
+                                              f16x8 (&b)[ring_planes<PL>()]) {
+#pragma unroll
+    for (int p = 0; p < act_f16_planes<PL>(); ++p) b[p] = B[act_plane<PL, NT>(GG, ct, p) + lane];
+    if constexpr (PL == X3Q) {
+        if ((GG & 3) < 3) {
+            b[2] = B[act_q8<NT>(GG >> 2, ct, GG & 3, 0) + lane];
+            b[3] = B[act_q8<NT>(GG >> 2, ct, GG & 3, 1) + lane];
+        }
+    }
+}
+template <int PL, int KQ>
+__device__ __forceinline__ f32x4 cross_products(const f16x8 (&w)[ring_planes<PL>()], const f16x8 (&b)[ring_planes<PL>()],
+                                                f32x4 c) {
+    if constexpr (PL != X3Q) {
+        c = mfma_h(w[2], b[0], c);
+        c = mfma_h(w[0], b[2], c);
+        c = mfma_h(w[1], b[1], c);
+    }
+    c = mfma_h(w[1], b[0], c);
+    c = mfma_h(w[0], b[1], c);
+    if constexpr (PL == X3Q && KQ < 3) c = mfma_q8<KQ < 3 ? KQ : 0>(w[2], w[3], b[2], b[3], c);
+    return c;
+}
+template <int PL, int G, int GEND, int TT, int NT, int D>
+__device__ __forceinline__ void stream_x3_rec(__amdgpu_buffer_rsrc_t W, __amdgpu_buffer_rsrc_t WQ, const int (&T)[TT],
+                                              const f16x8* __restrict__ B, int lane, int voff,
+                                              f16x8 (&ring)[D + 1][TT][ring_planes<PL>()], f32x4 (&acc)[TT][NT],
+                                              f32x4 (&cor)[TT][NT], f16x8 (&bc)[ring_planes<PL>()]) {
+    constexpr int RP = ring_planes<PL>();
     if constexpr (G < GEND) {
         if constexpr (G < KC_HID && ((X3_DIAG & 2) == 0 || G < D + 1)) {
 #pragma unroll
-            for (int t = 0; t < TT; ++t)
-#pragma unroll
-                for (int p = 0; p < X3P; ++p)
+            for (int t = 0; t < TT; ++t) {
+#pragma unroll
+                for (int p = 0; p < act_f16_planes<PL>(); ++p)
                     ring[G % (D + 1)][t][p] =
                         __builtin_bit_cast(f16x8, ldbuf4(W, voff, ((T[t] * KC_HID + G) * X3P + p) * 1024));
+                if constexpr (PL == X3Q && (G & 3) < 3) {
+#pragma unroll
+                    for (int h = 0; h < 2; ++h)
+                        ring[G % (D + 1)][t][2 + h] = __builtin_bit_cast(
+                            f16x8, ldbuf4(WQ, voff, (((T[t] * (KC_HID / 4) + G / 4) * 3 + (G & 3)) * 2 + h) * 1024));
+                }
+            }
         }
         __builtin_amdgcn_sched_barrier(0);
         if constexpr (G >= D) {
-            constexpr int GG = G - D, S = GG % (D + 1);
+            constexpr int GG = G - D, S = GG % (D + 1), KQ = GG & 3;
 #if X3_PRIO
             if ((__builtin_amdgcn_readfirstlane(threadIdx.x >> 8) ^ GG) & 1)
                 __builtin_amdgcn_s_setprio(1);
@@ -529,89 +629,69 @@
                 __builtin_amdgcn_s_setprio(0);
 #endif
 #if X3_BPIPE
-            if constexpr (GG == 0) {
-#pragma unroll
-                for (int p = 0; p < X3P; ++p) bc[p] = B[p * 64 + lane];
-            }
+            if constexpr (GG == 0) load_b_planes<PL, NT>(B, 0, 0, lane, bc);
 #pragma unroll
             for (int ct = 0; ct < NT; ++ct) {
-                f16x8 bn[X3P];
-                const int nx = ct + 1 < NT ? (GG * NT + ct + 1) : ((GG + 1) * NT);
-                if ((X3_DIAG & 1) == 0 && (ct + 1 < NT || GG + 1 < KC_HID)) {
-#pragma unroll
-                    for (int p = 0; p < X3P; ++p) bn[p] = B[(nx * X3P + p) * 64 + lane];
+                f16x8 bn[RP];
+                const int ng = ct + 1 < NT ? GG : GG + 1, nc = ct + 1 < NT ? ct + 1 : 0;
+                if ((X3_DIAG & 1) == 0 && (ct + 1 < NT || GG + 1 < KC_HID)) load_b_planes<PL, NT>(B, ng, nc, lane, bn);
+#if X3_DIAG & 1
+#pragma unroll
+                for (int p = 0; p < RP; ++p) {
+                    using u4 = __attribute__((ext_vector_type(4))) unsigned;
+                    bn[p] = __builtin_bit_cast(f16x8, __builtin_bit_cast(u4, bc[p]) ^ (unsigned)(ng * NT + nc + 1));
                 }
-#if X3_DIAG & 1
-#pragma unroll
-                for (int p = 0; p < X3P; ++p) {
-                    using u4 = __attribute__((ext_vector_type(4))) unsigned;
-                    bn[p] = __builtin_bit_cast(f16x8, __builtin_bit_cast(u4, bc[p]) ^ (unsigned)(nx + 1));
-                }
 #endif
                 __builtin_amdgcn_sched_barrier(0);
-                const f16x8 b0 = bc[0], b1 = bc[1], b2 = bc[2];
+                f16x8 b[RP];
+#pragma unroll
+                for (int p = 0; p < RP; ++p) b[p] = bc[p];
 #if X3_CHAIN
 #pragma unroll
                 for (int t = 0; t < TT; ++t) {
-                    f32x4 c = cor[t][ct];
-                    c = mfma_h(ring[S][t][2], b0, c);
-                    c = mfma_h(ring[S][t][0], b2, c);
-                    c = mfma_h(ring[S][t][1], b1, c);
-                    c = mfma_h(ring[S][t][1], b0, c);
-                    c = mfma_h(ring[S][t][0], b1, c);
-                    cor[t][ct] = c;
+                    cor[t][ct] = cross_products<PL, KQ>(ring[S][t], b, cor[t][ct]);
                     __builtin_amdgcn_sched_barrier(0);
                 }
 #pragma unroll
-                for (int t = 0; t < TT; ++t) acc[t][ct] = mfma_h(ring[S][t][0], b0, acc[t][ct]);
+                for (int t = 0; t < TT; ++t) acc[t][ct] = mfma_h(ring[S][t][0], b[0], acc[t][ct]);
 #else
 #pragma unroll
                 for (int t = 0; t < TT; ++t) {
-                    f32x4 c = cor[t][ct];
-                    c = mfma_h(ring[S][t][2], b0, c);
-                    c = mfma_h(ring[S][t][0], b2, c);
-                    c = mfma_h(ring[S][t][1], b1, c);
-                    c = mfma_h(ring[S][t][1], b0, c);
-                    c = mfma_h(ring[S][t][0], b1, c);
-                    cor[t][ct] = c;
-                    acc[t][ct] = mfma_h(ring[S][t][0], b0, acc[t][ct]);
+                    cor[t][ct] = cross_products<PL, KQ>(ring[S][t], b, cor[t][ct]);
+                    acc[t][ct] = mfma_h(ring[S][t][0], b[0], acc[t][ct]);
                 }
 #endif
                 __builtin_amdgcn_sched_barrier(0);
                 if (ct + 1 < NT || GG + 1 < KC_HID) {
 #pragma unroll
-                    for (int p = 0; p < X3P; ++p) bc[p] = bn[p];
+                    for (int p = 0; p < RP; ++p) bc[p] = bn[p];
                 }
             }
 #else
 #pragma unroll
             for (int ct = 0; ct < NT; ++ct) {
-                const f16x8 b0 = B[((GG * NT + ct) * X3P + 0) * 64 + lane];
-                const f16x8 b1 = B[((GG * NT + ct) * X3P + 1) * 64 + lane];
-                const f16x8 b2 = B[((GG * NT + ct) * X3P + 2) * 64 + lane];
+                f16x8 b[RP];
+                load_b_planes<PL, NT>(B, GG, ct, lane, b);
 #pragma unroll
                 for (int t = 0; t < TT; ++t) {
-                    f32x4 c = cor[t][ct];
-                    c = mfma_h(ring[S][t][2], b0, c);
-                    c = mfma_h(ring[S][t][0], b2, c);
-                    c = mfma_h(ring[S][t][1], b1, c);
-                    c = mfma_h(ring[S][t][1], b0, c);
-                    c = mfma_h(ring[S][t][0], b1, c);
-                    cor[t][ct] = c;
-                    acc[t][ct] = mfma_h(ring[S][t][0], b0, acc[t][ct]);
+                    cor[t][ct] = cross_products<PL, KQ>(ring[S][t], b, cor[t][ct]);
+                    acc[t][ct] = mfma_h(ring[S][t][0], b[0], acc[t][ct]);
                 }
             }
 #endif
         }
-        stream_x3_rec<G + 1, GEND, TT, NT, D>(W, T, B, lane, voff, ring, acc, cor, bc);
-    }
-}
-template <int G, int GEND, int TT, int NT, int D>
-__device__ __forceinline__ void stream_x3_step(__amdgpu_buffer_rsrc_t W, const int (&T)[TT], const f16x8* __restrict__ B,
-                                               int lane, int voff, f16x8 (&ring)[D + 1][TT][X3P],
+        stream_x3_rec<PL, G + 1, GEND, TT, NT, D>(W, WQ, T, B, lane, voff, ring, acc, cor, bc);
+    }
+}
+struct X3Weights {
+    __amdgpu_buffer_rsrc_t W, WQ;
+};
+template <int PL, int G, int GEND, int TT, int NT, int D>
+__device__ __forceinline__ void stream_x3_step(const X3Weights& w, const int (&T)[TT], const f16x8* __restrict__ B,
+                                               int lane, int voff, f16x8 (&ring)[D + 1][TT][ring_planes<PL>()],
                                                f32x4 (&acc)[TT][NT], f32x4 (&cor)[TT][NT]) {
-    f16x8 bc[X3P];
-    stream_x3_rec<G, GEND, TT, NT, D>(W, T, B, lane, voff, ring, acc, cor, bc);
+    f16x8 bc[ring_planes<PL>()];
+    stream_x3_rec<PL, G, GEND, TT, NT, D>(w.W, w.WQ, T, B, lane, voff, ring, acc, cor, bc);
 }
 
 template <int H, int NT, int TPW, int NP = NT>
@@ -627,13 +707,13 @@
     }
 }
 
-template <int H, int NT, int WV, int TPW, int DH, bool JVP = false>
-__device__ __forceinline__ void head_x3_head(__amdgpu_buffer_rsrc_t WH, const f16x8* __restrict__ act2h,
+template <int H, int NT, int WV, int TPW, int DH, bool JVP = false, int PL = X3P>
+__device__ __forceinline__ void head_x3_head(const X3Weights& WH, const f16x8* __restrict__ act2h,
                                              __amdgpu_buffer_rsrc_t RP, __amdgpu_buffer_rsrc_t RT, const int (&vo)[NT],
-                                             HeadSmem<NT, WV, X3P>& sm, const float (&uh)[NT], const float (&sh)[NT],
-                                             int wid, int lane, f16x8 (&ringh)[DH + 1][TPW][X3P],
+                                             HeadSmem<NT, WV, PL>& sm, const float (&uh)[NT], const float (&sh)[NT],
+                                             int wid, int lane, f16x8 (&ringh)[DH + 1][TPW][ring_planes<PL>()],
                                              f32x4 (&tpv)[TPW], f32x4 (&pov)[TPW][JVP ? NT / 2 : NT],
-                                             float (&pv)[HeadSmem<NT, WV, X3P>::kRedV]) {
+                                             float (&pv)[HeadSmem<NT, WV, PL>::kRedV]) {
     constexpr int NP = JVP ? NT / 2 : NT;
     const int q = lane >> 4, n = lane & 15;
     const int voff = lane * 16;
@@ -653,12 +733,12 @@
             }
             cor[t][ct] = f32x4{0.f, 0.f, 0.f, 0.f};
         }
-    stream_x3_step<DH, KC_HID + DH, TPW, NT, DH>(WH, TH, act2h, lane, voff, ringh, acc, cor);
+    stream_x3_step<PL, DH, KC_HID + DH, TPW, NT, DH>(WH, TH, act2h, lane, voff, ringh, acc, cor);
     if constexpr (H < 2) {
         int TN[TPW];
 #pragma unroll
         for (int t = 0; t < TPW; ++t) TN[t] = TH[t] + 16;
-        stream_x3_step<0, DH, TPW, NT, DH>(WH, TN, act2h, lane, voff, ringh, acc, cor);
+        stream_x3_step<PL, 0, DH, TPW, NT, DH>(WH, TN, act2h, lane, voff, ringh, acc, cor);
         head_x3_init_load<H + 1, NT, TPW, NP>(RP, RT, vo, wid, lane, tpv, pov);
     }
     __builtin_amdgcn_sched_barrier(0);
@@ -711,24 +791,30 @@
     __builtin_amdgcn_sched_barrier(0);
 }
 
-template <int NT, int WV, bool PRE = false, bool JVP = false>
+template <int NT, int WV, bool PRE = false, bool JVP = false, int PL = X3P>
 __device__ __forceinline__ void head_trunk_x3(const gp_head_weights& w, const float* __restrict__ pobj,
                                               const float* __restrict__ tproj, const int* obj_of_col,
-                                              HeadSmem<NT, WV, X3P>& sm, int trace_slot, const SplitScalars hs) {
+                                              HeadSmem<NT, WV, PL>& sm, int trace_slot, const SplitScalars hs) {
+    static_assert(PL == X3P || (PL == X3Q && !JVP), "the hybrid form has no tangent tiles");
     constexpr int TPW = 16 / WV;
     static_assert(TPW % 2 == 0, "the f16x3 trunk pairs a wave's output tiles into 32-deep chunks");
     static_assert(TPW <= 4, "SplitScalars carries at most four pose_encoder.0 tiles per wave");
     constexpr int CPW = TPW / 2;
     constexpr int NP = JVP ? NT / 2 : NT;
     static_assert(!JVP || NT % 2 == 0, "a JVP trunk pairs every primal tile with a tangent tile");
-    using SM = HeadSmem<NT, WV, X3P>;
+    using SM = HeadSmem<NT, WV, PL>;
     const int tid = tid_x();
     const int lane = tid & 63;
     const int wid = __builtin_amdgcn_readfirstlane(tid >> 6);
     const int q = lane >> 4, n = lane & 15;
     const int voff = lane * 16;
-    const __amdgpu_buffer_rsrc_t W2 = make_rsrc(w.pe2_h, HID * HID * 2 * X3P);
-    const __amdgpu_buffer_rsrc_t WH = make_rsrc(w.h1p_h, 3 * HID * HID * 2 * X3P);
+    X3Weights W2, WH;
+    W2.W = W2.WQ = make_rsrc(w.pe2_h, HID * HID * 2 * X3P);
+    WH.W = WH.WQ = make_rsrc(w.h1p_h, 3 * HID * HID * 2 * X3P);
+    if constexpr (PL == X3Q) {
+        W2.WQ = make_rsrc(w.pe2_q, HID * HID * 3);
+        WH.WQ = make_rsrc(w.h1p_q, 3 * HID * HID * 3);
+    }
     f16x8* act1h = reinterpret_cast<f16x8*>(sm.act1);
     f16x8* act2h = reinterpret_cast<f16x8*>(SM::kAliasAct ? sm.act1 : sm.act2);
     constexpr int D2 = X3_D2, DH = X3_DH;
@@ -740,8 +826,8 @@
     for (int t = 0; t < TPW; ++t)
 #pragma unroll
         for (int ct = 0; ct < NT; ++ct) acc2[t][ct] = cor2[t][ct] = f32x4{0.f, 0.f, 0.f, 0.f};
-    f16x8 ring2[D2 + 1][TPW][X3P];
-    stream_x3_step<0, D2, TPW, NT, D2>(W2, T2, act1h, lane, voff, ring2, acc2, cor2);
+    f16x8 ring2[D2 + 1][TPW][ring_planes<PL>()];
+    stream_x3_step<PL, 0, D2, TPW, NT, D2>(W2, T2, act1h, lane, voff, ring2, acc2, cor2);
     __syncthreads();
     PC_MARK(1);
     f32x4 bf[NT];
@@ -782,22 +868,22 @@
 #pragma unroll
                 for (int p = 0; p < X3P; ++p) act1h[(((Ta >> 1) * NT + ct + dt) * X3P + p) * 64 + lane] = pl[p];
             } else {
-                split3_pair(relu4(mfma_kgroup(a0, bf[ct], z) + bias0), relu4(mfma_kgroup(a1, bf[ct], z) + bias1), s1[ct], pl);
-#pragma unroll
-                for (int p = 0; p < X3P; ++p) act1h[(((Ta >> 1) * NT + ct) * X3P + p) * 64 + lane] = pl[p];
+                ActPlanes<PL> ap;
+                split_act<PL>(relu4(mfma_kgroup(a0, bf[ct], z) + bias0), relu4(mfma_kgroup(a1, bf[ct], z) + bias1), s1[ct], ap);
+                store_act<PL, NT>(act1h, Ta >> 1, ct, lane, ap);
             }
         }
     }
     __syncthreads();
     PC_MARK(2);
-    stream_x3_step<D2, KC_HID + D2, TPW, NT, D2>(W2, T2, act1h, lane, voff, ring2, acc2, cor2);
+    stream_x3_step<PL, D2, KC_HID + D2, TPW, NT, D2>(W2, T2, act1h, lane, voff, ring2, acc2, cor2);
     PC_MARK(3);
-    f16x8 ringh[DH + 1][TPW][X3P];
+    f16x8 ringh[DH + 1][TPW][ring_planes<PL>()];
     {
         int TH0[TPW];
 #pragma unroll
         for (int t = 0; t < TPW; ++t) TH0[t] = wid * TPW + t;
-        stream_x3_step<0, DH, TPW, NT, DH>(WH, TH0, act2h, lane, voff, ringh, acc2, cor2);
+        stream_x3_step<PL, 0, DH, TPW, NT, DH>(WH, TH0, act2h, lane, voff, ringh, acc2, cor2);
     }
     const __amdgpu_buffer_rsrc_t RP = make_rsrc(pobj, 0x7ffffff0u), RT = make_rsrc(tproj, 3 * HID * 4);
     int vo[NT];
@@ -806,7 +892,7 @@
     f32x4 tpv[TPW], pov[TPW][NP];
     head_x3_init_load<0, NT, TPW, NP>(RP, RT, vo, wid, lane, tpv, pov);
 #if X3_EPI_EARLY
-    f16x8 pls[CPW][NT][X3P];
+    ActPlanes<PL> pls[CPW][NT];
 #pragma unroll
     for (int c = 0; c < CPW; ++c) {
         const int Ta = T2[2 * c];
@@ -817,13 +903,13 @@
                 constexpr int dt = JVP ? NP : 0;
                 const f32x4 pre0 = (acc2[2 * c][ct] + cor2[2 * c][ct]) * u2[ct] + bias0;
                 const f32x4 pre1 = (acc2[2 * c + 1][ct] + cor2[2 * c + 1][ct]) * u2[ct] + bias1;
-                split3_pair(relu4(pre0), relu4(pre1), s2[ct], pls[c][ct]);
+                split3_pair(relu4(pre0), relu4(pre1), s2[ct], pls[c][ct].h);
                 split3_pair(mask4((acc2[2 * c][ct + dt] + cor2[2 * c][ct + dt]) * u2[ct + dt], pre0),
                             mask4((acc2[2 * c + 1][ct + dt] + cor2[2 * c + 1][ct + dt]) * u2[ct + dt], pre1),
-                            s2[ct + dt], pls[c][ct + dt]);
+                            s2[ct + dt], pls[c][ct + dt].h);
             } else {
-                split3_pair(relu4((acc2[2 * c][ct] + cor2[2 * c][ct]) * u2[ct] + bias0),
-                            relu4((acc2[2 * c + 1][ct] + cor2[2 * c + 1][ct]) * u2[ct] + bias1), s2[ct], pls[c][ct]);
+                split_act<PL>(relu4((acc2[2 * c][ct] + cor2[2 * c][ct]) * u2[ct] + bias0),
+                              relu4((acc2[2 * c + 1][ct] + cor2[2 * c + 1][ct]) * u2[ct] + bias1), s2[ct], pls[c][ct]);
             }
         }
     }
@@ -832,8 +918,7 @@
     for (int c = 0; c < CPW; ++c)
 #pragma unroll
         for (int ct = 0; ct < NT; ++ct)
-#pragma unroll
-            for (int p = 0; p < X3P; ++p) act2h[(((T2[2 * c] >> 1) * NT + ct) * X3P + p) * 64 + lane] = pls[c][ct][p];
+            store_act<PL, NT>(act2h, T2[2 * c] >> 1, ct, lane, pls[c][ct]);
 #else
     if constexpr (SM::kAliasAct) __syncthreads();
 #pragma unroll
@@ -844,10 +929,10 @@
         for (int ct = 0; ct < NP; ++ct) {
             f16x8 pl[X3P];
             if constexpr (!JVP) {
-                split3_pair(relu4((acc2[2 * c][ct] + cor2[2 * c][ct]) * u2[ct] + bias0),
-                            relu4((acc2[2 * c + 1][ct] + cor2[2 * c + 1][ct]) * u2[ct] + bias1), s2[ct], pl);
-#pragma unroll
-                for (int p = 0; p < X3P; ++p) act2h[(((Ta >> 1) * NT + ct) * X3P + p) * 64 + lane] = pl[p];
+                ActPlanes<PL> ap;
+                split_act<PL>(relu4((acc2[2 * c][ct] + cor2[2 * c][ct]) * u2[ct] + bias0),
+                              relu4((acc2[2 * c + 1][ct] + cor2[2 * c + 1][ct]) * u2[ct] + bias1), s2[ct], ap);
+                store_act<PL, NT>(act2h, Ta >> 1, ct, lane, ap);
             } else {
                 constexpr int dt = JVP ? NP : 0;
                 const f32x4 pre0 = (acc2[2 * c][ct] + cor2[2 * c][ct]) * u2[ct] + bias0;
@@ -871,29 +956,29 @@
     for (int v = 9 * NT; v < SM::kRedV; ++v) pv[v] = 0.f;
 #if X3_DIAG & 8
     if (wid < WV / 2) {
-        head_x3_head<0, NT, WV, TPW, DH, JVP>(WH, act2h, RP, RT, vo, sm, uh, sh, wid, lane, ringh, tpv, pov, pv);
+        head_x3_head<0, NT, WV, TPW, DH, JVP, PL>(WH, act2h, RP, RT, vo, sm, uh, sh, wid, lane, ringh, tpv, pov, pv);
         PC_MARK(13);
-        head_x3_head<1, NT, WV, TPW, DH, JVP>(WH, act2h, RP, RT, vo, sm, uh, sh, wid, lane, ringh, tpv, pov, pv);
+        head_x3_head<1, NT, WV, TPW, DH, JVP, PL>(WH, act2h, RP, RT, vo, sm, uh, sh, wid, lane, ringh, tpv, pov, pv);
         PC_MARK(14);
-        head_x3_head<2, NT, WV, TPW, DH, JVP>(WH, act2h, RP, RT, vo, sm, uh, sh, wid, lane, ringh, tpv, pov, pv);
+        head_x3_head<2, NT, WV, TPW, DH, JVP, PL>(WH, act2h, RP, RT, vo, sm, uh, sh, wid, lane, ringh, tpv, pov, pv);
         const int vw = wid + WV / 2;
         int TV[TPW];
 #pragma unroll
         for (int t = 0; t < TPW; ++t) TV[t] = vw * TPW + t;
-        stream_x3_step<0, DH, TPW, NT, DH>(WH, TV, act2h, lane, voff, ringh, acc2, cor2);
+        stream_x3_step<PL, 0, DH, TPW, NT, DH>(WH, TV, act2h, lane, voff, ringh, acc2, cor2);
         head_x3_init_load<0, NT, TPW, NP>(RP, RT, vo, vw, lane, tpv, pov);
-        head_x3_head<0, NT, WV, TPW, DH, JVP>(WH, act2h, RP, RT, vo, sm, uh, sh, vw, lane, ringh, tpv, pov, pv);
-        head_x3_head<1, NT, WV, TPW, DH, JVP>(WH, act2h, RP, RT, vo, sm, uh, sh, vw, lane, ringh, tpv, pov, pv);
-        head_x3_head<2, NT, WV, TPW, DH, JVP>(WH, act2h, RP, RT, vo, sm, uh, sh, vw, lane, ringh, tpv, pov, pv);
+        head_x3_head<0, NT, WV, TPW, DH, JVP, PL>(WH, act2h, RP, RT, vo, sm, uh, sh, vw, lane, ringh, tpv, pov, pv);
+        head_x3_head<1, NT, WV, TPW, DH, JVP, PL>(WH, act2h, RP, RT, vo, sm, uh, sh, vw, lane, ringh, tpv, pov, pv);
+        head_x3_head<2, NT, WV, TPW, DH, JVP, PL>(WH, act2h, RP, RT, vo, sm, uh, sh, vw, lane, ringh, tpv, pov, pv);
     }
 #else
-    head_x3_head<0, NT, WV, TPW, DH, JVP>(WH, act2h, RP, RT, vo, sm, uh, sh, wid, lane, ringh, tpv, pov, pv);
+    head_x3_head<0, NT, WV, TPW, DH, JVP, PL>(WH, act2h, RP, RT, vo, sm, uh, sh, wid, lane, ringh, tpv, pov, pv);
     if constexpr (X3_HEAD_BARRIER) __syncthreads();
     PC_MARK(13);
-    head_x3_head<1, NT, WV, TPW, DH, JVP>(WH, act2h, RP, RT, vo, sm, uh, sh, wid, lane, ringh, tpv, pov, pv);
+    head_x3_head<1, NT, WV, TPW, DH, JVP, PL>(WH, act2h, RP, RT, vo, sm, uh, sh, wid, lane, ringh, tpv, pov, pv);
     if constexpr (X3_HEAD_BARRIER) __syncthreads();
     PC_MARK(14);
-    head_x3_head<2, NT, WV, TPW, DH, JVP>(WH, act2h, RP, RT, vo, sm, uh, sh, wid, lane, ringh, tpv, pov, pv);
+    head_x3_head<2, NT, WV, TPW, DH, JVP, PL>(WH, act2h, RP, RT, vo, sm, uh, sh, wid, lane, ringh, tpv, pov, pv);
 #endif
     if constexpr (X3_PRIO) __builtin_amdgcn_s_setprio(0);
     PC_MARK(5);
diff --git a/genpose2_amd/csrc/gp_pack.hip b/genpose2_amd/csrc/gp_pack.hip
--- a/genpose2_amd/csrc/gp_pack.hip
+++ b/genpose2_amd/csrc/gp_pack.hip
@@ -79,6 +79,44 @@
                         }
     std::vector<uint32_t> out(h.size() / 2);
     std::memcpy(out.data(), h.data(), h.size() * 2);
+    return out;
+}
+
+uint8_t e4m3_byte(float v) {
+    const float a = std::fabs(v);
+    const uint8_t sign = std::signbit(v) ? 0x80 : 0;
+    if (a == 0.f) return sign;
+    int e = std::ilogb(a);
+    if (e < -6) e = -6;
+    int m = (int)std::nearbyint(std::ldexp(a, 3 - e));
+    if (m == 16) {
+        e += 1;
+        m = 8;
+    }
+    return sign | (uint8_t)(m < 8 ? m : (((e + 7) << 3) | (m - 8)));
+}
+
+std::vector<uint32_t> pack_q8(const std::vector<float>& w, int n_out, int k_in, int e) {
+    const int NT = n_out / 16, KGR = k_in / 128;
+    const int pe[3] = {-7, 4, 16};
+    std::vector<uint8_t> h((size_t)n_out * k_in * 3);
+    const float s = std::ldexp(1.0f, e);
+    for (int T = 0; T < NT; ++T)
+        for (int g = 0; g < KGR; ++g)
+            for (int q = 0; q < 4; ++q)
+                for (int i = 0; i < 16; ++i)
+                    for (int byte = 0; byte < 32; ++byte) {
+                        const int cc = byte >> 3, h16 = (byte >> 2) & 1, j4 = byte & 3;
+                        float r = w[(size_t)(16 * T + i) * k_in + 128 * g + 32 * cc + 16 * h16 + 4 * q + j4] * s;
+                        for (int plane = 0; plane < 3; ++plane) {
+                            const _Float16 v = (_Float16)r;
+                            r = r - (float)v;
+                            h[((((((size_t)T * KGR + g) * 3 + plane) * 2 + (byte >> 4)) * 4 + q) * 16 + i) * 16 + (byte & 15)] =
+                                e4m3_byte(std::ldexp((float)v, pe[plane]));
+                        }
+                    }
+    std::vector<uint32_t> out(h.size() / 4);
+    std::memcpy(out.data(), h.data(), h.size());
     return out;
 }
 
@@ -195,7 +233,7 @@
     return true;
 }
 
-bool pack_heads(StateDict& sd, Packer& P, int64_t* f) {
+bool pack_heads(StateDict& sd, Packer& P, int64_t* f, int64_t* fq) {
     const std::string n = "pose_score_net.";
     const float* pe0_w = sd.get(n + "pose_encoder.0.weight", 256 * 9);
     const float* pe0_b = sd.get(n + "pose_encoder.0.bias", 256);
@@ -260,6 +298,8 @@
     hsc[5] = (float)eh;
     hsc[6] = hsc[7] = 0.f;
     f[15] = P.add(hsc, 8);
+    fq[0] = P.add_bits(pack_q8(w_pe2, 256, 256, e2));
+    fq[1] = P.add_bits(pack_q8(h1_pose, 768, 256, eh));
     return true;
 }
 
@@ -277,7 +317,8 @@
 }
 
 int pack_all(int kind, int n, const char* const* names, const float* const* data, const int64_t* numel, Packer& P,
-             int64_t* fields, int64_t* enc_table) {
+             int64_t* fields, int64_t* enc_table, int64_t* fq) {
+    fq[0] = fq[1] = -1;
     GP_REQUIRE(kind >= GP_MODEL_SCORE && kind <= GP_MODEL_SCALE, "weights_pack: kind %d", kind);
     GP_REQUIRE(n >= 0 && (n == 0 || (names && data && numel)), "weights_pack: null arrays");
     StateDict sd;
@@ -293,7 +334,7 @@
         ok = pack_scale(sd, P, fields + GP_PACK_SCALE);
     } else {
         fields[GP_PACK_ENC] = 0;
-        ok = pack_encoder(sd, P, enc_table) && pack_heads(sd, P, fields + GP_PACK_HEADS);
+        ok = pack_encoder(sd, P, enc_table) && pack_heads(sd, P, fields + GP_PACK_HEADS, fq);
     }
     if (!ok) {
         gp_set_error("weights_pack: state dict entry %s", sd.missing.c_str());
@@ -318,7 +359,8 @@
                                     int64_t* fields, int64_t* enc_table) {
     GP_REQUIRE(need_floats && fields && enc_table, "weights_pack_host: null outputs");
     Packer P;
-    const int rc = pack_all(kind, n, names, data, numel, P, fields, enc_table);
+    int64_t fq[2];
+    const int rc = pack_all(kind, n, names, data, numel, P, fields, enc_table, fq);
     if (rc) return rc;
     *need_floats = P.buf.size();
     if (out) {
@@ -334,9 +376,9 @@
     GP_REQUIRE(out, "weights_pack: null out");
     *out = nullptr;
     Packer P;
-    int64_t fields[GP_PACK_NFIELDS];
+    int64_t fields[GP_PACK_NFIELDS], fq[2];
     gp_weights* w = new gp_weights();
-    int rc = pack_all(kind, n, names, data, numel, P, fields, w->table);
+    int rc = pack_all(kind, n, names, data, numel, P, fields, w->table, fq);
     if (rc) {
         delete w;
         return rc;
@@ -357,6 +399,9 @@
     } else {
         const float** h = reinterpret_cast<const float**>(&w->heads);
         for (int i = 0; i < 16; ++i) h[i] = at(fields[GP_PACK_HEADS + i]);
+        w->heads.pe2_q = at(fq[0]);
+        w->heads.h1p_q = at(fq[1]);
+        w->heads.q8_flags = GP_Q8_EVAL;
     }
     *out = w;
     return GP_OK;
diff --git a/genpose2_amd/csrc/gp_score.hip b/genpose2_amd/csrc/gp_score.hip
--- a/genpose2_amd/csrc/gp_score.hip
+++ b/genpose2_amd/csrc/gp_score.hip
@@ -111,7 +111,11 @@
                              const float* x, int rows, int k, float* score, hipStream_t stream) {
     GP_REQUIRE(w && pobj && tproj_row && x && score && rows >= 0 && k >= 1, "score_eval: bad arguments");
     if (!rows) return GP_OK;
-    if (w->pe2_h)
+    if (w->pe2_h && (w->q8_flags & GP_Q8_EVAL) && w->pe2_q && w->h1p_q &&
+        ((w->q8_flags & GP_Q8_ALL_TILES) || head_pick_nt(rows, true) == 4))
+        hipLaunchKernelGGL((head_eval_kernel<0, X3Q>), dim3((rows + 15) / 16), dim3(EVAL_WV * 64), 0, stream, *w, pobj, tproj_row,
+                       sigma, x, rows, k, score);
+    else if (w->pe2_h)
         hipLaunchKernelGGL((head_eval_kernel<0, X3P>), dim3((rows + 15) / 16), dim3(EVAL_WV * 64), 0, stream, *w, pobj, tproj_row,
                        sigma, x, rows, k, score);
     else
@@ -592,6 +596,8 @@
     GP_REQUIRE(workspace_bytes >= gp_pc_workspace_size(rows), "pc_sample: workspace too small");
     const bool split = w->pe2_h != nullptr;
     GP_REQUIRE(!split || (w->h1p_h && w->hsc), "pc_sample: pe2_h, h1p_h and hsc must be given together");
+    GP_REQUIRE((w->pe2_q != nullptr) == (w->h1p_q != nullptr), "pc_sample: pe2_q and h1p_q must be given together");
+    const bool q8 = split && gw == nullptr && w->pe2_q != nullptr && (nt == 4 || (w->q8_flags & GP_Q8_ALL_TILES));
     PCArgs a;
     a.w = *w;
     a.pobj = pobj;
@@ -632,6 +638,12 @@
             ag.gw = *gw;
             hipLaunchKernelGGL((pc_step_kernel<1, PC_WV1, 0, true>), grid, dim3(PC_WV1 * 64), 0, stream, ag, i, cur, prev);
         }
+        else if (q8 && nt == 4)
+            hipLaunchKernelGGL((pc_step_kernel<4, PC_WV1, X3Q>), grid, dim3(PC_WV1 * 64), 0, stream, a, i, cur, prev);
+        else if (q8 && nt == 2)
+            hipLaunchKernelGGL((pc_step_kernel<2, PC_WV1, X3Q>), grid, dim3(PC_WV1 * 64), 0, stream, a, i, cur, prev);
+        else if (q8)
+            hipLaunchKernelGGL((pc_step_kernel<1, PC_WV1, X3Q>), grid, dim3(PC_WV1 * 64), 0, stream, a, i, cur, prev);
         else if (nt == 4)
             hipLaunchKernelGGL((pc_step_kernel<4, PC_WV1, X3P>), grid, dim3(PC_WV1 * 64), 0, stream, a, i, cur, prev);
         else if (nt == 2)
diff --git a/genpose2_amd/device.py b/genpose2_amd/device.py
--- a/genpose2_amd/device.py
+++ b/genpose2_amd/device.py
@@ -179,12 +179,18 @@
         return out
 
 
+PC_SMALL_DEFAULT = "auto"
+
+
 class HeadModel:
 
     def __init__(self, sd: weights.StateDict, device: torch.device):
         self.lib = _lib.load()
         self.device = device
         self.up = _Uploaded(pack.pack_heads(sd), device)
+        self.pc_small = os.environ.get("GENPOSE2_PC_SMALL") or PC_SMALL_DEFAULT
+        if self.pc_small not in ("f16", "fp8", "auto"):
+            raise ValueError(f"GENPOSE2_PC_SMALL={self.pc_small!r} (f16 | fp8 | auto)")
         self.set_arith(os.environ.get("GENPOSE2_HEAD_ARITH", "f16x3"))
         self._pc_ws: Optional[torch.Tensor] = None
         self._gw = None
@@ -210,8 +216,16 @@
         ptrs = {k: self.up.ptr(k) for k in pack.HEAD_FIELDS}
         if arith == "f32":
             ptrs.update(pe2_h=None, h1p_h=None, hsc=None)
+        elif self.pc_small != "f16":
+            ptrs.update({k: self.up.ptr(k) for k in pack.HEAD_Q8_FIELDS}, q8_flags=3 if self.pc_small == "fp8" else 1)
         self.arith = arith
         self.w = _lib.HeadWeights(**ptrs)
+
+    def set_pc_small(self, form: str) -> None:
+        if form not in ("f16", "fp8", "auto"):
+            raise ValueError(f"unknown form {form!r} (f16 | fp8 | auto)")
+        self.pc_small = form
+        self.set_arith(self.arith)
 
     def _s(self):
         return ctypes.c_void_p(stream_handle(self.device))
diff --git a/genpose2_amd/pack.py b/genpose2_amd/pack.py
--- a/genpose2_amd/pack.py
+++ b/genpose2_amd/pack.py
@@ -121,6 +121,46 @@
 
 HEAD_PLANES = 3
 
+HEAD_Q8_FIELDS = ("pe2_q", "h1p_q")
+Q8_PLANE_EXPONENTS = (-7, 4, 16)
+
+
+def e4m3_bits(x: np.ndarray) -> np.ndarray:
+    x = np.asarray(x, np.float64)
+    a = np.abs(x)
+    assert float(a.max(initial=0.0)) <= 448.0
+    e = np.maximum(np.floor(np.log2(np.where(a > 0, a, 1.0))), -6.0)
+    m = np.rint(a / np.exp2(e - 3)).astype(np.int64)
+    e = np.where(m == 16, e + 1, e).astype(np.int64)
+    m = np.where(m == 16, 8, m)
+    bits = np.where(m < 8, m, ((e + 7) << 3) | (m - 8))
+    return (bits | (np.signbit(x).astype(np.int64) << 7)).astype(np.uint8)
+
+
+def e4m3_value(b: np.ndarray) -> np.ndarray:
+    b = np.asarray(b, np.uint8).astype(np.int64)
+    ex, m = (b >> 3) & 15, b & 7
+    v = np.where(ex == 0, m * 2.0 ** -9, (8 + m) * np.exp2(ex - 10.0))
+    return np.where(b & 128, -v, v)
+
+
+def pack_q8_fragments(w: np.ndarray, e: int) -> np.ndarray:
+    n_out, k_in = w.shape
+    assert n_out % 16 == 0 and k_in % 128 == 0, (n_out, k_in)
+    r = (np.asarray(w, np.float32) * np.float32(2.0 ** e)).astype(np.float32)
+    ps = []
+    for ex in Q8_PLANE_EXPONENTS:
+        h = r.astype(np.float16)
+        ps.append(e4m3_bits(h.astype(np.float64) * 2.0 ** ex))
+        r = (r - h.astype(np.float32)).astype(np.float32)
+    NT, KGR = n_out // 16, k_in // 128
+
+    def frag(p):
+        return p.reshape(NT, 16, KGR, 4, 2, 4, 4).transpose(0, 2, 5, 1, 3, 4, 6).reshape(NT, KGR, 64, 2, 16)
+    out = np.stack([frag(p) for p in ps], axis=2)
+    out = out.transpose(0, 1, 2, 4, 3, 5)
+    return np.ascontiguousarray(out).reshape(-1).view(np.int32)
+
 
 def split_constants(p: Dict[str, np.ndarray], e2: int, eh: int) -> np.ndarray:
     a0 = np.abs(p["pe0_w"].astype(np.float64)).sum(1).max()
@@ -152,6 +192,8 @@
     e2, eh = split_exponent(p["pe2_w"]), split_exponent(h1_pose)
     out["pe2_h"] = pack_h16_fragments(p["pe2_w"], e2, HEAD_PLANES)
     out["h1p_h"] = pack_h16_fragments(h1_pose, eh, HEAD_PLANES)
+    out["pe2_q"] = pack_q8_fragments(p["pe2_w"], e2)
+    out["h1p_q"] = pack_q8_fragments(h1_pose, eh)
     out["hsc"] = np.asarray(split_constants(p, e2, eh), np.float32)
     return out
 
diff --git a/include/genpose_hip.h b/include/genpose_hip.h
--- a/include/genpose_hip.h
+++ b/include/genpose_hip.h
@@ -90,7 +90,11 @@
     const void *pe2_h;
     const void *h1p_h;
     const float *hsc;
+    const void *pe2_q;
+    const void *h1p_q;
+    size_t q8_flags;
 } gp_head_weights;
+enum { GP_Q8_EVAL = 1, GP_Q8_ALL_TILES = 2 };
 
 int gp_head_object_proj(const gp_head_weights *w, const float *pts_feat, int b, float *pobj,
                         hipStream_t stream);
```
